# levayz/ProtoSAM

Measured on AMD Instinct MI355X. Metric: query-slices/sec (512x512) end-to-end ProtoSAM infer, higher is better.
Workload: dtype f16

## Files before the change

include/protosam_hip.h:

```cpp
#ifndef PROTOSAM_HIP_H
#define PROTOSAM_HIP_H
#include <stddef.h>
#ifdef __cplusplus
extern "C" {
#endif

int psam_gemm_f16(const void* A, const void* W, const float* bias, void* out, const float* resid, const float* gamma,
                  int M, int N, int K, int lda, int ldw, int ldo, int ldr, int resid_mod, int out_seg,
                  int out_seg_stride, int out_seg_off, int epilogue, void* stream);
int psam_gemm_f16_heads(const void* A, const void* W, const float* bias, void* out, int M, int N, int K, int lda, int ldw,
                        int hd, void* stream);
int psam_gemm_f16_ln(const void* A, const void* W, const float* bias, void* out, const float* resid, const float* gamma,
                     int M, int N, int K, int lda, int ldw, int ldo, int ldr, int resid_mod, int out_seg,
                     int out_seg_stride, int out_seg_off, int epilogue, void* out16, int ld16, float* stats,
                     const float* ln_mr, const float* ln_s, void* stream);
int psam_ln_finalize(const float* stats, int M, int D, float eps, float* mr, void* stream);


int psam_gemm_splitk_ranges(int M, int N, int K);
int psam_gemm_f16_splitk_ln(const void* A, const void* W, const float* bias, float* x, int M, int N, int K, int lda, int ldw, int ldx,
                            int ks, float* ws, const float* ln_w, const float* ln_b, float eps, void* out16, int ld16, void* stream);

int psam_gemm_set_tile(int tile);
int psam_gemm_asm_variant(int variant);
int psam_gemm_set_option(const char* name, int value);
int psam_gemm_set_workspace(void* ptr, size_t bytes);

int psam_layernorm(const float* x, const float* w, const float* b, void* y, float* y2, int M, int D, int ldx, int ldy,
                   float eps, int out_dtype, int zero_tail_rows, void* stream);

int psam_attention_f16(const void* qkv, void* out, const float* rel_h, const float* rel_w, const void* relq,
                       const void* rpack, const void* pad_row, int B, int N, int H, int hd, float scale, int mode, int gh,
                       int gw, int ws, int head_major, void* stream);
int psam_attention_set_variant(int v);
int psam_attention_fused_relpos(int B, int N, int H, int hd, int gh, int gw);

int psam_relpos(const void* qkv, const void* Rpack, float* rel_h, float* rel_w, void* relq, int B, int N, int H, int hd,
                int gw, int K, int windowed, float scale, int head_major, void* stream);

int psam_alp_bank(const float* sup, int ld, int h, int w, int C, const float* mask, const float* bmask, int MH, int MW,
                  int pool_w, int kernel_size, float thresh, float eps, float* bank, int cap, int* meta, int* slot_bg,
                  int* slot_fg, float* mres, int force_mode, void* stream);

int psam_alp_sim(const float* qry, long long q_bstride, int ld, int B, int npix, int C, const float* bank, int cap,
                 const int* meta, float eps, float sim_scale, float* part, float* pred, int which_only, void* stream);
int psam_alp_sim_pairs(const float* qry, long long q_bstride, int ld, int npix, int C, const void* tab, int n_entries,
                       int max_groups, float eps, float sim_scale, float* part, float* pred, void* stream);

int psam_patchify_bilinear(const float* img, int B, int C, int H, int W, int S, int P, int Kpad, void* out, void* stream);
int psam_bilinear_nchw(const float* in, int planes, int IH, int IW, int OH, int OW, float* out, void* stream);
int psam_resize2d(const float* in, int planes, int IH, int IW, int OH, int OW, int mode, float* out, void* stream);
int psam_bilinear_tokens(const float* in, long long in_bstride, int ld, int B, int ih, int iw, int C, int oh, int ow,
                         float* out, void* stream);
int psam_prob_argmax(const float* logits, int B, int IH, int IW, int OH, int OW, float* prob, void* pred, int* fg_sum,
                     void* stream);
int psam_broadcast_rows(const float* row, int D, float* out, int B, long long stride, long long off, void* stream);
int psam_prob2_argmax(const float* scores, int P, int IH, int IW, int OH, int OW, void* pred, float* pfg2, int* fg_sum,
                      float* prob, void* stream);
int psam_scores_prob_argmax(const float* scores, int P, int GH, int GW, int IH, int IW, int OH, int OW, float* prob, void* pred,
                            int* fg_sum, void* stream);
int psam_minmax(const float* x, int B, long long n_per_img, void* mm, void* stream);
int psam_sam_patchify(const float* img, const void* mm, int B, int S, int P, const float* mean3, const float* std3,
                      int quantise, void* out, void* u8out, void* stream);
int psam_normalize_chw(const void* x, int in_u8, int B, long long plane, const float* mean3, const float* std3,
                       float* y, void* stream);
int psam_im2col3x3(const void* in, int B, int H, int W, int C, void* out, void* stream);
int psam_cast_f16(const float* x, void* y, long long n, void* stream);
int psam_cast_f32(const void* x, float* y, long long n, void* stream);
int psam_gelu_f32(float* x, long long n, void* stream);
int psam_split_f16(const float* x, void* hi, void* lo, long long n, int write_hi, void* stream);

int psam_ccl(const void* pred, const float* pfg, int H, int W, int cap, int* labels, int* parent, int* counters,
             int* roots, int* acc_i, void* acc_u, double* acc_d, const int* fg_sum, double* tab, void* stream);
int psam_ccl_batch(const void* pred, const float* pfg, long long pfg_stride, int B, int H, int W, int cap, int* labels, int* parent,
                   int* counters, int* roots, int* acc_i, void* acc_u, double* acc_d, const int* fg_sum, double* tab, void* stream);

int psam_small_linear(const float* x, const float* x2, const float* W, const float* b, const float* resid, float* y,
                      int G, int M, int N, int K, long long xg, long long wg, long long bg, long long yg, int ldx,
                      int ldy, int act, void* stream);
int psam_small_linear_splitk(const float* x, const float* W, const float* b, const float* resid, float* y, float* parts, int M, int N,
                             int K, int ks, int ldx, int ldy, void* stream);
int psam_small_attention(const void* q, const float* k, const float* v, void* out, int B, int Tq, int Tk, int NH, int hd,
                         int ldq, int ldk, int ldv, int ldo, int q_f16, void* stream);
int psam_t2i_attention(const float* q, const void* K, const void* V, float* out, int B, int T, int Nk, int NH,
                       int kv_f32, void* stream);
int psam_t2i_attention_split(const float* q, const void* K, const void* V, float* out, int B, int T, int Nk, int NH,
                             int kv_f32, int S, float* part, void* stream);
int psam_gemm_f32(const float* a, const float* a2, int a2_mod, const float* w, const float* bias, const float* resid,
                  float* out, int M, int N, int K, int lda, int ldw, int ldo, void* stream);
int psam_gemm_f32_heads(const float* a, const float* a2, int a2_mod, const float* w, const float* bias, float* out, int M, int N, int K,
                        int lda, int ldw, int nk, int hd, void* stream);

int psam_gemm_f32x3(const float* a, const float* a2, int a2_mod, const void* wh, const void* wl, const float* bias, const float* resid,
                    float* out, int M, int N, int K, int lda, int ldw, int ldo, int nk, int hd, float acc_scale, void* stream);
int psam_ln_pe(const float* x, const float* add_vec, const float* w, const float* b, const float* pe, float* y32,
               void* y16, void* ype16, int M, int in_mod, int pe_mod, float eps, int do_ln, const int* img_of_prompt,
               void* stream);
int psam_dense_pe(const float* G, int gh, int gw, float* pe, void* stream);
int psam_prompt_tokens(const float* coords, const int* labels, const float* G, const float* type_emb,
                       const float* out_tok, int B, int Ns, float img_size, float* tokens, void* stream);
int psam_upscale_tail(const float* u1, const float* lnw, const float* lnb, const float* W2r, const float* b2,
                      const float* hyper, float* masks, int B, int g, void* stream);
int psam_mask_upsample(const float* low, int planes, int IN, int MID, int variant, float* out, void* stream);
int psam_mask_union(const float* low, int B, int C, int sel, int IN, int MID, int OUT, int variant, float thr,
                    float* pred, void* stream);
int psam_mask_union_seg(const float* low, int Pm, int C, int sel, int IN, const int* segs, int nseg, int nout, int MID, int OUT,
                        int variant, float thr, void* out, void* stream);

int psam_mask_stats(const float* low, int B, int C, int first, int nsel, int IN, int MID, int H, int W, int variant,
                    float thr, float off, int* stats, void* stream);
int psam_mask_binarize(const float* low, const int* idx, int n, int IN, int MID, int H, int W, int variant, float thr,
                       unsigned char* out, const unsigned char* label, long long* counts, void* stream);
int psam_plane_stats(const float* planes, int n, int H, int W, float thr, float off, int* stats, void* out, void* stream);

int psam_rle_workspace(int H, int W, long long* ints_per_mask);
int psam_rle_count(const unsigned char* masks, int n, int H, int W, int* cells, long long* totals, void* stream);
int psam_rle_write(const unsigned char* masks, int n, int H, int W, const int* cells, const long long* offsets, int* counts,
                   void* stream);
int psam_rle_decode(const long long* ends, const long long* offsets, int n, int H, int W, unsigned char* masks_out,
                    void* stream);

int psam_seg_counts(const void* pred, int pred_dtype, int pred_planes, long long pred_stride, const void* label,
                    int label_dtype, int label_planes, long long label_stride, int H, int W, const int* rows, int n,
                    long long* out, void* stream);

int psam_mask_downscale(const float* masks, const float* wts, int n, int g, float eps, float* out, void* stream);

int psam_neg_points(const int* labels, const float* pbg, const double* tab, int H, int W, int max_comp, int r, float thr,
                    unsigned long long* keys, void* stream);
int psam_neg_points_batch(const int* labels, const float* pbg, long long pbg_stride, const double* tabs, int cap, int P, int H,
                          int W, int max_comp, int r, float thr, unsigned long long* keys, void* stream);

int psam_volume_stats(const void* vol, int vol_dtype, long long n, float slope, float inter, double* out, void* stream);
int psam_volume_slices(const void* vol, int vol_dtype, int Z, int H, int W, float slope, float inter, float mean,
                       float inv_std, int S, int tile, int mode, float* out, void* stream);

int psam_im2col(const void* in, int B, int H, int W, int C, int kh, int kw, int stride, int dil, int pad, int ldo, void* out,
                void* stream);
int psam_im2col_stem(const float* img, int B, int H, int W, int ldo, void* out, void* stream);
int psam_maxpool3x3s2(const void* in, int B, int H, int W, int C, void* out, void* stream);

int psam_rotate_nearest(const float* src, float* dst, const float* xg, const float* yg, const float* rt6, int C, int H, int W,
                        int crop_y, int crop_x, int outH, int outW, void* stream);
int psam_resize_aa(const float* src, float* tmp, float* dst, int C, int H, int W, int OH, int OW, void* stream);

#ifdef __cplusplus
}
#endif
#endif
```

protosam_amd/_lib.py:

```python
import ctypes
import os

import torch

_HERE = os.path.dirname(os.path.abspath(__file__))
LIB_PATH = os.environ.get("PSAM_LIB_PATH") or os.path.join(_HERE, "libprotosam_hip.so")

c_void_p, c_int, c_float, c_longlong, c_size_t = ctypes.c_void_p, ctypes.c_int, ctypes.c_float, ctypes.c_longlong, ctypes.c_size_t

SIGNATURES = {
    "psam_gemm_f16": [c_void_p, c_void_p, c_void_p, c_void_p, c_void_p, c_void_p] + [c_int] * 12 + [c_void_p],
    "psam_gemm_f16_heads": [c_void_p, c_void_p, c_void_p, c_void_p] + [c_int] * 6 + [c_void_p],
    "psam_gemm_f16_ln": [c_void_p] * 6 + [c_int] * 12 + [c_void_p, c_int, c_void_p, c_void_p, c_void_p, c_void_p],
    "psam_ln_finalize": [c_void_p, c_int, c_int, c_float, c_void_p, c_void_p],
    "psam_gemm_splitk_ranges": [c_int, c_int, c_int],
    "psam_gemm_f16_splitk_ln": [c_void_p, c_void_p, c_void_p, c_void_p] + [c_int] * 7 + [c_void_p, c_void_p, c_void_p, c_float, c_void_p, c_int,
                                c_void_p],
    "psam_gemm_set_tile": [c_int],
    "psam_gemm_asm_variant": [c_int],
    "psam_gemm_set_option": [ctypes.c_char_p, c_int],
    "psam_gemm_set_workspace": [c_void_p, c_size_t],
    "psam_layernorm": [c_void_p, c_void_p, c_void_p, c_void_p, c_void_p, c_int, c_int, c_int, c_int, c_float,
                       c_int, c_int, c_void_p],
    "psam_attention_f16": [c_void_p, c_void_p, c_void_p, c_void_p, c_void_p, c_void_p, c_void_p, c_int, c_int, c_int, c_int,
                           c_float, c_int, c_int, c_int, c_int, c_int, c_void_p],
    "psam_attention_set_variant": [c_int],
    "psam_attention_fused_relpos": [c_int] * 6,
    "psam_relpos": [c_void_p, c_void_p, c_void_p, c_void_p, c_void_p] + [c_int] * 7 + [c_float, c_int, c_void_p],
    "psam_alp_bank": [c_void_p, c_int, c_int, c_int, c_int, c_void_p, c_void_p, c_int, c_int, c_int, c_int, c_float, c_float,
                      c_void_p, c_int, c_void_p, c_void_p, c_void_p, c_void_p, c_int, c_void_p],
    "psam_alp_sim": [c_void_p, c_longlong, c_int, c_int, c_int, c_int, c_void_p, c_int, c_void_p, c_float, c_float,
                     c_void_p, c_void_p, c_int, c_void_p],
    "psam_alp_sim_pairs": [c_void_p, c_longlong, c_int, c_int, c_int, c_void_p, c_int, c_int, c_float, c_float, c_void_p, c_void_p,
                           c_void_p],
    "psam_patchify_bilinear": [c_void_p, c_int, c_int, c_int, c_int, c_int, c_int, c_int, c_void_p, c_void_p],
    "psam_bilinear_nchw": [c_void_p, c_int, c_int, c_int, c_int, c_int, c_void_p, c_void_p],
    "psam_resize2d": [c_void_p, c_int, c_int, c_int, c_int, c_int, c_int, c_void_p, c_void_p],
    "psam_bilinear_tokens": [c_void_p, c_longlong, c_int, c_int, c_int, c_int, c_int, c_int, c_int, c_void_p, c_void_p],
    "psam_prob_argmax": [c_void_p, c_int, c_int, c_int, c_int, c_int, c_void_p, c_void_p, c_void_p, c_void_p],
    "psam_broadcast_rows": [c_void_p, c_int, c_void_p, c_int, c_longlong, c_longlong, c_void_p],
    "psam_prob2_argmax": [c_void_p, c_int, c_int, c_int, c_int, c_int, c_void_p, c_void_p, c_void_p, c_void_p, c_void_p],
    "psam_scores_prob_argmax": [c_void_p] + [c_int] * 7 + [c_void_p] * 4,
    "psam_minmax": [c_void_p, c_int, c_longlong, c_void_p, c_void_p],
    "psam_im2col3x3": [c_void_p, c_int, c_int, c_int, c_int, c_void_p, c_void_p],
    "psam_cast_f16": [c_void_p, c_void_p, c_longlong, c_void_p],
    "psam_cast_f32": [c_void_p, c_void_p, c_longlong, c_void_p],
    "psam_gelu_f32": [c_void_p, c_longlong, c_void_p],
    "psam_split_f16": [c_void_p, c_void_p, c_void_p, c_longlong, c_int, c_void_p],
    "psam_small_linear": [c_void_p] * 6 + [c_int] * 4 + [c_longlong] * 4 + [c_int] * 3 + [c_void_p],
    "psam_small_attention": [c_void_p] * 4 + [c_int] * 10 + [c_void_p],
    "psam_t2i_attention": [c_void_p] * 4 + [c_int] * 5 + [c_void_p],
    "psam_t2i_attention_split": [c_void_p] * 4 + [c_int] * 6 + [c_void_p] * 2,
    "psam_gemm_f32": [c_void_p, c_void_p, c_int, c_void_p, c_void_p, c_void_p, c_void_p] + [c_int] * 6 + [c_void_p],
    "psam_gemm_f32_heads": [c_void_p, c_void_p, c_int, c_void_p, c_void_p, c_void_p] + [c_int] * 7 + [c_void_p],
    "psam_gemm_f32x3": [c_void_p, c_void_p, c_int] + [c_void_p] * 5 + [c_int] * 8 + [c_float, c_void_p],
    "psam_small_linear_splitk": [c_void_p] * 6 + [c_int] * 6 + [c_void_p],
    "psam_ln_pe": [c_void_p] * 8 + [c_int, c_int, c_int, c_float, c_int, c_void_p, c_void_p],
    "psam_dense_pe": [c_void_p, c_int, c_int, c_void_p, c_void_p],
    "psam_prompt_tokens": [c_void_p] * 5 + [c_int, c_int, c_float, c_void_p, c_void_p],
    "psam_upscale_tail": [c_void_p] * 7 + [c_int, c_int, c_void_p],
    "psam_mask_upsample": [c_void_p, c_int, c_int, c_int, c_int, c_void_p, c_void_p],
    "psam_mask_union": [c_void_p, c_int, c_int, c_int, c_int, c_int, c_int, c_int, c_float, c_void_p, c_void_p],
    "psam_mask_union_seg": [c_void_p, c_int, c_int, c_int, c_int, c_void_p, c_int, c_int, c_int, c_int, c_int, c_float,
                            c_void_p, c_void_p],
    "psam_mask_stats": [c_void_p, c_int, c_int, c_int, c_int, c_int, c_int, c_int, c_int, c_int, c_float, c_float,
                        c_void_p, c_void_p],
    "psam_im2col": [c_void_p] + [c_int] * 10 + [c_void_p, c_void_p],
    "psam_im2col_stem": [c_void_p, c_int, c_int, c_int, c_int, c_void_p, c_void_p],
    "psam_maxpool3x3s2": [c_void_p, c_int, c_int, c_int, c_int, c_void_p, c_void_p],
    "psam_rotate_nearest": [c_void_p, c_void_p, c_void_p, c_void_p, c_void_p, c_int, c_int, c_int, c_int, c_int, c_int,
                            c_int, c_void_p],
    "psam_resize_aa": [c_void_p, c_void_p, c_void_p, c_int, c_int, c_int, c_int, c_int, c_void_p],
    "psam_volume_stats": [c_void_p, c_int, ctypes.c_longlong, c_float, c_float, c_void_p, c_void_p],
    "psam_volume_slices": [c_void_p, c_int, c_int, c_int, c_int, c_float, c_float, c_float, c_float, c_int, c_int, c_int,
                           c_void_p, c_void_p],
    "psam_neg_points": [c_void_p, c_void_p, c_void_p, c_int, c_int, c_int, c_int, c_float, c_void_p, c_void_p],
    "psam_neg_points_batch": [c_void_p, c_void_p, c_longlong, c_void_p] + [c_int] * 6 + [c_float, c_void_p, c_void_p],
    "psam_mask_downscale": [c_void_p, c_void_p, c_int, c_int, c_float, c_void_p, c_void_p],
    "psam_plane_stats": [c_void_p, c_int, c_int, c_int, c_float, c_float, c_void_p, c_void_p, c_void_p],
    "psam_rle_workspace": [c_int, c_int, ctypes.POINTER(c_longlong)],
    "psam_rle_count": [c_void_p, c_int, c_int, c_int, c_void_p, c_void_p, c_void_p],
    "psam_rle_write": [c_void_p, c_int, c_int, c_int, c_void_p, c_void_p, c_void_p, c_void_p],
    "psam_rle_decode": [c_void_p, c_void_p, c_int, c_int, c_int, c_void_p, c_void_p],
    "psam_seg_counts": [c_void_p, c_int, c_int, c_longlong, c_void_p, c_int, c_int, c_longlong, c_int, c_int, c_void_p, c_int,
                        c_void_p, c_void_p],
    "psam_mask_binarize": [c_void_p, c_void_p, c_int, c_int, c_int, c_int, c_int, c_int, c_float, c_void_p, c_void_p,
                           c_void_p, c_void_p],
    "psam_normalize_chw": [c_void_p, c_int, c_int, c_longlong, ctypes.POINTER(c_float), ctypes.POINTER(c_float),
                           c_void_p, c_void_p],
    "psam_ccl": [c_void_p, c_void_p, c_int, c_int, c_int] + [c_void_p] * 9 + [c_void_p],
    "psam_ccl_batch": [c_void_p, c_void_p, c_longlong, c_int, c_int, c_int, c_int] + [c_void_p] * 9 + [c_void_p],
    "psam_sam_patchify": [c_void_p, c_void_p, c_int, c_int, c_int, ctypes.POINTER(c_float), ctypes.POINTER(c_float),
                          c_int, c_void_p, c_void_p, c_void_p],
}

_lib = None


class HipExtensionMissing(RuntimeError):
    pass


def _preload_torch_hip_runtime():
    tl = os.path.join(os.path.dirname(torch.__file__), "lib", "libamdhip64.so")
    if os.path.exists(tl):
        ctypes.CDLL(tl, mode=ctypes.RTLD_GLOBAL)


def lib():
    global _lib
    if _lib is not None:
        return _lib
    if not os.path.exists(LIB_PATH):
        raise HipExtensionMissing(
            f"{LIB_PATH} not found: build it with `make -C protosam_amd/csrc` (or __graft_entry__.build()). "
            "protosam_amd has no CPU fallback.")
    _preload_torch_hip_runtime()
    L = ctypes.CDLL(LIB_PATH)
    for name, argtypes in SIGNATURES.items():
        fn = getattr(L, name)
        fn.argtypes = argtypes
        fn.restype = c_int
    _lib = L
    return L


def check(status, name):
    if status != 0:
        raise RuntimeError(f"{name} failed with status {status} (1 = bad argument, 2 = launch error)")
```

protosam_amd/csrc/gemm.hip:

```cpp
#include "common.h"
#include "gemm_asm_meta.h"
#include <stdlib.h>
#include <string.h>
#include <type_traits>
#include <map>
#include <string>
#include <vector>

enum { EPI_F16 = 0, EPI_GELU_F16 = 1, EPI_F32 = 2, EPI_RELU_F16 = 3 };

struct GemmArgs {
  const half_t* A;
  const half_t* W;
  const float* bias;
  void* out;
  const float* resid;
  const float* gamma;
  int M, N, K;
  int lda, ldw, ldo, ldr;
  int resid_mod;
  int out_seg;
  int out_seg_stride;
  int out_seg_off;
  int map_mode;
// ... 858 lines not shown
        bv[j][q] = p.bias ? *reinterpret_cast<const float4*>(p.bias + nbase + j * 32 + 8 * q + 4 * lg)
                          : make_float4(0.f, 0.f, 0.f, 0.f);
        if (LNF) sv[j][q] = *reinterpret_cast<const float4*>(p.ln_s + nbase + j * 32 + 8 * q + 4 * lg);
      }
    if (LNF) {
#pragma unroll
      for (int sidx = 0; sidx < 4; ++sidx) {
        int m = mbase + sidx * 32 + lr;
        m = m < p.M ? m : p.M - 1;
        mrv[sidx] = *reinterpret_cast<const float2*>(p.ln_mr + (size_t)m * 2);
      }
    }
    __builtin_amdgcn_sched_barrier(0);
    issue_next();
    __builtin_amdgcn_sched_barrier(0);
#pragma unroll
    for (int sidx = 0; sidx < 4; ++sidx) {
      if (LNF) {
        slab_park16h<true>(acc[sidx >> 1][sidx & 1][0], acc[sidx >> 1][sidx & 1][1], slab, bv, lane, EPI == EPI_GELU_F16, sv,
                           mrv[sidx]);
      } else {
        slab_park16h<false>(acc[sidx >> 1][sidx & 1][0], acc[sidx >> 1][sidx & 1][1], slab, bv, lane, EPI == EPI_GELU_F16, bv,
                            make_float2(0.f, 1.f));
      }
      slab_emit16h(slab, mbase + sidx * 32, nbase, lane, p);
    }
  }
}

template <int EPI, bool LNF = false, bool SPLITK = false>
__global__ __launch_bounds__(512) void gemm8kp_f16_kernel(GemmArgs p, int total) {
  extern __shared__ __attribute__((aligned(16))) half_t ring[];
  constexpr int HT = 128 * 64;
  const int ntn = p.N / 256;
  const int ntm = (p.M + 255) / 256;
  const int t = threadIdx.x, lane = t & 63;
  const int wv = __builtin_amdgcn_readfirstlane(t >> 6);
  const int wr = wv >> 2, wc = wv & 3;
  const int lr = lane & 31, lg = lane >> 5;
  half_t* slab = ring + 8 * HT + wv * 2048;
  const int nk = p.K / 64;
  const unsigned bh = 32u * (unsigned)p.ldw;
  const int arow0 = wr * 64 + lr, brow0 = wc * 32 + lr;

  const int KSP = SPLITK ? p.ksplit : 1;
  int idx = blockIdx.x, tm = 0, tn = 0;
  while (idx < total && !tile_map(idx / KSP, ntm, ntn, p.map_mode, tm, tn)) idx += gridDim.x;
  if (idx >= total) return;
  int k_lo = SPLITK ? (idx % KSP) * nk / KSP : 0, k_hi = SPLITK ? (idx % KSP + 1) * nk / KSP : nk;

  unsigned aoff[2][2], boff[2];
  auto offsets = [&](int m0, int n0) {
#pragma unroll
    for (int j = 0; j < 2; ++j) {
      const int lrow = j * 64 + (t >> 3);
      const int chunk = (t & 7) ^ ((lrow >> 1) & 7);
      const int arow = (lrow >> 6) * 128 + (lrow & 63);
      const int brow = (lrow >> 5) * 64 + (lrow & 31);
#pragma unroll
      for (int h = 0; h < 2; ++h) {
        int am = m0 + arow + h * 64;
        am = am < p.M ? am : p.M - 1;
        aoff[j][h] = (unsigned)am * (unsigned)p.lda + chunk * 8;
      }
      boff[j] = (unsigned)(n0 + brow) * (unsigned)p.ldw + chunk * 8;
    }
  };
  auto stage = [&](int which, int kt) {
    half_t* dst = ring + ((kt & 1) * 4 + which) * HT + wv * 512;
    const int h = which & 1;
#pragma unroll
    for (int j = 0; j < 2; ++j) {
      const half_t* g = which < 2 ? p.A + (aoff[j][h] + (unsigned)kt * 64u) : p.W + (boff[j] + h * bh + (unsigned)kt * 64u);
      glds16(g, dst + j * 4096);
    }
  };
  auto prologue = [&](int k0, int k1) {
    stage(0, k0); stage(2, k0); stage(3, k0); stage(1, k0);
    if (k1 - k0 > 1) stage(0, k0 + 1);
  };

  offsets(tm * 256, tn * 256);
  prologue(k_lo, k_hi);

  half8_t fa[2][2];
  half8_t fb[2][2][2];

#define RD_A(bufp, h, kh)                                                                                         \
  _Pragma("unroll") for (int i = 0; i < 2; ++i) _Pragma("unroll") for (int k2 = 0; k2 < 2; ++k2)                   \
      fa[i][k2] = *reinterpret_cast<const half8_t*>(&(bufp)[(h) * HT + lds_off64(arow0 + i * 32, ((kh) * 2 + k2) * 2 + lg)]);
#define RD_B(bufp, kh)                                                                                            \
  _Pragma("unroll") for (int b = 0; b < 2; ++b) _Pragma("unroll") for (int k2 = 0; k2 < 2; ++k2)                   \
      fb[kh][b][k2] = *reinterpret_cast<const half8_t*>(&(bufp)[(2 + b) * HT + lds_off64(brow0, ((kh) * 2 + k2) * 2 + lg)]);
#define MMA_H(a, kh)                                                                                              \
  _Pragma("unroll") for (int k2 = 0; k2 < 2; ++k2) _Pragma("unroll") for (int i = 0; i < 2; ++i)                   \
      _Pragma("unroll") for (int b = 0; b < 2; ++b)                                                               \
          acc[a][i][b] = __builtin_amdgcn_mfma_f32_32x32x16_f16(fb[kh][b][k2], fa[i][k2], acc[a][i][b], 0, 0, 0);
#define PHASE_SYNC_IN()                                   \
  __builtin_amdgcn_s_barrier();                           \
  asm volatile("s_waitcnt lgkmcnt(0)" ::: "memory");      \
  __builtin_amdgcn_sched_barrier(0);                      \
  __builtin_amdgcn_s_setprio(1);
#define PHASE_SYNC_OUT()                                  \
  __builtin_amdgcn_s_setprio(0);                          \
  __builtin_amdgcn_sched_barrier(0);                      \
  __builtin_amdgcn_s_barrier();                           \
  asm volatile("" ::: "memory");

  bool first = true;
  for (;;) {
    const int m0 = tm * 256, n0 = tn * 256;
    f32x16 acc[2][2][2];
#pragma unroll
    for (int a = 0; a < 2; ++a)
#pragma unroll
      for (int i = 0; i < 2; ++i)
#pragma unroll
        for (int b = 0; b < 2; ++b)
#pragma unroll
          for (int r = 0; r < 16; ++r) acc[a][i][b][r] = 0.f;

    if (first) { if (k_hi - k_lo > 1) wait_vmcnt<4>(); else wait_vmcnt<2>(); } else { wait_vmcnt<0>(); }
    first = false;
    __builtin_amdgcn_s_barrier();
    if (wr == 1) __builtin_amdgcn_s_barrier();
    asm volatile("" ::: "memory");

    for (int kt = k_lo; kt < k_hi; ++kt) {
      const half_t* buf = ring + (kt & 1) * 4 * HT;
      const bool more1 = kt + 1 < k_hi, more2 = kt + 2 < k_hi;
#define LOAD_PHASE(RDS, ST) RDS __builtin_amdgcn_sched_barrier(0); ST
      LOAD_PHASE(RD_B(buf, 0) __builtin_amdgcn_sched_barrier(0); RD_A(buf, 0, 0), if (more1) stage(2, kt + 1);)
      if (more1) wait_vmcnt<6>(); else wait_vmcnt<0>();
      PHASE_SYNC_IN();
      MMA_H(0, 0)
      PHASE_SYNC_OUT();
      LOAD_PHASE(RD_B(buf, 1) __builtin_amdgcn_sched_barrier(0); RD_A(buf, 0, 1), if (more1) stage(3, kt + 1);)
      if (more1) wait_vmcnt<6>(); else wait_vmcnt<0>();
      PHASE_SYNC_IN();
      MMA_H(0, 1)
      PHASE_SYNC_OUT();
      LOAD_PHASE(RD_A(buf, 1, 0), if (more1) stage(1, kt + 1);)
      if (more1) wait_vmcnt<6>(); else wait_vmcnt<0>();
      PHASE_SYNC_IN();
      MMA_H(1, 0)
      PHASE_SYNC_OUT();
      LOAD_PHASE(RD_A(buf, 1, 1), if (more2) stage(0, kt + 2);)
      if (more2) { wait_vmcnt<4>(); } else if (more1) { wait_vmcnt<2>(); } else { wait_vmcnt<0>(); }
      PHASE_SYNC_IN();
      MMA_H(1, 1)
      PHASE_SYNC_OUT();
#undef LOAD_PHASE
    }
    if (wr == 0) __builtin_amdgcn_s_barrier();

    int nidx = idx + gridDim.x, ntm_ = 0, ntn_ = 0;
    while (nidx < total && !tile_map(nidx / KSP, ntm, ntn, p.map_mode, ntm_, ntn_)) nidx += gridDim.x;
    const bool have = nidx < total;
    const int nk_lo = SPLITK && have ? (nidx % KSP) * nk / KSP : 0, nk_hi = SPLITK && have ? (nidx % KSP + 1) * nk / KSP : nk;
    auto issue_next = [&]() {
      if (have) {
        offsets(ntm_ * 256, ntn_ * 256);
        prologue(nk_lo, nk_hi);
      }
    };
    __builtin_amdgcn_sched_barrier(0);
#ifndef PSAM_EPI_EARLY_NEXT
#define PSAM_EPI_EARLY_NEXT 1
#endif
#if PSAM_EPI_EARLY_NEXT
    persist_epilogue<EPI, LNF, SPLITK>(acc, slab, m0 + wr * 128, n0 + wc * 64, lane, p, SPLITK ? idx % KSP : 0, issue_next);
#else
    issue_next();
    __builtin_amdgcn_sched_barrier(0);
    persist_epilogue<EPI, LNF, SPLITK>(acc, slab, m0 + wr * 128, n0 + wc * 64, lane, p, SPLITK ? idx % KSP : 0);
#endif
    if (!have) break;
    idx = nidx; tm = ntm_; tn = ntn_; k_lo = nk_lo; k_hi = nk_hi;
  }
#undef RD_A
#undef RD_B
#undef MMA_H
#undef PHASE_SYNC_IN
#undef PHASE_SYNC_OUT
}

template <int EPI, bool LNF = false>
static void launch8kp(const GemmArgs& p, hipStream_t s) {
  constexpr int LDS = 2 * 4 * 128 * 64 * 2 + 8 * 4096;
  static bool attr = false;
  if (!attr) {
    (void)hipFuncSetAttribute((const void*)gemm8kp_f16_kernel<EPI, LNF>, hipFuncAttributeMaxDynamicSharedMemorySize, LDS);
    attr = true;
  }
  const int ntm = (p.M + 255) / 256, ntn = p.N / 256;
  GemmArgs q = p;
  q.map_mode = pick_map_mode(ntm, ntn);
  const int total = tile_map_grid(ntm, ntn, q.map_mode);
  hipLaunchKernelGGL((gemm8kp_f16_kernel<EPI, LNF>), dim3(total < num_cus() ? total : num_cus()), dim3(512), LDS, s, q, total);
}

__global__ __launch_bounds__(256) void splitk_reduce_kernel(const float* __restrict__ ws, int ks, const float* __restrict__ bias,
                                                            const float* __restrict__ gamma, const float* resid, int ldr,
                                                            int resid_mod, float* out, int ldo, int M, int N) {
  const int n4 = N >> 2;
  const size_t i = (size_t)blockIdx.x * 256 + threadIdx.x;
  if (i >= (size_t)M * n4) return;
  const int m = (int)(i / n4), n = (int)(i - (size_t)m * n4) * 4;
  float4 v = bias ? *reinterpret_cast<const float4*>(bias + n) : make_float4(0.f, 0.f, 0.f, 0.f);
  for (int r = 0; r < ks; ++r) {
    const float4 q = *reinterpret_cast<const float4*>(ws + ((size_t)r * M + m) * N + n);
    v.x += q.x; v.y += q.y; v.z += q.z; v.w += q.w;
  }
  if (gamma) {
    const float4 g = *reinterpret_cast<const float4*>(gamma + n);
    v.x *= g.x; v.y *= g.y; v.z *= g.z; v.w *= g.w;
  }
  if (resid) {
    const size_t rrow = resid_mod ? (size_t)(m % resid_mod) : (size_t)m;
    const float4 r = *reinterpret_cast<const float4*>(resid + rrow * ldr + n);
    v.x += r.x; v.y += r.y; v.z += r.z; v.w += r.w;
  }
  *reinterpret_cast<float4*>(out + (size_t)m * ldo + n) = v;
}

struct KsWorkspace { float* ptr = nullptr; size_t bytes = 0; hipEvent_t done = nullptr; hipStream_t last = nullptr; bool used = false; };
static std::map<int, KsWorkspace> g_ks;
static KsWorkspace* ks_workspace() {
  int dev = 0;
  (void)hipGetDevice(&dev);
  auto it = g_ks.find(dev);
  return it == g_ks.end() || !it->second.ptr ? nullptr : &it->second;
}
extern "C" int psam_gemm_set_workspace(void* ptr, size_t bytes) {
  if (ptr && (reinterpret_cast<uintptr_t>(ptr) & 15)) return PSAM_ERR_ARG;
  int dev = 0;
  (void)hipGetDevice(&dev);
  KsWorkspace& w = g_ks[dev];
  w.ptr = (float*)ptr;
  w.bytes = ptr ? bytes : 0;
  w.used = false;
  return PSAM_OK;
}

static void launch8kp_splitk(const GemmArgs& p, hipStream_t s) {
  constexpr int LDS = 2 * 4 * 128 * 64 * 2 + 8 * 4096;
  static bool attr = false;
  if (!attr) {
    (void)hipFuncSetAttribute((const void*)gemm8kp_f16_kernel<EPI_F32, false, true>, hipFuncAttributeMaxDynamicSharedMemorySize, LDS);
    attr = true;
  }
  const int ntm = (p.M + 255) / 256, ntn = p.N / 256;
  GemmArgs q = p;
  q.map_mode = 1;
  KsWorkspace* w = ks_workspace();
  q.ks_ws = w->ptr;
  if (w->used && w->last != s) (void)hipStreamWaitEvent(s, w->done, 0);
  const int total = ntm * ntn * q.ksplit;
  hipLaunchKernelGGL((gemm8kp_f16_kernel<EPI_F32, false, true>), dim3(total < num_cus() ? total : num_cus()), dim3(512), LDS, s, q, total);
  const size_t n4 = (size_t)p.M * (p.N / 4);
  hipLaunchKernelGGL(splitk_reduce_kernel, dim3((unsigned)((n4 + 255) / 256)), dim3(256), 0, s, w->ptr, q.ksplit, p.bias, p.gamma,
                     p.resid, p.ldr, p.resid_mod, reinterpret_cast<float*>(p.out), p.ldo, p.M, p.N);
  if (!w->done) (void)hipEventCreateWithFlags(&w->done, hipEventDisableTiming);
  (void)hipEventRecord(w->done, s);
  w->last = s;
  w->used = true;
}


extern "C" const unsigned char psam_gemm_asm_co[];
extern "C" const unsigned char psam_gemm_asm_co_end[];
struct AsmGemmArgs {
  const void* A; const void* W; const void* bias; void* out; const void* resid; const void* gamma; const void* tab;
  int M, N, K, lda, ldw, ldo, ldr, G, flags, pad;
  void* trace;
  void* out16; float* stats; int ld16, pad2;
};
static_assert(sizeof(AsmGemmArgs) == 128, "kernarg layout of gemm_asm_gen.py");
struct AsmModule { hipModule_t mod = nullptr; int state = 0; std::map<int, std::vector<hipFunction_t>> fns; std::map<std::string, hipFunction_t> named; };
static std::map<int, AsmModule> g_asm;
static int g_asm_variant = 0;
extern "C" int psam_gemm_asm_variant(int v) {
  g_asm_variant = v;
  return PSAM_OK;
}
static AsmModule* asm_module() {
  AsmModule& m = g_asm[cur_device()];
  if (m.state == 0) {
    m.state = -1;
    const char* path = getenv("PSAM_GEMM_ASM_CO");
    hipError_t st = path ? hipModuleLoad(&m.mod, path) : hipModuleLoadData(&m.mod, psam_gemm_asm_co);
    if (st != hipSuccess) { (void)hipGetLastError(); return nullptr; }
    m.state = 1;
  }
  return m.state < 0 ? nullptr : &m;
}
static const hipFunction_t* asm_load(int family = 1) {
  AsmModule* m = asm_module();
  if (!m) return nullptr;
  const int key = family * 1000 + g_asm_variant;
  auto it = m->fns.find(key);
  if (it != m->fns.end()) return it->second.data();
  const char* names[3] = {"f16", "gelu", "f32"};
  const char* suffix[3] = {"", "_l2", "_ln"};
  const int nf = (family == 1 && g_asm_variant == 0) ? 9 : 3;
  std::vector<hipFunction_t> f(9, nullptr);
  for (int i = 0; i < nf; ++i) {
    std::string n = std::string(family == 2 ? "psam_gemm_asm2_" : "psam_gemm_asm_") + names[i % 3] + suffix[i / 3] +
                    (g_asm_variant > 0 ? "_v" + std::to_string(g_asm_variant) : std::string());
    if (hipModuleGetFunction(&f[i], m->mod, n.c_str()) != hipSuccess) {
      (void)hipGetLastError();
      if (i < 6) return nullptr;
      f[i] = nullptr;
    }
  }
  for (int i = nf; i < 6; ++i) f[i] = f[i - 3];
  return (m->fns[key] = f).data();
}
hipFunction_t psam_asm_function(const char* name) {
  AsmModule* m = asm_module();
  if (!m) return nullptr;
  auto it = m->named.find(name);
  if (it != m->named.end()) return it->second;
  hipFunction_t f = nullptr;
  if (hipModuleGetFunction(&f, m->mod, name) != hipSuccess) { (void)hipGetLastError(); f = nullptr; }
  return m->named[name] = f;
}
struct AsmTable { int grid; int* dev; };
static std::map<unsigned long long, AsmTable> g_asm_tabs;
static const AsmTable* asm_table(int ntm, int ntn, int mode, int halves = 0, int wg_per_cu = 1) {
  int dev = 0;
  (void)hipGetDevice(&dev);
  if (ntm >= 4096 || ntn >= (1 << 20)) return nullptr;
  const unsigned long long key = ((unsigned long long)eff_cus() << 52) | ((unsigned long long)ntm << 40) | ((unsigned long long)ntn << 20) | ((unsigned long long)(halves ? 1 : 0) << 19) |
                                 ((unsigned long long)(halves & 1) << 18) | ((unsigned long long)(wg_per_cu - 1) << 16) | ((unsigned long long)mode << 8) | (unsigned)dev;
  auto it = g_asm_tabs.find(key);
  if (it != g_asm_tabs.end()) return &it->second;
  const int total = tile_map_grid(ntm, ntn, mode);
  const int G = total < eff_cus() * wg_per_cu ? total : eff_cus() * wg_per_cu;
  std::vector<std::vector<int>> lists(G);
  for (int b = 0; b < G; ++b)
    for (int idx = b; idx < total; idx += G) {
      int tm = 0, tn = 0;
      if (!tile_map(idx, ntm, ntn, mode, tm, tn)) continue;
      if (!halves) { lists[b].push_back(tm | (tn << 16)); continue; }
      lists[b].push_back(tm | ((2 * tn) << 16));
      if (2 * tn + 1 < halves) lists[b].push_back(tm | ((2 * tn + 1) << 16));
    }
  size_t rows = 0;
  for (auto& l : lists) rows = l.size() > rows ? l.size() : rows;
  rows += 3;
  std::vector<int> h(rows * G, -1);
  for (int b = 0; b < G; ++b)
    for (size_t i = 0; i < lists[b].size(); ++i) h[i * G + b] = lists[b][i];
  AsmTable t;
  t.grid = G;
  t.dev = nullptr;
  if (hipMalloc((void**)&t.dev, h.size() * sizeof(int)) != hipSuccess) return nullptr;
  if (hipMemcpy(t.dev, h.data(), h.size() * sizeof(int), hipMemcpyHostToDevice) != hipSuccess) {
    (void)hipFree(t.dev);
    return nullptr;
  }
  return &(g_asm_tabs[key] = t);
}
static bool asm_eligible(const GemmArgs& p, int epilogue, int lnf) {
  if (lnf) {
    const hipFunction_t* f = asm_load(1);
    const bool cons = p.ln_mr || p.ln_s, prod = p.out16 || p.stats;
    if (!f || g_asm_variant != 0 || (cons && prod)) return false;
    if (cons && (!f[6 + epilogue] || !p.ln_mr || !p.ln_s || !p.bias || (reinterpret_cast<uintptr_t>(p.ln_mr) & 15) || (reinterpret_cast<uintptr_t>(p.ln_s) & 15))) return false;
    if (prod && (!f[8] || !p.out16 || !p.stats)) return false;
  }
  if (p.head_hd || p.out_seg || epilogue > EPI_F32) return false;
  if (p.resid_mod && (epilogue != EPI_F32 || !p.resid || p.resid_mod < 256 || (p.resid_mod & (p.resid_mod - 1)) != 0 || g_asm_variant != 0)) return false;
  if (p.N % 256 || p.K % 64 || p.K < 128 || p.M < 1) return false;
  if ((p.lda % 8) || (p.ldw % 8) || (reinterpret_cast<uintptr_t>(p.A) & 15) || (reinterpret_cast<uintptr_t>(p.W) & 15)) return false;
  const unsigned long long lim = 0xffffffffull;
  if ((unsigned long long)p.M * p.lda * 2 > lim || (unsigned long long)p.N * p.ldw * 2 > lim) return false;
  if (p.bias && (reinterpret_cast<uintptr_t>(p.bias) & 15)) return false;
  if (epilogue == EPI_F32) {
    if ((p.ldo % 4) || (reinterpret_cast<uintptr_t>(p.out) & 15) || (unsigned long long)p.M * p.ldo * 4 > lim) return false;
    if (p.resid && ((p.ldr % 4) || (reinterpret_cast<uintptr_t>(p.resid) & 15) || (unsigned long long)p.M * p.ldr * 4 > lim)) return false;
    if (p.gamma && (reinterpret_cast<uintptr_t>(p.gamma) & 15)) return false;
  } else {
    if (!p.wide16 || (unsigned long long)p.M * p.ldo * 2 > lim) return false;
  }
  return true;
}
static bool asm2_eligible(const GemmArgs& p, int epilogue, int lnf) {
  if (epilogue > EPI_F32 || (p.N % 128)) return false;
  GemmArgs q = p;
  q.N = 256;
  if (lnf || p.resid_mod || !asm_eligible(q, epilogue, 0)) return false;
  if ((unsigned long long)p.N * p.ldw * 2 > 0xffffffffull) return false;
  const int e = epilogue == EPI_F16 ? PSAM_ASM2_E_F16 : epilogue == EPI_GELU_F16 ? PSAM_ASM2_E_GELU : PSAM_ASM2_E_F32;
  return p.K / 64 >= e + 1 && p.K / 64 >= 3;
}
static int launch_asm(const GemmArgs& p, int epilogue, hipStream_t s, int family = 1) {
  const hipFunction_t* fns = asm_load(family);
  if (!fns) return PSAM_ERR_LAUNCH;
  const int ntm = (p.M + 255) / 256, ntn = family >= 2 ? p.N / 128 : p.N / 256;
  const AsmTable* t = asm_table(ntm, ntn, pick_map_mode(ntm, ntn));
  if (!t) return PSAM_ERR_LAUNCH;
  AsmGemmArgs a;
  a.A = p.A; a.W = p.W; a.bias = p.bias; a.out = p.out; a.resid = p.resid; a.gamma = p.gamma; a.tab = t->dev;
  a.M = p.M; a.N = p.N; a.K = p.K; a.lda = p.lda; a.ldw = p.ldw; a.ldo = p.ldo; a.ldr = p.resid ? p.ldr : 0; a.G = t->grid;
  a.flags = p.gamma ? 1 : 0;
  a.pad = (family == 1 && p.resid_mod > 0) ? p.resid_mod - 1 : -1;
  a.trace = nullptr;
  const bool ln_cons = family == 1 && p.ln_mr && p.ln_s, ln_prod = family == 1 && (p.out16 || p.stats);
  if (ln_cons) {
    a.resid = p.ln_mr;
    a.gamma = p.ln_s + p.N;
  }
  a.out16 = p.out16; a.stats = p.stats; a.ld16 = p.ld16; a.pad2 = 0;
  static const char* tr = getenv("PSAM_GEMM_ASM_TRACE");
  const bool trace = tr && g_asm_variant > 0;
  if (trace) { (void)hipMalloc(&a.trace, (size_t)t->grid * 32); (void)hipMemsetAsync(a.trace, 0, (size_t)t->grid * 32, s); }
  size_t sz = ln_prod ? sizeof(a) : 104;
  void* extra[] = {HIP_LAUNCH_PARAM_BUFFER_POINTER, &a, HIP_LAUNCH_PARAM_BUFFER_SIZE, &sz, HIP_LAUNCH_PARAM_END};
  const size_t out_bytes = (size_t)p.M * p.N * (epilogue == EPI_F32 ? 4 : 2);
  const int fsel = (ln_cons || ln_prod) ? 6 + epilogue : epilogue + ((family == 1 && out_bytes <= ((size_t)48 << 20)) ? 3 : 0);
  if (hipModuleLaunchKernel(fns[fsel], t->grid, 1, 1, 256, 1, 1, 0, s, nullptr, extra) != hipSuccess) {
    (void)hipGetLastError();
    return PSAM_ERR_LAUNCH;
  }
  if (trace) {
    std::vector<unsigned> h((size_t)t->grid * 8);
    (void)hipStreamSynchronize(s);
    (void)hipMemcpy(h.data(), a.trace, h.size() * 4, hipMemcpyDeviceToHost);
    (void)hipFree(a.trace);
    double loop = 0, epi = 0, kt = 0, tot = 0, rt = 0;
    unsigned tmax = 0;
    for (int b = 0; b < t->grid; ++b) rt += h[(size_t)t->grid * 4 + b * 4];
    for (int b = 0; b < t->grid; ++b) { loop += h[b * 4]; epi += h[b * 4 + 1]; kt += h[b * 4 + 2]; tot += h[b * 4 + 3]; tmax = h[b * 4 + 3] > tmax ? h[b * 4 + 3] : tmax; }
    const double tiles = kt / (p.K / 64);
    if (kt > 0) fprintf(stderr, "asm v%d %dx%dx%d epi%d: %.0f cycles per K-tile, %.0f cycles per epilogue (%.1f tiles per workgroup) kernel entry to exit: mean %.0f max %u cycles = %.1f us (shader clock %.0f MHz)\n", g_asm_variant, p.M, p.N,
                        p.K, epilogue, loop / kt, epi / tiles, tiles / t->grid, tot / t->grid, tmax, rt / t->grid * 0.01, rt > 0 ? tot / rt * 100.0 : 0.0);
  }
  return PSAM_OK;
}

static const AsmTable* asm_table_splitk(int ntm, int ntn, int ks) {
  int dev = 0;
  (void)hipGetDevice(&dev);
  if (ntm >= 4096 || ntn >= (1 << 16) || ks < 2 || ks > 8) return nullptr;
  const unsigned long long key = (1ull << 63) | ((unsigned long long)eff_cus() << 52) | ((unsigned long long)ntm << 40) | ((unsigned long long)ntn << 20) |
                                 ((unsigned long long)ks << 8) | (unsigned)dev;
  auto it = g_asm_tabs.find(key);
  if (it != g_asm_tabs.end()) return &it->second;
  const int mode = pick_map_mode(ntm, ntn);
  const int ntiles = tile_map_grid(ntm, ntn, mode);
  std::vector<int> items;
  for (int idx = 0; idx < ntiles; ++idx) {
    int tm = 0, tn = 0;
    if (!tile_map(idx, ntm, ntn, mode, tm, tn)) continue;
    for (int r = 0; r < ks; ++r) items.push_back(tm | (r << 12) | (tn << 16));
  }
  const int total = (int)items.size();
  const int G = total < eff_cus() ? total : eff_cus();
  const size_t rows = (size_t)(total + G - 1) / G + 3;
  std::vector<int> h(rows * G, -1);
  for (int i = 0; i < total; ++i) h[(size_t)(i / G) * G + (i % G)] = items[i];
  AsmTable t;
  t.grid = G;
  t.dev = nullptr;
  if (hipMalloc((void**)&t.dev, h.size() * sizeof(int)) != hipSuccess) return nullptr;
  if (hipMemcpy(t.dev, h.data(), h.size() * sizeof(int), hipMemcpyHostToDevice) != hipSuccess) {
    (void)hipFree(t.dev);
    return nullptr;
  }
  return &(g_asm_tabs[key] = t);
}

#define SKR_MAXV 8
__global__ __launch_bounds__(256) void splitk_reduce_ln_kernel(const float* __restrict__ ws, int ks, const float* __restrict__ bias,
                                                               float* __restrict__ x, int ldx, const float* __restrict__ ln_w,
                                                               const float* __restrict__ ln_b, float eps, half_t* __restrict__ out16, int ld16,
                                                               int M, int N) {
  const int row = blockIdx.x * 4 + (threadIdx.x >> 6), lane = threadIdx.x & 63;
  if (row >= M) return;
  const int nv = N >> 2;
  const size_t Mp = (size_t)((M + 255) & ~255);
  float4 v[SKR_MAXV];
  float* xr = x + (size_t)row * ldx;
#pragma unroll
  for (int k = 0; k < SKR_MAXV; ++k) {
    const int i = lane + 64 * k;
    if (i < nv) v[k] = bias ? reinterpret_cast<const float4*>(bias)[i] : make_float4(0.f, 0.f, 0.f, 0.f);
  }
  for (int r = 0; r < ks; ++r) {
    const float4* pr = reinterpret_cast<const float4*>(ws + ((size_t)r * Mp + row) * N);
#pragma unroll
    for (int k = 0; k < SKR_MAXV; ++k) {
      const int i = lane + 64 * k;
      if (i < nv) { const float4 q = pr[i]; v[k].x += q.x; v[k].y += q.y; v[k].z += q.z; v[k].w += q.w; }
    }
  }
  float s = 0.f;
#pragma unroll
  for (int k = 0; k < SKR_MAXV; ++k) {
    const int i = lane + 64 * k;
    if (i < nv) {
      const float4 q = reinterpret_cast<const float4*>(xr)[i];
      v[k].x += q.x; v[k].y += q.y; v[k].z += q.z; v[k].w += q.w;
      reinterpret_cast<float4*>(xr)[i] = v[k];
      s += (v[k].x + v[k].y) + (v[k].z + v[k].w);
    }
  }
  if (!out16) return;
  float mean = 0.f, rstd = 1.f;
  if (ln_w) {
    mean = wave_sum(s) / (float)N;
    float q = 0.f;
#pragma unroll
    for (int k = 0; k < SKR_MAXV; ++k) {
      const int i = lane + 64 * k;
      if (i < nv) {
        const float a = v[k].x - mean, c = v[k].y - mean, d = v[k].z - mean, e = v[k].w - mean;
        q += (a * a + c * c) + (d * d + e * e);
      }
    }
    rstd = 1.0f / sqrtf(wave_sum(q) / (float)N + eps);
  }
#pragma unroll
  for (int k = 0; k < SKR_MAXV; ++k) {
    const int i = lane + 64 * k;
    if (i < nv) {
      float o0 = v[k].x, o1 = v[k].y, o2 = v[k].z, o3 = v[k].w;
      if (ln_w) {
        const float4 ww = reinterpret_cast<const float4*>(ln_w)[i], bb = reinterpret_cast<const float4*>(ln_b)[i];
        o0 = (o0 - mean) * rstd * ww.x + bb.x; o1 = (o1 - mean) * rstd * ww.y + bb.y;
        o2 = (o2 - mean) * rstd * ww.z + bb.z; o3 = (o3 - mean) * rstd * ww.w + bb.w;
      }
      half4_t h = {(half_t)o0, (half_t)o1, (half_t)o2, (half_t)o3};
      *reinterpret_cast<half4_t*>(out16 + (size_t)row * ld16 + i * 4) = h;
    }
  }
}

extern "C" int psam_gemm_splitk_ranges(int M, int N, int K) {
  if (M <= 0 || N <= 0 || K <= 0 || (N % 256) || (K % 64) || N > 64 * 4 * SKR_MAXV) return 0;
  const int tiles = ((M + 255) / 256) * (N / 256), nkt = K / 64, ncu = eff_cus();
  if (tiles * 2 > ncu) return 0;
  int ks = ncu / tiles;
  if (ks > 8) ks = 8;
  while (ks >= 2 && nkt / ks < 16) --ks;
  if (ks < 2 || tiles * ks * 4 < ncu * 3) return 0;
  return psam_asm_function("psam_gemm_asm_f32_sk") ? ks : 0;
}

extern "C" int psam_gemm_f16_splitk_ln(const void* A, const void* W, const float* bias, float* x, int M, int N, int K, int lda, int ldw,
                                       int ldx, int ks, float* ws, const float* ln_w, const float* ln_b, float eps, void* out16, int ld16,
                                       void* stream) {
  if (ks < 2 || ks > 8 || ks != psam_gemm_splitk_ranges(M, N, K) || !ws || !x || (ldx % 4) || (ln_w && !ln_b) || (out16 && (ld16 % 4)))
    return PSAM_ERR_ARG;
  if ((reinterpret_cast<uintptr_t>(ws) | reinterpret_cast<uintptr_t>(x) | reinterpret_cast<uintptr_t>(bias) | reinterpret_cast<uintptr_t>(ln_w) |
       reinterpret_cast<uintptr_t>(ln_b)) & 15 || (reinterpret_cast<uintptr_t>(out16) & 7))
    return PSAM_ERR_ARG;
  GemmArgs p;
  p.A = (const half_t*)A; p.W = (const half_t*)W; p.bias = nullptr; p.out = ws; p.resid = nullptr; p.gamma = nullptr;
  p.M = M; p.N = N; p.K = K; p.lda = lda; p.ldw = ldw; p.ldo = N; p.ldr = 0;
  p.resid_mod = 0; p.out_seg = 0; p.out_seg_stride = 0; p.out_seg_off = 0; p.map_mode = 0; p.head_hd = 0;
  p.out16 = nullptr; p.ld16 = 0; p.stats = nullptr; p.ln_mr = nullptr; p.ln_s = nullptr; p.wide16 = false; p.ksplit = 1; p.ks_ws = nullptr;
  if (!asm_eligible(p, EPI_F32, 0) || (unsigned long long)ks * ((M + 255) & ~255) * N * 4 > 0xffffffffull) return PSAM_ERR_ARG;
  hipFunction_t fn = psam_asm_function("psam_gemm_asm_f32_sk");
  const AsmTable* t = asm_table_splitk((M + 255) / 256, N / 256, ks);
  if (!fn || !t) return PSAM_ERR_LAUNCH;
  AsmGemmArgs a;
  a.A = A; a.W = W; a.bias = nullptr; a.out = ws; a.resid = nullptr; a.gamma = nullptr; a.tab = t->dev;
  a.M = M; a.N = N; a.K = K; a.lda = lda; a.ldw = ldw; a.ldo = N; a.ldr = 0; a.G = t->grid; a.flags = 0; a.pad = ks;
  a.trace = nullptr; a.out16 = nullptr; a.stats = nullptr; a.ld16 = 0; a.pad2 = 0;
  size_t sz = 104;
  void* extra[] = {HIP_LAUNCH_PARAM_BUFFER_POINTER, &a, HIP_LAUNCH_PARAM_BUFFER_SIZE, &sz, HIP_LAUNCH_PARAM_END};
  hipStream_t s = (hipStream_t)stream;
  if (hipModuleLaunchKernel(fn, t->grid, 1, 1, 256, 1, 1, 0, s, nullptr, extra) != hipSuccess) {
    (void)hipGetLastError();
    return PSAM_ERR_LAUNCH;
  }
  hipLaunchKernelGGL(splitk_reduce_ln_kernel, dim3((M + 3) / 4), dim3(256), 0, s, ws, ks, bias, x, ldx, ln_w, ln_b, eps, (half_t*)out16, ld16, M, N);
  return psam_launch_status();
}

enum { OPT_ASM = 0, OPT_HALF, OPT_SPLITK, OPT_NSPLIT, OPT_DEEP, OPT_SMALL, OPT_COUNT };
static const char* const g_opt_names[OPT_COUNT] = {"asm", "half_tiles", "splitk", "nsplit", "deep", "small"};
static const char* const g_opt_env[OPT_COUNT] = {"PSAM_GEMM_ASM", "PSAM_GEMM_HALF", "PSAM_GEMM_SPLITK", "PSAM_GEMM_NSPLIT", "PSAM_GEMM_DEEP", "PSAM_GEMM_SMALL"};
static int g_opt[OPT_COUNT] = {-1, -1, -1, -1, -1, -1};
static int gemm_option(int i) {
  if (g_opt[i] < 0) { const char* e = getenv(g_opt_env[i]); g_opt[i] = e ? (atoi(e) != 0) : 1; }
  return g_opt[i];
}
extern "C" int psam_gemm_set_option(const char* name, int value) {
  if (name && strcmp(name, "max_wgs") == 0) { g_max_wgs = value > 0 ? value : 0; return PSAM_OK; }
  for (int i = 0; i < OPT_COUNT; ++i)
    if (name && strcmp(name, g_opt_names[i]) == 0) { g_opt[i] = value != 0; return PSAM_OK; }
  return PSAM_ERR_ARG;
}
static int g_tile_override = -1;
extern "C" int psam_gemm_set_tile(int t) {
  g_tile_override = t;
  return PSAM_OK;
}
static int pick_tile(int M, int N, int K, int epilogue) {
  if (g_tile_override < 0) {
    const char* e = getenv("PSAM_GEMM_TILE");
    g_tile_override = e ? atoi(e) : 0;
  }
  if (g_tile_override > 0) return g_tile_override;
  if (N % 256 == 0) {
    const long t256 = (long)((M + 255) / 256) * (N / 256);
    const long ncu = eff_cus();
    const long rounds = (t256 + ncu - 1) / ncu;
    const bool short_f32 = epilogue == EPI_F32 && K < 2048;
    const int fill = short_f32 ? 95 : (epilogue == EPI_F32 || rounds > 1) ? 80 : 50;
    if (K >= 768 && t256 * 100 >= rounds * ncu * fill) {
      return gemm_option(OPT_ASM) ? 15 : 11;
    }
  }
  if (N % 128 == 0 && K >= 768) {
    const int half_on = gemm_option(OPT_HALF);
    const long th = (long)((M + 255) / 256) * (N / 128), ncu = eff_cus();
    if (half_on && th * 20 >= ncu * 9) return 16;
  }
  return 1;
}

struct LnFold {
  void* out16 = nullptr;
  int ld16 = 0;
  float* stats = nullptr;
  const float* ln_mr = nullptr;
  const float* ln_s = nullptr;
};

static int gemm_dispatch(const void* A, const void* W, const float* bias, void* out, const float* resid,
                         const float* gamma, int M, int N, int K, int lda, int ldw, int ldo, int ldr,
                         int resid_mod, int out_seg, int out_seg_stride, int out_seg_off, int epilogue, int head_hd,
                         void* stream, const LnFold& ln = LnFold()) {
  if (M <= 0 || N <= 0 || K <= 0 || (N % BN) != 0 || (K % BK) != 0 || (lda % 8) != 0 || (ldw % 8) != 0 ||
      (ldo % 4) != 0 || (resid && (ldr % 4) != 0))
    return PSAM_ERR_ARG;
  if (epilogue < 0 || epilogue > 3) return PSAM_ERR_ARG;
  if (epilogue == EPI_RELU_F16 && resid_mod != 0) return PSAM_ERR_ARG;
  GemmArgs p;
  p.A = (const half_t*)A;
  p.W = (const half_t*)W;
  p.bias = bias;
  p.out = out;
  p.resid = resid;
  p.gamma = gamma;
  p.M = M;
  p.N = N;
  p.K = K;
  p.lda = lda;
  p.ldw = ldw;
  p.ldo = ldo;
  p.ldr = ldr;
  p.resid_mod = resid_mod;
  p.out_seg = out_seg;
  p.out_seg_stride = out_seg_stride;
  p.out_seg_off = out_seg_off;
  { static int mm = -2; if (mm == -2) { const char* e = getenv("PSAM_GEMM_MAP"); mm = e ? atoi(e) : (xcd_maps_apply() ? 0 : 1); } p.map_mode = mm; }
  p.head_hd = head_hd;
  p.out16 = (half_t*)ln.out16;
  p.ld16 = ln.ld16;
  p.stats = ln.stats;
  p.ln_mr = ln.ln_mr;
  p.ln_s = ln.ln_s;
  const bool ln_prod = ln.out16 || ln.stats, ln_cons = ln.ln_mr || ln.ln_s;
  if (ln_prod && (epilogue != EPI_F32 || (ln.out16 && ((ln.ld16 % 8) != 0 || (reinterpret_cast<uintptr_t>(ln.out16) & 15) != 0)))) return PSAM_ERR_ARG;
  if (ln_cons && (!(epilogue == EPI_F16 || epilogue == EPI_GELU_F16) || !ln.ln_mr || !ln.ln_s)) return PSAM_ERR_ARG;
  const int ntm = (M + BM - 1) / BM, ntn = N / BN;
  dim3 grid(tile_map_grid(ntm, ntn, p.map_mode)), block(256);
  hipStream_t s = (hipStream_t)stream;
  int tsel = epilogue == EPI_RELU_F16 ? 1 : pick_tile(M, N, K, epilogue);
  p.wide16 = (ldo % 8) == 0 && (reinterpret_cast<uintptr_t>(out) & 15) == 0 && (!head_hd || head_hd % 8 == 0);
  if (tsel == 16 && !asm2_eligible(p, epilogue, ln_prod || ln_cons)) tsel = (g_tile_override > 0 || ln_prod || ln_cons) ? 15 : 1;
  if (tsel == 15 && !asm_eligible(p, epilogue, ln_prod || ln_cons)) tsel = (N % 256 == 0) ? 11 : 1;
  if (tsel != 1 && tsel != 11 && tsel != 12 && tsel != 13 && tsel != 15 && tsel != 16) tsel = (N % 256 == 0) ? 11 : 1;
  if (tsel == 11 && (N % 256) != 0) tsel = 1;
  if (tsel == 11 && epilogue != EPI_F32 && !p.wide16) tsel = 1;
  if (ln_cons && !p.wide16) return PSAM_ERR_ARG;
  {
    static const bool logging = getenv("PSAM_GEMM_LOG") != nullptr;
    if (logging) {
      static std::map<std::string, int> seen;
      char key[160];
      snprintf(key, sizeof(key), "%d x %d x %d epilogue %d ln %d%d head_hd %d out_seg %d resid_mod %d -> tile %d", M, N, K, epilogue, (int)ln_prod,
               (int)ln_cons, head_hd, out_seg, resid_mod, tsel);
      if (seen[key]++ == 0) fprintf(stderr, "psam_gemm_f16: %s\n", key);
    }
  }
  if (tsel == 15) return launch_asm(p, epilogue, s);
  if (tsel == 16) return launch_asm(p, epilogue, s, 2);
  p.ksplit = 1;
  p.ks_ws = nullptr;
  {
    const int ks_on = gemm_option(OPT_SPLITK);
    const bool auto_sel = g_tile_override <= 0;
    const KsWorkspace* ksw = ks_workspace();
    hipStreamCaptureStatus cap = hipStreamCaptureStatusNone;
    if (ksw && hipStreamIsCapturing(s, &cap) != hipSuccess) { (void)hipGetLastError(); cap = hipStreamCaptureStatusNone; }
    if (ks_on && auto_sel && ksw && cap == hipStreamCaptureStatusNone && tsel == 1 && epilogue == EPI_F32 && !ln_prod && !ln_cons && !head_hd && N % 256 == 0 &&
        out_seg == 0 && (ldo % 4) == 0) {
      const int t256 = ((M + 255) / 256) * (N / 256), nkt = K / 64;
      int ks = num_cus() / t256;
      if (ks > nkt / 24) ks = nkt / 24;
      if (ks > 8) ks = 8;
      while (ks >= 2 && (size_t)ks * M * N * sizeof(float) > ksw->bytes) --ks;
      if (ks >= 2 && t256 * ks * 4 >= num_cus() * 3) {
        p.ksplit = ks;
        launch8kp_splitk(p, s);
        return psam_launch_status();
      }
    }
  }
  const bool lnf = ln_prod || ln_cons;
  if ((tsel == 13 || (tsel == 1 && g_tile_override <= 0 && gemm_option(OPT_SMALL) && (int)grid.x * 2 <= num_cus())) && !lnf && !head_hd && K >= 64 &&
      epilogue != EPI_RELU_F16 && (epilogue == EPI_F32 || (ldo % 4) == 0)) {
    switch (epilogue) {
      case EPI_F16: launch_s64<EPI_F16>(p, s); break;
      case EPI_GELU_F16: launch_s64<EPI_GELU_F16>(p, s); break;
      default: launch_s64<EPI_F32>(p, s); break;
    }
    return psam_launch_status();
  }
  if (tsel == 13) tsel = 1;
  if ((tsel == 12 || (tsel == 1 && g_tile_override <= 0 && gemm_option(OPT_DEEP) && (int)grid.x <= num_cus())) && !lnf && K >= 256 &&
      epilogue != EPI_RELU_F16) {
    switch (epilogue) {
      case EPI_F16: launch_deep<EPI_F16>(p, grid, s); break;
      case EPI_GELU_F16: launch_deep<EPI_GELU_F16>(p, grid, s); break;
      default: launch_deep<EPI_F32>(p, grid, s); break;
    }
    return psam_launch_status();
  }
  if (tsel == 12) tsel = 1;
  if (tsel == 11) {
    if (lnf) {
      if (epilogue == EPI_F16) launch8kp<EPI_F16, true>(p, s);
      else if (epilogue == EPI_GELU_F16) launch8kp<EPI_GELU_F16, true>(p, s);
      else launch8kp<EPI_F32, true>(p, s);
    } else {
      if (epilogue == EPI_F16) launch8kp<EPI_F16>(p, s);
      else if (epilogue == EPI_GELU_F16) launch8kp<EPI_GELU_F16>(p, s);
      else launch8kp<EPI_F32>(p, s);
    }
    return psam_launch_status();
  }
  if (lnf) {
    switch (epilogue) {
      case EPI_F16: hipLaunchKernelGGL((gemm_f16_kernel<EPI_F16, true>), grid, block, 0, s, p); break;
      case EPI_GELU_F16: hipLaunchKernelGGL((gemm_f16_kernel<EPI_GELU_F16, true>), grid, block, 0, s, p); break;
      default: hipLaunchKernelGGL((gemm_f16_kernel<EPI_F32, true>), grid, block, 0, s, p); break;
    }
    return psam_launch_status();
  }
  switch (epilogue) {
    case EPI_F16: hipLaunchKernelGGL(gemm_f16_kernel<EPI_F16>, grid, block, 0, s, p); break;
    case EPI_GELU_F16: hipLaunchKernelGGL(gemm_f16_kernel<EPI_GELU_F16>, grid, block, 0, s, p); break;
    case EPI_RELU_F16: hipLaunchKernelGGL(gemm_f16_kernel<EPI_RELU_F16>, grid, block, 0, s, p); break;
    default: hipLaunchKernelGGL(gemm_f16_kernel<EPI_F32>, grid, block, 0, s, p); break;
  }
  return psam_launch_status();
}

extern "C" int psam_gemm_f16(const void* A, const void* W, const float* bias, void* out, const float* resid,
                             const float* gamma, int M, int N, int K, int lda, int ldw, int ldo, int ldr,
                             int resid_mod, int out_seg, int out_seg_stride, int out_seg_off, int epilogue,
                             void* stream) {
  {
    const int ns_on = gemm_option(OPT_NSPLIT);
    const int ncu = num_cus();
    const int ntm = (M + 255) / 256;
    const bool whole16 = epilogue == EPI_GELU_F16 && pick_tile(M, N, K, epilogue) == 16 && K / 64 >= PSAM_ASM2_E_GELU + 1 &&
                         (lda % 8) == 0 && (ldw % 8) == 0 && (ldo % 8) == 0 && ((reinterpret_cast<uintptr_t>(A) | reinterpret_cast<uintptr_t>(W) |
                           reinterpret_cast<uintptr_t>(out) | reinterpret_cast<uintptr_t>(bias)) & 15) == 0;
    if (ns_on && !whole16 && g_tile_override <= 0 && (epilogue == EPI_F16 || epilogue == EPI_GELU_F16) && out_seg == 0 && N % 256 == 0 &&
        K >= 768 && ntm > 0 && ntm <= ncu) {
      const int ntn = N / 256, c1 = ncu / ntm;
      if (c1 >= 1 && c1 < ntn && ntm * c1 * 100 >= ncu * 95 && (ntn - c1) * 2 <= c1) {
        const int n1 = c1 * 256;
        const half_t* Wh = (const half_t*)W;
        int st = gemm_dispatch(A, W, bias, out, resid, gamma, M, n1, K, lda, ldw, ldo, ldr, resid_mod, 0, 0, 0, epilogue, 0, stream);
        if (st != PSAM_OK) return st;
        return gemm_dispatch(A, Wh + (size_t)n1 * ldw, bias ? bias + n1 : nullptr, (half_t*)out + n1, resid, gamma ? gamma + n1 : nullptr,
                             M, N - n1, K, lda, ldw, ldo, ldr, resid_mod, 0, 0, 0, epilogue, 0, stream);
      }
    }
  }
  return gemm_dispatch(A, W, bias, out, resid, gamma, M, N, K, lda, ldw, ldo, ldr, resid_mod, out_seg, out_seg_stride,
                       out_seg_off, epilogue, 0, stream);
}

extern "C" int psam_gemm_f16_ln(const void* A, const void* W, const float* bias, void* out, const float* resid,
                                const float* gamma, int M, int N, int K, int lda, int ldw, int ldo, int ldr, int resid_mod,
                                int out_seg, int out_seg_stride, int out_seg_off, int epilogue, void* out16, int ld16,
                                float* stats, const float* ln_mr, const float* ln_s, void* stream) {
  LnFold ln;
  ln.out16 = out16; ln.ld16 = ld16; ln.stats = stats; ln.ln_mr = ln_mr; ln.ln_s = ln_s;
  if (stats && (N % 64) != 0) return PSAM_ERR_ARG;
  return gemm_dispatch(A, W, bias, out, resid, gamma, M, N, K, lda, ldw, ldo, ldr, resid_mod, out_seg, out_seg_stride,
                       out_seg_off, epilogue, 0, stream, ln);
}

extern "C" int psam_gemm_f16_heads(const void* A, const void* W, const float* bias, void* out, int M, int N, int K, int lda,
                                   int ldw, int hd, void* stream) {
  if (hd <= 0 || (hd % 4) != 0 || (N % hd) != 0) return PSAM_ERR_ARG;
  return gemm_dispatch(A, W, bias, out, nullptr, nullptr, M, N, K, lda, ldw,  N, 0, 0, 0, 0, 0, EPI_F16,
                       hd, stream);
}
```

protosam_amd/csrc/gemm_asm_gen.py:

```python
#!/usr/bin/env python3
import sys

from asm_common import AsmWriter, kernel_begin, kernel_end, kernel_metadata, module_text, younger

import os
_pol = (os.environ.get("PSAM_GEN_GEMM_DMA", ",") + ",").split(",")
DMA_POLICY_A, DMA_POLICY_W = (" " + _pol[0] if _pol[0] else ""), (" " + _pol[1] if _pol[1] else "")
GELU_MODE = os.environ.get("PSAM_GEN_GELU", "sigpoly")

S_KARG = 0
S_WG = 2
S_A, S_W, S_BIAS, S_OUT, S_RES, S_GAM, S_TAB = 4, 6, 8, 10, 12, 14, 16
S_M, S_N, S_K, S_LDA, S_LDW, S_LDO, S_LDR, S_G, S_FLAGS = 18, 19, 20, 21, 22, 23, 24, 25, 26
S_RMASK = 27
SRD_A, SRD_B, SRD_O, SRD_R, SRD_BIAS, SRD_GAM = 28, 32, 36, 40, 44, 48
S_M0BASE = 68
S_KREM, S_DKREM, S_NK = 69, 70, 71
S_TCUR, S_TDMA, S_TNEXT, S_CUR, S_STRIDE = 72, 73, 74, 75, 76
S_WV, S_WR, S_WC = 77, 78, 79
S_FA, S_FB = 80, 81
S_LDA2, S_LDW2 = 82, 83
S_T0, S_T1, S_T2, S_T3, S_T4 = 84, 85, 86, 87, 88
S_ROW4, S_TOFF, S_N0X4, S_ROFF, S_RROW4 = 89, 90, 91, 92, 93
S_C = 52
S_ROW28, S_RROW28 = 65, 66
S_ACC_LOOP, S_ACC_EPI, S_NKT = 67, 94, 95
S_TS0, S_TS1, S_TRP = 96, 98, 100
S_SKQ, S_SKREM, S_SKR, S_SKT = 96, 97, 98, 99
NUM_SGPR = 102

V_TID = 0
V_FA = 1
V_FB = 5
V_DA = 9
V_DB = 17
V_LANE, V_LR, V_LG, V_T0, V_T1, V_T2, V_T3 = 25, 26, 27, 28, 29, 30, 31
V_SFOFF, V_MFOFF, V_RSOFF, V_RSTD = 25, 26, 27, 28
SRD_O16, SRD_ST = 96, 52
S_LD16X2, S_O16ROW4, S_STROW4, S_O16ROW28, S_STROW28, S_PARTS8, S_O16OFF, S_STOFF = 56, 57, 58, 59, 60, 61, 62, 63
S_EXROW = 100
V_O16, V_ST, V_SQ, V_SUM = 25, 254, 26, 252
SRD_MR, SRD_SF, SRD_MF = 40, 48, 96
V_SET = [32, 64, 96, 128]
V_PARK = 160
V_EADDR = 176
V_EM = [180, 212]
V_TMP = 244
V_BIAS = 96
V_OLANE, V_RLANE, V_O, V_R = 248, 249, 250, 251
V_BG0, V_GG0, V_BG1, V_GG1 = 168, 172, 244, 28

LDS_BUF = 16384
LDS_SLAB = 131072

EPI_F16, EPI_GELU_F16, EPI_F32 = 0, 1, 2


class Gen(AsmWriter):
    def __init__(self, name, epi, sched):
        AsmWriter.__init__(self, name)
        self.epi, self.sched = epi, sched
        self.lnc = bool(sched.get("ln_cons")) and epi != EPI_F32
        self.lnp = bool(sched.get("ln_prod")) and epi == EPI_F32
        self.sk = bool(sched.get("splitk")) and epi == EPI_F32 and not self.lnp
        assert not (self.sk and sched.get("trace"))

    def item_rows_cols(self, item):
        e = self.e
        e("s_and_b32 s%d, s%d, 0x%x" % (S_T0, item, 0xfff if self.sk else 0xffff))
        e("s_lshr_b32 s%d, s%d, 16" % (S_T1, item))

    def item_ktiles(self, item, dst):
        e = self.e
        e("s_bfe_u32 s%d, s%d, 0x4000c" % (S_SKR, item))
        e("s_cmp_lt_u32 s%d, s%d" % (S_SKR, S_SKREM))
        e("s_addc_u32 s%d, s%d, 0" % (dst, S_SKQ))

    def switch_tile(self):
        e = self.e
        done, out = self.u("L_sw_none"), self.u("L_sw_out")
        e("s_mov_b32 s%d, s%d" % (S_TDMA, S_TNEXT))
        e("s_cmp_eq_u32 s%d, -1" % S_TDMA)
        e("s_cbranch_scc1 %s" % done)
        self.item_rows_cols(S_TDMA)
        e("s_lshl_b32 s%d, s%d, 8" % (S_T0, S_T0))
        e("s_lshl_b32 s%d, s%d, 8" % (S_T1, S_T1))
        e("s_mul_i32 s%d, s%d, s%d" % (S_T2, S_T0, S_LDA2))
        e("s_mul_hi_u32 s%d, s%d, s%d" % (S_T3, S_T0, S_LDA2))
        e("s_add_u32 s%d, s%d, s%d" % (SRD_A, S_A, S_T2))
        e("s_addc_u32 s%d, s%d, s%d" % (SRD_A + 1, S_A + 1, S_T3))
        e("s_sub_u32 s%d, s%d, s%d" % (S_T4, S_M, S_T0))
        e("s_mul_i32 s%d, s%d, s%d" % (SRD_A + 2, S_T4, S_LDA2))
        e("s_mul_i32 s%d, s%d, s%d" % (S_T2, S_T1, S_LDW2))
        e("s_mul_hi_u32 s%d, s%d, s%d" % (S_T3, S_T1, S_LDW2))
        e("s_add_u32 s%d, s%d, s%d" % (SRD_B, S_W, S_T2))
        e("s_addc_u32 s%d, s%d, s%d" % (SRD_B + 1, S_W + 1, S_T3))
        e("s_sub_u32 s%d, s%d, s%d" % (S_T4, S_N, S_T1))
        e("s_mul_i32 s%d, s%d, s%d" % (SRD_B + 2, S_T4, S_LDW2))
        if self.sk:
            self.item_ktiles(S_TDMA, S_DKREM)
            e("s_min_u32 s%d, s%d, s%d" % (S_SKT, S_SKR, S_SKREM))
            e("s_mul_i32 s%d, s%d, s%d" % (S_T4, S_SKR, S_SKQ))
            e("s_add_u32 s%d, s%d, s%d" % (S_T4, S_T4, S_SKT))
            e("s_lshl_b32 s%d, s%d, 7" % (S_T4, S_T4))
            for srd in (SRD_A, SRD_B):
                e("s_add_u32 s%d, s%d, s%d" % (srd, srd, S_T4))
                e("s_addc_u32 s%d, s%d, 0" % (srd + 1, srd + 1))
                e("s_max_u32 s%d, s%d, s%d" % (srd + 2, srd + 2, S_T4))
                e("s_sub_u32 s%d, s%d, s%d" % (srd + 2, srd + 2, S_T4))
        else:
            e("s_mov_b32 s%d, s%d" % (S_DKREM, S_NK))
        e("s_add_u32 s%d, s%d, s%d" % (S_CUR, S_CUR, S_STRIDE))
        e("s_load_dword s%d, s[%d:%d], s%d" % (S_TNEXT, S_TAB, S_TAB + 1, S_CUR))
        e("s_branch %s" % out)
        self.lab(done)
        e("s_mov_b32 s%d, 0" % (SRD_A + 2))
        e("s_mov_b32 s%d, 0" % (SRD_B + 2))
        e("s_mov_b32 s%d, 0x7fffffff" % S_DKREM)
        self.lab(out)

    def dma_m0(self, p):
        j = p & 7
        const = (65536 if p >= 8 else 0) + (j >> 2) * 32768 + (j & 3) * 4096
        return "s_add_u32 m0, s%d, 0x%x" % (S_M0BASE, const)

    def dma_issue(self, p):
        if p < 8:
            return "buffer_load_dwordx4 v%d, s[%d:%d], 0 offen%s lds" % (V_DA + p, SRD_A, SRD_A + 3, DMA_POLICY_A)
        return "buffer_load_dwordx4 v%d, s[%d:%d], 0 offen%s lds" % (V_DB + p - 8, SRD_B, SRD_B + 3, DMA_POLICY_W)

    def dma_advance(self):
        out = []
        for srd in (SRD_A, SRD_B):
            out += ["s_add_u32 s%d, s%d, 128" % (srd, srd), "s_addc_u32 s%d, s%d, 0" % (srd + 1, srd + 1),
                    "s_max_u32 s%d, s%d, 128" % (srd + 2, srd + 2), "s_sub_u32 s%d, s%d, 128" % (srd + 2, srd + 2)]
        out.append("s_sub_u32 s%d, s%d, 1" % (S_DKREM, S_DKREM))
        return out

    def frag_read(self, st, ks, idx):
        if idx < 4:
            return "ds_read_b128 v[%d:%d], v%d offset:%d" % (V_SET[st] + 4 * idx, V_SET[st] + 4 * idx + 3, V_FA + ks, idx * 4096)
        j = idx - 4
        return "ds_read_b128 v[%d:%d], v%d offset:%d" % (V_SET[st] + 16 + 4 * j, V_SET[st] + 16 + 4 * j + 3, V_FB + ks, j * 4096)

    def mfma(self, st, rb, cb, zero):
        blk = (rb * 4 + cb) * 16
        a = "v[%d:%d]" % (V_SET[st] + 16 + 4 * cb, V_SET[st] + 16 + 4 * cb + 3)
        b = "v[%d:%d]" % (V_SET[st] + 4 * rb, V_SET[st] + 4 * rb + 3)
        cc = "0" if zero else "a[%d:%d]" % (blk, blk + 15)
        return "v_mfma_f32_32x32x16_f16 a[%d:%d], %s, %s, %s" % (blk, blk + 15, a, b, cc)

    def build_slots(self):
        sc = self.sched
        slots = [[] for _ in range(64)]
        for i in range(16):
            if not sc.get("no_reads"):
                slots[sc["rd23"][i]].append(self.frag_read(2 + i // 8, 2 + i // 8, i % 8))
        for i, r in enumerate((V_FA + 2, V_FA + 3, V_FB + 2, V_FB + 3)):
            slots[sc["tog23"] + i].append("v_xor_b32 v%d, 0x%x, v%d" % (r, LDS_BUF, r))
        if not sc.get("no_epilogue"):
            slots[sc.get("pre_slot", 17)] += ["s_cmp_eq_u32 s%d, 1" % S_KREM, "s_cbranch_scc1 L_pre_%s" % self.name, "L_pre_ret_%s:" % self.name]
        if self.lnc and not sc.get("no_epilogue"):
            slots[48] += ["s_cmp_eq_u32 s%d, 1" % S_KREM, "s_cbranch_scc1 L_pre2_%s" % self.name, "L_pre2_ret_%s:" % self.name]
        a = sc["barA"]
        if not sc.get("no_barrier"):
            slots[a] += ["s_waitcnt lgkmcnt(0)", "s_barrier"]
        slots[a] += ["s_cmp_eq_u32 s%d, 0" % S_DKREM, "s_cbranch_scc1 L_switch_%s" % self.name, "L_switch_ret_%s:" % self.name]
        for p in range(16):
            s = sc["dma"][p]
            if sc.get("no_dma"):
                continue
            slots[s - 1].append(self.dma_m0(p))
            slots[s].append(self.dma_issue(p))
        last = sc["dma"][15]
        adv = self.dma_advance()
        for i, ins in enumerate(adv):
            slots[min(63, last + 1 + i // 3)].append(ins)
        slots[min(63, last + 1)].append("s_xor_b32 s%d, s%d, 0x%x" % (S_M0BASE, S_M0BASE, LDS_BUF))
        b = sc["barB"]
        issued = sum(1 for p in range(16) if sc["dma"][p] <= b)
        if not sc.get("no_barrier"):
            slots[b] += ["s_waitcnt vmcnt(%d)" % (0 if sc.get("no_dma") else issued), "s_barrier"]
        if sc.get("prio"):
            slots[0].insert(0, "s_setprio %d" % sc["prio"])
        for i in range(16):
            s = sc["rd01"][i]
            assert s > b
            if not sc.get("no_reads"):
                slots[s].append(self.frag_read(i // 8, i // 8, i % 8))
        return slots

    def ktile(self, slots, zero_first):
        e = self.e
        for s in range(64):
            ks, rb, cb = s // 16, (s % 16) // 4, s % 4
            if s == 0:
                e("s_waitcnt lgkmcnt(8)")
            if s == 16:
                e("s_waitcnt lgkmcnt(15)")
            e(self.mfma(ks, rb, cb, zero_first and ks == 0))
            for ins in slots[s]:
                if ins.endswith(":"):
                    self.lab(ins[:-1])
                else:
                    e(ins)
            if s == 15 and zero_first:
                e("s_branch L_after_ks0_%s" % self.name)
                return

    def gelu_pair(self, x, t):
        e = self.e
        d, n, p = t, t + 2, t + 4
        mode = self.sched.get("gelu_mode", "packed")
        if mode == "none":
            return
        e("v_pk_mul_f32 v[%d:%d], v[%d:%d], v[%d:%d]" % (n, n + 1, x, x + 1, x, x + 1))
        for i in range(2):
            e("v_fma_f32 v%d, |v%d|, s%d, 1.0" % (d + i, x + i, S_C))
        e("v_pk_mul_f32 v[%d:%d], v[%d:%d], s[%d:%d] op_sel_hi:[1,0]" % (n, n + 1, n, n + 1, S_C + 4, S_C + 5))
        for i in range(2):
            e(("v_mov_b32 v%d, v%d" if mode == "notrans" else "v_rcp_f32 v%d, v%d") % (d + i, d + i))
        for i in range(2):
            e(("v_mov_b32 v%d, v%d" if mode == "notrans" else "v_exp_f32 v%d, v%d") % (n + i, n + i))
        e("v_pk_fma_f32 v[%d:%d], v[%d:%d], s[%d:%d], v[%d:%d] op_sel_hi:[1,0,1]" % (p, p + 1, d, d + 1, S_C + 2, S_C + 3, V_TMP + 8, V_TMP + 9))
        for k in range(3):
            e("v_pk_fma_f32 v[%d:%d], v[%d:%d], v[%d:%d], s[%d:%d] op_sel_hi:[1,1,0]" % (p, p + 1, p, p + 1, d, d + 1, S_C + 6 + 2 * k, S_C + 7 + 2 * k))
        e("v_pk_mul_f32 v[%d:%d], v[%d:%d], v[%d:%d] neg_lo:[0,1] neg_hi:[0,1]" % (p, p + 1, d, d + 1, p, p + 1))
        e("v_pk_fma_f32 v[%d:%d], v[%d:%d], v[%d:%d], 1.0 op_sel_hi:[1,1,0]" % (p, p + 1, p, p + 1, n, n + 1))
        for i in range(2):
            e("v_bfi_b32 v%d, s%d, v%d, v%d" % (p + i, S_C + 12, p + i, x + i))
        e("v_pk_mul_f32 v[%d:%d], v[%d:%d], 0.5 op_sel_hi:[1,0]" % (x, x + 1, x, x + 1))
        e("v_pk_fma_f32 v[%d:%d], v[%d:%d], v[%d:%d], v[%d:%d]" % (x, x + 1, x, x + 1, p, p + 1, x, x + 1))

    def gelu_quad(self, xa, ta, xb, tb):
        e = self.e
        mode = self.sched.get("gelu_mode", GELU_MODE)
        if mode != "sigpoly":
            self.gelu_pair(xa, ta)
            self.gelu_pair(xb, tb)
            return
        P = ((xa, ta, ta + 2), (xb, tb, tb + 2))
        for (x, u, q) in P:
            e("v_pk_mul_f32 v[%d:%d], v[%d:%d], v[%d:%d]" % (u, u + 1, x, x + 1, x, x + 1))
        for (x, u, q) in P:
            e("v_pk_fma_f32 v[%d:%d], v[%d:%d], s[%d:%d], v[%d:%d] op_sel_hi:[1,0,1]" % (q, q + 1, u, u + 1, S_C, S_C + 1, V_TMP + 8, V_TMP + 9))
        for k in range(3):
            for (x, u, q) in P:
                e("v_pk_fma_f32 v[%d:%d], v[%d:%d], v[%d:%d], s[%d:%d] op_sel_hi:[1,1,0]" % (q, q + 1, q, q + 1, u, u + 1, S_C + 2 + 2 * k, S_C + 3 + 2 * k))
        for (x, u, q) in P:
            e("v_pk_mul_f32 v[%d:%d], v[%d:%d], v[%d:%d]" % (q, q + 1, x, x + 1, q, q + 1))
        for i in range(2):
            for (x, u, q) in P:
                e("v_exp_f32 v%d, v%d" % (q + i, q + i))
        for (x, u, q) in P:
            e("v_pk_add_f32 v[%d:%d], v[%d:%d], 1.0 op_sel_hi:[1,0]" % (q, q + 1, q, q + 1))
        for i in range(2):
            for (x, u, q) in P:
                e("v_rcp_f32 v%d, v%d" % (q + i, q + i))
        for (x, u, q) in P:
            e("v_pk_mul_f32 v[%d:%d], v[%d:%d], v[%d:%d]" % (x, x + 1, x, x + 1, q, q + 1))

    def tile_offsets(self, esize):
        e = self.e
        self.item_rows_cols(S_TCUR)
        e("s_lshl_b32 s%d, s%d, 8" % (S_T0, S_T0))
        e("s_lshl_b32 s%d, s%d, 8" % (S_T1, S_T1))
        e("s_mul_i32 s%d, s%d, s%d" % (S_TOFF, S_T0, S_LDO))
        e("s_add_u32 s%d, s%d, s%d" % (S_TOFF, S_TOFF, S_T1))
        e("s_lshl_b32 s%d, s%d, %d" % (S_TOFF, S_TOFF, 1 if esize == 2 else 2))
        if self.sk:
            e("s_bfe_u32 s%d, s%d, 0x4000c" % (S_SKR, S_TCUR))
            e("s_add_u32 s%d, s%d, 255" % (S_SKT, S_M))
            e("s_andn2_b32 s%d, s%d, 255" % (S_SKT, S_SKT))
            e("s_mul_i32 s%d, s%d, s%d" % (S_SKT, S_SKT, S_LDO))
            e("s_lshl_b32 s%d, s%d, 2" % (S_SKT, S_SKT))
            e("s_mul_i32 s%d, s%d, s%d" % (S_SKT, S_SKT, S_SKR))
            e("s_add_u32 s%d, s%d, s%d" % (S_TOFF, S_TOFF, S_SKT))
        e("s_lshl_b32 s%d, s%d, 2" % (S_N0X4, S_T1))

    F16_BIAS, F16_EM = 180, (96, 128)
    F32_RING, F32_EM = (180, 212, 96), 128

    def resid_loads(self, slab, vm, dest=None):
        e = self.e
        rb, h = slab >> 1, slab & 1
        kind, base = dest if dest else ("v", self.F32_RING[slab % 3])
        for it in range(8):
            e("buffer_load_dwordx4 %s[%d:%d], v%d, s[%d:%d], 0 offen offset:%d%s" % (kind, base + 4 * it, base + 4 * it + 3, V_R, SRD_R, SRD_R + 3, h * 256,
                                                                                   self.sched.get("resid_policy", "")))
            vm.append(("res", slab))
            if it < 7:
                e("v_add_u32 v%d, s%d, v%d" % (V_R, S_RROW4, V_R))
        if h == 0:
            e("v_subrev_u32 v%d, s%d, v%d" % (V_R, S_RROW28, V_R))
        else:
            e("v_add_u32 v%d, s%d, v%d" % (V_R, S_RROW4, V_R))

    def pre_epilogue(self):
        e = self.e
        vm = []
        self.item_rows_cols(S_TCUR)
        e("s_lshl_b32 s%d, s%d, 8" % (S_T0, S_T0))
        e("s_lshl_b32 s%d, s%d, 8" % (S_T1, S_T1))
        e("s_lshl_b32 s%d, s%d, 2" % (S_N0X4, S_T1))
        if self.epi == EPI_F32:
            if self.sched.get("trace"):
                e("s_mul_i32 s%d, s%d, s%d" % (S_ROFF, S_T0, S_LDR))
            else:
                e("s_and_b32 s%d, s%d, s%d" % (S_T2, S_T0, S_RMASK))
                e("s_mul_i32 s%d, s%d, s%d" % (S_ROFF, S_T2, S_LDR))
            e("s_add_u32 s%d, s%d, s%d" % (S_ROFF, S_ROFF, S_T1))
            e("s_lshl_b32 s%d, s%d, 2" % (S_ROFF, S_ROFF))
            e("v_add_u32 v%d, s%d, v%d" % (V_R, S_ROFF, V_RLANE))
            for h in range(2):
                bb, gg = (V_BG0, V_GG0) if h == 0 else (V_BG1, V_GG1)
                e("buffer_load_dwordx4 v[%d:%d], v%d, s[%d:%d], s%d offen offset:%d" % (bb, bb + 3, V_TMP + 11, SRD_BIAS, SRD_BIAS + 3, S_N0X4, h * 256))
                e("buffer_load_dwordx4 v[%d:%d], v%d, s[%d:%d], s%d offen offset:%d" % (gg, gg + 3, V_TMP + 11, SRD_GAM, SRD_GAM + 3, S_N0X4, h * 256))
                vm += [("bg", 0), ("bg", 0)]
            self.resid_loads(0, vm)
            self.resid_loads(1, vm)
        else:
            for cb in range(4):
                for q in range(4):
                    r = self.F16_BIAS + (cb * 4 + q) * 4
                    e("buffer_load_dwordx4 v[%d:%d], v%d, s[%d:%d], s%d offen offset:%d" % (r, r + 3, V_TMP + 11, SRD_BIAS, SRD_BIAS + 3, S_N0X4, (cb * 32 + 8 * q) * 4))
                    vm.append(("bias", 0))
        return vm

    def pre2_epilogue(self):
        e = self.e
        vm = []
        e("s_and_b32 s%d, s%d, 0xffff" % (S_T0, S_TCUR))
        e("s_lshr_b32 s%d, s%d, 16" % (S_T1, S_TCUR))
        e("s_lshl_b32 s%d, s%d, 12" % (S_T2, S_T1))
        e("s_lshl_b32 s%d, s%d, 12" % (S_T3, S_T0))
        e("s_lshl_b32 s%d, s%d, 11" % (S_T4, S_T0))
        for cb in range(4):
            e("buffer_load_dwordx4 v[%d:%d], v%d, s[%d:%d], s%d offen offset:%d" % (96 + 4 * cb, 99 + 4 * cb, V_SFOFF, SRD_SF, SRD_SF + 3, S_T2, cb * 512))
            vm.append(("sf", 0))
        for rb in range(4):
            e("buffer_load_dwordx4 v[%d:%d], v%d, s[%d:%d], s%d offen offset:%d" % (112 + 4 * rb, 115 + 4 * rb, V_MFOFF, SRD_MF, SRD_MF + 3, S_T3, rb * 512))
            vm.append(("mf", 0))
        for rb in range(4):
            e("buffer_load_dword v%d, v%d, s[%d:%d], s%d offen offset:%d" % (V_RSTD + rb, V_RSOFF, SRD_MR, SRD_MR + 3, S_T4, rb * 256))
            vm.append(("rs", 0))
        return vm

    def younger(self, vm, tag):
        return younger(vm, tag)

    def epilogue_f16(self, gelu, vm):
        e = self.e
        self.c("---- epilogue: bias (+ GELU) -> fp16, through the wave's slab so that 16 lanes store one 256-byte row piece")
        e("s_nop 7")
        self.tile_offsets(2)
        e("v_add_u32 v%d, s%d, v%d" % (V_O, S_TOFF, V_OLANE))
        e("s_waitcnt vmcnt(%d)" % self.younger(vm, ("bias", 0)))
        if self.lnc:
            self.c("folded LayerNorm: acc -= mean_row * s_col, one rank-1 MFMA per block (fp16 hi / lo operands: fp32-accurate)")
            e("s_waitcnt vmcnt(%d)" % self.younger(vm, ("rs", 0)))
            for rb in range(4):
                for cb in range(4):
                    blk = (rb * 4 + cb) * 16
                    e("v_mfma_f32_32x32x16_f16 a[%d:%d], v[%d:%d], v[%d:%d], a[%d:%d]" % (blk, blk + 15, 96 + 4 * cb, 99 + 4 * cb, 112 + 4 * rb, 115 + 4 * rb, blk, blk + 15))
            e("s_nop 7")
            e("s_nop 7")
            e("s_nop 3")
        for rb in range(4):
            em = self.F16_EM[rb & 1]
            for cb in range(4):
                for q in range(4):
                    blk = (rb * 4 + cb) * 16 + 4 * q
                    t = V_TMP
                    for i in range(4):
                        e("v_accvgpr_read_b32 v%d, a%d" % (t + i, blk + i))
                    b = self.F16_BIAS + (cb * 4 + q) * 4
                    if self.lnc:
                        rp, hs = V_RSTD + (rb & ~1), rb & 1
                        for hh in range(2):
                            e("v_pk_fma_f32 v[%d:%d], v[%d:%d], v[%d:%d], v[%d:%d] op_sel:[0,%d,0] op_sel_hi:[1,%d,1]" % (
                                t + 2 * hh, t + 2 * hh + 1, t + 2 * hh, t + 2 * hh + 1, rp, rp + 1, b + 2 * hh, b + 2 * hh + 1, hs, hs))
                    else:
                        e("v_pk_add_f32 v[%d:%d], v[%d:%d], v[%d:%d]" % (t, t + 1, t, t + 1, b, b + 1))
                        e("v_pk_add_f32 v[%d:%d], v[%d:%d], v[%d:%d]" % (t + 2, t + 3, t + 2, t + 3, b + 2, b + 3))
                    if gelu:
                        self.gelu_quad(t, self.F16_EM[(rb + 1) & 1], t + 2, self.F16_EM[(rb + 1) & 1] + 8)
                    e("v_cvt_pk_f16_f32 v%d, v%d, v%d" % (t, t, t + 1))
                    e("v_cvt_pk_f16_f32 v%d, v%d, v%d" % (t + 1, t + 2, t + 3))
                    e("ds_write_b64 v%d, v[%d:%d]" % (V_PARK + cb * 4 + q, t, t + 1))
            for it in range(8):
                e("ds_read_b128 v[%d:%d], v%d offset:%d" % (em + 4 * it, em + 4 * it + 3, V_EADDR + (it & 3), (it >> 2) * 4096))
            for it in range(8):
                e("s_waitcnt lgkmcnt(%d)" % (7 - it))
                e("buffer_store_dwordx4 v[%d:%d], v%d, s[%d:%d], 0 offen%s" % (em + 4 * it, em + 4 * it + 3, V_O, SRD_O, SRD_O + 3, self.sched.get("store_policy", "")))
                e("v_add_u32 v%d, s%d, v%d" % (V_O, S_ROW4, V_O))

    def epilogue_f32(self, vm):
        e = self.e
        deep = self.sched.get("deep_ring", False)
        self.c("---- epilogue: out = resid + gamma * (acc + bias) in fp32; eight 32x64 slabs through the wave's 8 KiB; the residual")
        self.c("     slabs come through a ring of three (two requested in the last K-tile, one more ahead of every slab processed).")
        e("s_nop 7")
        self.tile_offsets(4)
        e("v_add_u32 v%d, s%d, v%d" % (V_O, S_TOFF, V_OLANE))
        if self.lnp:
            self.lnp_setup()
        self.resid_loads(2, vm)
        nog = self.u("L_gamma")
        e("s_bitcmp1_b32 s%d, 0" % S_FLAGS)
        e("s_cbranch_scc1 %s" % nog)
        e("s_waitcnt vmcnt(%d)" % self.younger(vm, ("bg", 0)))
        for gg in (V_GG0, V_GG1):
            for i in range(4):
                e("v_mov_b32 v%d, 1.0" % (gg + i))
        self.lab(nog)
        em = self.F32_EM
        R0, R1, R2 = self.F32_RING
        if deep:
            where = {0: ("v", R0), 1: ("v", R1), 2: ("v", R2), 3: ("a", 0), 4: ("v", R0), 5: ("a", 32), 6: ("v", R1), 7: ("a", 64)}
            after_park = {0: 3, 1: 5, 2: 7}
            after_slab = {0: 4, 1: 6}
        else:
            where = dict((j, ("v", self.F32_RING[j % 3])) for j in range(8))
            after_park = {}
            after_slab = dict((j, j + 3) for j in range(5))
        for slab in range(8):
            rb, h = slab >> 1, slab & 1
            for cbl in range(2):
                for q in range(4):
                    blk = (rb * 4 + 2 * h + cbl) * 16 + 4 * q
                    e("ds_write_b128 v%d, a[%d:%d]" % (V_PARK + cbl * 4 + q, blk, blk + 3))
            for it in range(8):
                e("ds_read_b128 v[%d:%d], v%d offset:%d" % (em + 4 * it, em + 4 * it + 3, V_EADDR + (it & 3), (it >> 2) * 4096))
            if slab in after_park:
                e("s_waitcnt lgkmcnt(7)")
                self.resid_loads(after_park[slab], vm, where[after_park[slab]])
            kind, rbase = where[slab]
            bb, gg = (V_BG0, V_GG0) if h == 0 else (V_BG1, V_GG1)
            e("s_waitcnt vmcnt(%d)" % self.younger(vm, ("res", slab)))
            for it in range(8):
                if kind == "a":
                    for i in range(4):
                        e("v_accvgpr_read_b32 v%d, a%d" % (R2 + 4 * it + i, rbase + 4 * it + i))
                e("s_waitcnt lgkmcnt(%d)" % (7 - it))
                r = em + 4 * it
                rr = (R2 if kind == "a" else rbase) + 4 * it
                for half in range(2):
                    e("v_pk_add_f32 v[%d:%d], v[%d:%d], v[%d:%d]" % (r + 2 * half, r + 2 * half + 1, r + 2 * half, r + 2 * half + 1, bb + 2 * half, bb + 2 * half + 1))
                for half in range(2):
                    e("v_pk_fma_f32 v[%d:%d], v[%d:%d], v[%d:%d], v[%d:%d]" % (r + 2 * half, r + 2 * half + 1, r + 2 * half, r + 2 * half + 1, gg + 2 * half, gg + 1 + 2 * half,
                                                                      rr + 2 * half, rr + 2 * half + 1))
                e("buffer_store_dwordx4 v[%d:%d], v%d, s[%d:%d], 0 offen offset:%d%s" % (r, r + 3, V_O, SRD_O, SRD_O + 3, h * 256, self.sched.get("store_policy", "")))
                vm.append(("st", slab))
                if self.lnp:
                    self.ln_producer_row(r, h, vm, slab)
                if it < 7:
                    e("v_add_u32 v%d, s%d, v%d" % (V_O, S_ROW4, V_O))
                    if self.lnp:
                        e("v_add_u32 v%d, s%d, v%d" % (V_O16, S_O16ROW4, V_O16))
                        e("v_add_u32 v%d, s%d, v%d" % (V_ST, S_STROW4, V_ST))
            if h == 0:
                e("v_subrev_u32 v%d, s%d, v%d" % (V_O, S_ROW28, V_O))
            else:
                e("v_add_u32 v%d, s%d, v%d" % (V_O, S_ROW4, V_O))
            if self.lnp:
                for vv, r28, r4 in ((V_O16, S_O16ROW28, S_O16ROW4), (V_ST, S_STROW28, S_STROW4)):
                    e(("v_subrev_u32 v%d, s%d, v%d" if h == 0 else "v_add_u32 v%d, s%d, v%d") % (vv, r28 if h == 0 else r4, vv))
            if slab in after_slab:
                self.resid_loads(after_slab[slab], vm, where[after_slab[slab]])

    def lnp_setup(self):
        e = self.e
        e("s_lshl_b32 s%d, s%d, 7" % (S_T2, S_WR))
        e("s_add_u32 s%d, s%d, s%d" % (S_T2, S_T2, S_T0))
        e("s_lshl_b32 s%d, s%d, 7" % (S_T3, S_WC))
        e("s_add_u32 s%d, s%d, s%d" % (S_T3, S_T3, S_T1))
        e("s_mul_i32 s%d, s%d, s%d" % (S_O16OFF, S_T2, S_LD16X2))
        e("s_lshl_b32 s%d, s%d, 1" % (S_T4, S_T3))
        e("s_add_u32 s%d, s%d, s%d" % (S_O16OFF, S_O16OFF, S_T4))
        e("s_mul_i32 s%d, s%d, s%d" % (S_STOFF, S_T2, S_PARTS8))
        e("s_lshr_b32 s%d, s%d, 6" % (S_T4, S_T3))
        e("s_lshl_b32 s%d, s%d, 3" % (S_T4, S_T4))
        e("s_add_u32 s%d, s%d, s%d" % (S_STOFF, S_STOFF, S_T4))
        e("v_bfe_u32 v%d, v0, 4, 2" % V_SQ)
        e("v_mul_lo_u32 v%d, v%d, s%d" % (V_ST, V_SQ, S_PARTS8))
        e("v_add_u32 v%d, s%d, v%d" % (V_ST, S_STOFF, V_ST))
        e("v_mul_lo_u32 v%d, v%d, s%d" % (V_O16, V_SQ, S_LD16X2))
        e("v_and_b32 v%d, 15, v0" % V_SQ)
        e("v_lshl_add_u32 v%d, v%d, 3, v%d" % (V_O16, V_SQ, V_O16))
        e("v_add_u32 v%d, s%d, v%d" % (V_O16, S_O16OFF, V_O16))

    def ln_producer_row(self, r, h, vm, slab):
        e = self.e
        abl = self.sched.get("lnp_ablate", "")
        if "valu" in abl:
            e("v_cvt_pk_f16_f32 v%d, v%d, v%d" % (V_SQ, r, r + 1))
            e("v_cvt_pk_f16_f32 v%d, v%d, v%d" % (V_SQ + 1, r + 2, r + 3))
        if "valu" not in abl:
            self.ln_producer_valu(r)
        if "st16" not in abl:
            e("buffer_store_dwordx2 v[%d:%d], v%d, s[%d:%d], 0 offen offset:%d%s" % (V_SQ, V_SQ + 1, V_O16, SRD_O16, SRD_O16 + 3, h * 128, self.sched.get("store16_policy", "")))
            vm.append(("st", slab))
        if "stst" not in abl:
            e("s_mov_b64 exec, s[%d:%d]" % (S_EXROW, S_EXROW + 1))
            e("buffer_store_dwordx2 v[%d:%d], v%d, s[%d:%d], 0 offen offset:%d" % (V_SUM, V_SUM + 1, V_ST, SRD_ST, SRD_ST + 3, h * 8))
            vm.append(("st", slab))
            e("s_mov_b64 exec, -1")

    def ln_producer_valu(self, r):
        e = self.e
        e("v_pk_add_f32 v[%d:%d], v[%d:%d], v[%d:%d]" % (V_SUM, V_SUM + 1, r, r + 1, r + 2, r + 3))
        e("v_pk_mul_f32 v[%d:%d], v[%d:%d], v[%d:%d]" % (V_SQ, V_SQ + 1, r, r + 1, r, r + 1))
        e("v_pk_fma_f32 v[%d:%d], v[%d:%d], v[%d:%d], v[%d:%d]" % (V_SQ, V_SQ + 1, r + 2, r + 3, r + 2, r + 3, V_SQ, V_SQ + 1))
        e("v_add_f32 v%d, v%d, v%d" % (V_SUM, V_SUM, V_SUM + 1))
        e("v_add_f32 v%d, v%d, v%d" % (V_SUM + 1, V_SQ, V_SQ + 1))
        dpp = ("quad_perm:[1,0,3,2]", "quad_perm:[2,3,0,1]", "row_half_mirror", "row_mirror")
        fill = ["v_cvt_pk_f16_f32 v%d, v%d, v%d" % (V_SQ, r, r + 1), "v_cvt_pk_f16_f32 v%d, v%d, v%d" % (V_SQ + 1, r + 2, r + 3), "s_nop 0", "s_nop 0"]
        e("s_nop 0")
        for st in range(4):
            e("v_add_f32_dpp v%d, v%d, v%d %s row_mask:0xf bank_mask:0xf" % (V_SUM, V_SUM, V_SUM, dpp[st]))
            e("v_add_f32_dpp v%d, v%d, v%d %s row_mask:0xf bank_mask:0xf" % (V_SUM + 1, V_SUM + 1, V_SUM + 1, dpp[st]))
            e(fill[st])

    def kernel(self):
        e, n = self.e, self.name
        esize = 4 if self.epi == EPI_F32 else 2
        self.L += kernel_begin(n)
        e("s_load_dwordx16 s[4:19], s[0:1], 0x0")
        e("s_load_dwordx8 s[20:27], s[0:1], 0x40")
        if self.sched.get("trace"):
            e("s_load_dwordx2 s[%d:%d], s[0:1], 0x60" % (S_TRP, S_TRP + 1))
            e("s_memtime s[%d:%d]" % (S_TS0, S_TS0 + 1))
            e("s_waitcnt lgkmcnt(0)")
            e("s_mov_b32 s3, s%d" % S_TS0)
            e("s_memrealtime s[%d:%d]" % (S_TS0, S_TS0 + 1))
            e("s_waitcnt lgkmcnt(0)")
            e("s_mov_b32 s27, s%d" % S_TS0)
            for r in (S_ACC_LOOP, S_ACC_EPI, S_NKT):
                e("s_mov_b32 s%d, 0" % r)
        e("v_and_b32 v%d, 63, v0" % V_LANE)
        e("v_lshrrev_b32 v%d, 6, v0" % V_T0)
        e("s_nop 1")
        e("v_readfirstlane_b32 s%d, v%d" % (S_WV, V_T0))
        e("v_and_b32 v%d, 31, v%d" % (V_LR, V_LANE))
        e("v_lshrrev_b32 v%d, 5, v%d" % (V_LG, V_LANE))
        e("s_waitcnt lgkmcnt(0)")
        e("s_lshr_b32 s%d, s%d, 1" % (S_WR, S_WV))
        e("s_and_b32 s%d, s%d, 1" % (S_WC, S_WV))
        e("s_lshl_b32 s%d, s%d, 15" % (S_FA, S_WR))
        e("s_lshl_b32 s%d, s%d, 15" % (S_FB, S_WC))
        e("s_add_u32 s%d, s%d, 0x10000" % (S_FB, S_FB))
        e("s_lshl_b32 s%d, s%d, 1" % (S_LDA2, S_LDA))
        e("s_lshl_b32 s%d, s%d, 1" % (S_LDW2, S_LDW))
        e("s_lshr_b32 s%d, s%d, 6" % (S_NK, S_K))
        if self.sk:
            lp, dn = self.u("L_skdiv"), self.u("L_skdiv_done")
            e("s_mov_b32 s%d, 0" % S_SKQ)
            e("s_mov_b32 s%d, s%d" % (S_SKREM, S_NK))
            self.lab(lp)
            e("s_cmp_lt_u32 s%d, s%d" % (S_SKREM, S_RMASK))
            e("s_cbranch_scc1 %s" % dn)
            e("s_sub_u32 s%d, s%d, s%d" % (S_SKREM, S_SKREM, S_RMASK))
            e("s_add_u32 s%d, s%d, 1" % (S_SKQ, S_SKQ))
            e("s_branch %s" % lp)
            self.lab(dn)
        e("s_lshl_b32 s%d, s%d, 10" % (S_M0BASE, S_WV))
        e("s_lshl_b32 s%d, s%d, 2" % (S_CUR, S_WG))
        e("s_lshl_b32 s%d, s%d, 2" % (S_STRIDE, S_G))
        e("s_load_dword s%d, s[%d:%d], s%d" % (S_TNEXT, S_TAB, S_TAB + 1, S_CUR))
        for srd in (SRD_A, SRD_B, SRD_O, SRD_R, SRD_BIAS, SRD_GAM):
            e("s_mov_b32 s%d, 0x00020000" % (srd + 3))
        e("s_mov_b32 s%d, s%d" % (SRD_O, S_OUT)); e("s_mov_b32 s%d, s%d" % (SRD_O + 1, S_OUT + 1))
        e("s_mul_i32 s%d, s%d, s%d" % (SRD_O + 2, S_M, S_LDO)); e("s_lshl_b32 s%d, s%d, %d" % (SRD_O + 2, SRD_O + 2, 1 if esize == 2 else 2))
        if self.sk:
            e("s_add_u32 s%d, s%d, 255" % (S_T0, S_M))
            e("s_andn2_b32 s%d, s%d, 255" % (S_T0, S_T0))
            e("s_mul_i32 s%d, s%d, s%d" % (SRD_O + 2, S_T0, S_LDO))
            e("s_lshl_b32 s%d, s%d, 2" % (SRD_O + 2, SRD_O + 2))
            e("s_mul_i32 s%d, s%d, s%d" % (SRD_O + 2, SRD_O + 2, S_RMASK))
        e("s_mov_b32 s%d, s%d" % (SRD_R, S_RES)); e("s_mov_b32 s%d, s%d" % (SRD_R + 1, S_RES + 1))
        if self.sched.get("trace") or self.epi != EPI_F32 or self.sk:
            e("s_mul_i32 s%d, s%d, s%d" % (SRD_R + 2, S_M, S_LDR)); e("s_lshl_b32 s%d, s%d, 2" % (SRD_R + 2, SRD_R + 2))
        else:
            e("s_add_u32 s%d, s%d, 1" % (S_T0, S_RMASK))
            e("s_cmp_eq_u32 s%d, -1" % S_RMASK)
            e("s_cselect_b32 s%d, s%d, s%d" % (S_T0, S_M, S_T0))
            e("s_mul_i32 s%d, s%d, s%d" % (SRD_R + 2, S_T0, S_LDR)); e("s_lshl_b32 s%d, s%d, 2" % (SRD_R + 2, SRD_R + 2))
        e("s_mov_b32 s%d, s%d" % (SRD_BIAS, S_BIAS)); e("s_mov_b32 s%d, s%d" % (SRD_BIAS + 1, S_BIAS + 1))
        e("s_lshl_b32 s%d, s%d, 2" % (SRD_BIAS + 2, S_N))
        e("s_mov_b32 s%d, s%d" % (SRD_GAM, S_GAM)); e("s_mov_b32 s%d, s%d" % (SRD_GAM + 1, S_GAM + 1))
        e("s_lshl_b32 s%d, s%d, 2" % (SRD_GAM + 2, S_N))
        for ptr, srd in ((S_BIAS, SRD_BIAS), (S_RES, SRD_R), (S_GAM, SRD_GAM)):
            e("s_or_b32 s%d, s%d, s%d" % (S_T0, ptr, ptr + 1))
            e("s_cmp_eq_u32 s%d, 0" % S_T0)
            e("s_cselect_b32 s%d, 0, s%d" % (srd + 2, srd + 2))
        e("v_lshrrev_b32 v%d, 1, v%d" % (V_T0, V_LR))
        e("v_and_b32 v%d, 7, v%d" % (V_T0, V_T0))
        e("v_lshlrev_b32 v%d, 7, v%d" % (V_T1, V_LR))
        for ks in range(4):
            e("v_or_b32 v%d, %d, v%d" % (V_T2, 2 * ks, V_LG))
            e("v_xor_b32 v%d, v%d, v%d" % (V_T2, V_T2, V_T0))
            e("v_lshl_add_u32 v%d, v%d, 4, v%d" % (V_T2, V_T2, V_T1))
            e("v_add_u32 v%d, s%d, v%d" % (V_FA + ks, S_FA, V_T2))
            e("v_add_u32 v%d, s%d, v%d" % (V_FB + ks, S_FB, V_T2))
        e("v_lshrrev_b32 v%d, 3, v%d" % (V_T0, V_LANE))
        e("s_lshl_b32 s%d, s%d, 3" % (S_T0, S_WV))
        e("v_add_u32 v%d, s%d, v%d" % (V_T0, S_T0, V_T0))
        e("v_lshrrev_b32 v%d, 1, v%d" % (V_T1, V_T0))
        e("v_and_b32 v%d, 7, v%d" % (V_T1, V_T1))
        e("v_and_b32 v%d, 7, v%d" % (V_T2, V_LANE))
        e("v_xor_b32 v%d, v%d, v%d" % (V_T1, V_T1, V_T2))
        e("v_lshlrev_b32 v%d, 4, v%d" % (V_T1, V_T1))
        for j in range(8):
            e("v_add_u32 v%d, %d, v%d" % (V_T2, j * 32, V_T0))
            e("v_mul_lo_u32 v%d, v%d, s%d" % (V_T3, V_T2, S_LDA2))
            e("v_add_u32 v%d, v%d, v%d" % (V_DA + j, V_T3, V_T1))
            e("v_mul_lo_u32 v%d, v%d, s%d" % (V_T3, V_T2, S_LDW2))
            e("v_add_u32 v%d, v%d, v%d" % (V_DB + j, V_T3, V_T1))
        e("s_lshl_b32 s%d, s%d, 13" % (S_T0, S_WV))
        e("s_add_u32 s%d, s%d, 0x%x" % (S_T0, S_T0, LDS_SLAB))
        e("v_and_b32 v%d, 15, v%d" % (V_T0, V_LR))
        e("v_lshlrev_b32 v%d, 8, v%d" % (V_T1, V_LR))
        e("v_add_u32 v%d, s%d, v%d" % (V_T1, S_T0, V_T1))
        if self.epi == EPI_F32:
            e("v_xor_b32 v%d, v%d, v%d" % (V_T0, V_T0, V_LG))
            for cq in range(8):
                e("v_xor_b32 v%d, %d, v%d" % (V_T2, (cq >> 2) * 8 + 2 * (cq & 3), V_T0))
                e("v_lshl_add_u32 v%d, v%d, 4, v%d" % (V_PARK + cq, V_T2, V_T1))
        else:
            e("v_lshl_add_u32 v%d, v%d, 3, v%d" % (V_T1, V_LG, V_T1))
            for cq in range(16):
                e("v_xor_b32 v%d, %d, v%d" % (V_T2, cq, V_T0))
                e("v_lshl_add_u32 v%d, v%d, 4, v%d" % (V_PARK + cq, V_T2, V_T1))
        e("v_lshrrev_b32 v%d, 4, v%d" % (V_T0, V_LANE))
        e("v_and_b32 v%d, 15, v%d" % (V_T1, V_LANE))
        for i in range(4):
            e("v_add_u32 v%d, %d, v%d" % (V_T2, 4 * i, V_T0))
            e("v_xor_b32 v%d, v%d, v%d" % (V_T3, V_T2, V_T1))
            e("v_and_b32 v%d, 15, v%d" % (V_T3, V_T3))
            e("v_lshlrev_b32 v%d, 4, v%d" % (V_T3, V_T3))
            e("v_lshl_add_u32 v%d, v%d, 8, v%d" % (V_T3, V_T2, V_T3))
            e("v_add_u32 v%d, s%d, v%d" % (V_EADDR + i, S_T0, V_T3))
        e("s_lshl_b32 s%d, s%d, 7" % (S_T1, S_WR))
        e("v_add_u32 v%d, s%d, v%d" % (V_T2, S_T1, V_T0))
        e("s_lshl_b32 s%d, s%d, 7" % (S_T2, S_WC))
        cols = 8 if esize == 2 else 4
        e("v_mul_lo_u32 v%d, v%d, s%d" % (V_T3, V_T2, S_LDO))
        e("v_mad_u32_u24 v%d, v%d, %d, v%d" % (V_T3, V_T1, cols, V_T3))
        e("v_add_u32 v%d, s%d, v%d" % (V_T3, S_T2, V_T3))
        e("v_lshlrev_b32 v%d, %d, v%d" % (V_OLANE, 1 if esize == 2 else 2, V_T3))
        e("s_lshl_b32 s%d, s%d, %d" % (S_ROW4, S_LDO, 3 if esize == 2 else 4))
        e("s_mul_i32 s%d, s%d, 7" % (S_ROW28, S_ROW4))
        if self.epi == EPI_F32:
            e("v_mul_lo_u32 v%d, v%d, s%d" % (V_T3, V_T2, S_LDR))
            e("v_mad_u32_u24 v%d, v%d, 4, v%d" % (V_T3, V_T1, V_T3))
            e("v_add_u32 v%d, s%d, v%d" % (V_T3, S_T2, V_T3))
            e("v_lshlrev_b32 v%d, 2, v%d" % (V_RLANE, V_T3))
            e("s_lshl_b32 s%d, s%d, 4" % (S_RROW4, S_LDR))
            e("s_mul_i32 s%d, s%d, 7" % (S_RROW28, S_RROW4))
            e("v_lshlrev_b32 v%d, 2, v%d" % (V_T3, V_T1))
            e("v_add_u32 v%d, s%d, v%d" % (V_T3, S_T2, V_T3))
            e("v_lshlrev_b32 v%d, 2, v%d" % (V_TMP + 11, V_T3))
        else:
            e("v_lshlrev_b32 v%d, 2, v%d" % (V_T3, V_LG))
            e("v_add_u32 v%d, s%d, v%d" % (V_T3, S_T2, V_T3))
            e("v_lshlrev_b32 v%d, 2, v%d" % (V_TMP + 11, V_T3))
        if self.epi == EPI_GELU_F16 and self.sched.get("gelu_mode", GELU_MODE) == "sigpoly":
            consts = [0xb658b1ce, 0xb658b1ce, 0x39bce2fa, 0x39bce2fa, 0xbdd78116, 0xbdd78116, 0xc01354b6, 0xc01354b6]
            for i, cst in enumerate(consts):
                e("s_mov_b32 s%d, 0x%08x" % (S_C + i, cst))
            e("v_mov_b32 v%d, 0x38b90ca2" % (V_TMP + 8))
            e("v_mov_b32 v%d, 0x38b90ca2" % (V_TMP + 9))
        elif self.epi == EPI_GELU_F16:
            consts = [0x3e6d3388, 0x3e6d3388, 0x3f87dc22, 0x3f87dc22, 0xbf38aa3b, 0xbf38aa3b, 0x3fb5f0e3, 0x3fb5f0e3,
                      0xbe91a98e, 0xbe91a98e, 0x3e827906, 0x3e827906, 0x7fffffff]
            for i, cst in enumerate(consts):
                e("s_mov_b32 s%d, 0x%08x" % (S_C + i, cst))
            e("v_mov_b32 v%d, 0xbfba00e3" % (V_TMP + 8))
            e("v_mov_b32 v%d, 0xbfba00e3" % (V_TMP + 9))
        if self.lnp:
            e("s_load_dwordx4 s[%d:%d], s[0:1], 0x68" % (SRD_O16, SRD_O16 + 3))
            e("s_load_dword s%d, s[0:1], 0x78" % S_LD16X2)
            e("s_waitcnt lgkmcnt(0)")
            e("s_mov_b32 s%d, s%d" % (SRD_ST, SRD_O16 + 2)); e("s_mov_b32 s%d, s%d" % (SRD_ST + 1, SRD_O16 + 3))
            e("s_lshl_b32 s%d, s%d, 1" % (S_LD16X2, S_LD16X2))
            e("s_mul_i32 s%d, s%d, s%d" % (SRD_O16 + 2, S_M, S_LD16X2)); e("s_mov_b32 s%d, 0x00020000" % (SRD_O16 + 3))
            e("s_lshr_b32 s%d, s%d, 6" % (S_PARTS8, S_N)); e("s_lshl_b32 s%d, s%d, 3" % (S_PARTS8, S_PARTS8))
            e("s_mul_i32 s%d, s%d, s%d" % (SRD_ST + 2, S_M, S_PARTS8)); e("s_mov_b32 s%d, 0x00020000" % (SRD_ST + 3))
            e("s_lshl_b32 s%d, s%d, 2" % (S_O16ROW4, S_LD16X2)); e("s_mul_i32 s%d, s%d, 7" % (S_O16ROW28, S_O16ROW4))
            e("s_lshl_b32 s%d, s%d, 2" % (S_STROW4, S_PARTS8)); e("s_mul_i32 s%d, s%d, 7" % (S_STROW28, S_STROW4))
            e("s_mov_b32 s%d, 0x00010001" % S_EXROW); e("s_mov_b32 s%d, 0x00010001" % (S_EXROW + 1))
        if self.lnc:
            e("s_mov_b32 s%d, s%d" % (SRD_MR, S_RES)); e("s_mov_b32 s%d, s%d" % (SRD_MR + 1, S_RES + 1))
            e("s_lshl_b32 s%d, s%d, 3" % (SRD_MR + 2, S_M)); e("s_mov_b32 s%d, 0x00020000" % (SRD_MR + 3))
            e("s_add_u32 s%d, s%d, s%d" % (SRD_MF, S_RES, SRD_MR + 2)); e("s_addc_u32 s%d, s%d, 0" % (SRD_MF + 1, S_RES + 1))
            e("s_lshl_b32 s%d, s%d, 4" % (SRD_MF + 2, S_M)); e("s_mov_b32 s%d, 0x00020000" % (SRD_MF + 3))
            e("s_mov_b32 s%d, s%d" % (SRD_SF, S_GAM)); e("s_mov_b32 s%d, s%d" % (SRD_SF + 1, S_GAM + 1))
            e("s_lshl_b32 s%d, s%d, 4" % (SRD_SF + 2, S_N)); e("s_mov_b32 s%d, 0x00020000" % (SRD_SF + 3))
            e("v_lshlrev_b32 v%d, 4, v%d" % (V_T0, V_LR))
            e("s_lshl_b32 s%d, s%d, 11" % (S_T0, S_WC))
            e("s_lshl_b32 s%d, s%d, 11" % (S_T1, S_WR))
            e("v_add_u32 v%d, s%d, v%d" % (V_T1, S_T0, V_T0))
            e("v_add_u32 v%d, s%d, v%d" % (V_T2, S_T1, V_T0))
            e("v_mov_b32 v%d, 0x40000000" % V_T3)
            e("v_cmp_eq_u32 vcc, 1, v%d" % V_LG)
            e("v_cndmask_b32 v%d, v%d, v%d, vcc" % (V_T1, V_T1, V_T3))
            e("v_cndmask_b32 v%d, v%d, v%d, vcc" % (V_T2, V_T2, V_T3))
            e("v_lshlrev_b32 v%d, 3, v%d" % (V_T0, V_LR))
            e("s_lshl_b32 s%d, s%d, 10" % (S_T1, S_WR))
            e("s_add_u32 s%d, s%d, 4" % (S_T1, S_T1))
            e("v_add_u32 v%d, s%d, v%d" % (V_RSOFF, S_T1, V_T0))
            e("v_mov_b32 v%d, v%d" % (V_SFOFF, V_T1))
            e("v_mov_b32 v%d, v%d" % (V_MFOFF, V_T2))
        e("s_waitcnt lgkmcnt(0)")
        e("s_cmp_eq_u32 s%d, -1" % S_TNEXT)
        e("s_cbranch_scc1 L_exit_%s" % n)
        if self.sched.get("stagger"):
            groups, units = self.sched["stagger"]
            lp, done = self.u("L_stag"), self.u("L_stag_done")
            if self.sched.get("stagger_by") == "xcd":
                assert groups == 2
                e("s_bfe_u32 s%d, s%d, 0x10002" % (S_T0, S_WG))
            else:
                e("s_lshr_b32 s%d, s%d, 3" % (S_T0, S_WG))
                e("s_and_b32 s%d, s%d, %d" % (S_T0, S_T0, groups - 1))
            e("s_mul_i32 s%d, s%d, %d" % (S_T0, S_T0, units))
            self.lab(lp)
            e("s_cmp_eq_u32 s%d, 0" % S_T0)
            e("s_cbranch_scc1 %s" % done)
            e("s_sleep 127")
            e("s_sub_u32 s%d, s%d, 1" % (S_T0, S_T0))
            e("s_branch %s" % lp)
            self.lab(done)
        self.switch_tile()
        for kt in range(2):
            for p in range(16):
                e(self.dma_m0(p))
                e("s_nop 0")
                e(self.dma_issue(p))
            for ins in self.dma_advance():
                e(ins)
            e("s_xor_b32 s%d, s%d, 0x%x" % (S_M0BASE, S_M0BASE, LDS_BUF))
        e("s_mov_b32 s%d, s%d" % (S_TCUR, S_TDMA))
        if self.sk:
            self.item_ktiles(S_TCUR, S_KREM)
        else:
            e("s_mov_b32 s%d, s%d" % (S_KREM, S_NK))
        e("s_waitcnt vmcnt(16)")
        e("s_barrier")
        for i in range(16):
            e(self.frag_read(i // 8, i // 8, i % 8))
        for r in (V_FA, V_FA + 1, V_FB, V_FB + 1):
            e("v_xor_b32 v%d, 0x%x, v%d" % (r, LDS_BUF, r))
        slots = self.build_slots()
        self.lab("L_tile_begin_%s" % n)
        if self.sched.get("trace"):
            e("s_memtime s[%d:%d]" % (S_TS0, S_TS0 + 1))
        self.ktile(slots, True)
        self.L.append(".p2align 4")
        self.lab("L_loop_%s" % n)
        e("s_waitcnt lgkmcnt(8)")
        for s in range(16):
            e(self.mfma(0, s // 4, s % 4, False))
            for ins in slots[s]:
                e(ins)
        self.lab("L_after_ks0_%s" % n)
        for s in range(16, 64):
            ks, rb, cb = s // 16, (s % 16) // 4, s % 4
            if s == 16:
                e("s_waitcnt lgkmcnt(15)")
            e(self.mfma(ks, rb, cb, False))
            for ins in slots[s]:
                if ins.endswith(":"):
                    self.lab(ins[:-1])
                else:
                    e(ins)
        for r in (V_FA, V_FA + 1, V_FB, V_FB + 1):
            e("v_xor_b32 v%d, 0x%x, v%d" % (r, LDS_BUF, r))
        e("s_sub_u32 s%d, s%d, 1" % (S_KREM, S_KREM))
        e("s_cmp_eq_u32 s%d, 0" % S_KREM)
        e("s_cbranch_scc0 L_loop_%s" % n)
        if self.sched.get("trace"):
            e("s_memtime s[%d:%d]" % (S_TS1, S_TS1 + 1))
            e("s_waitcnt lgkmcnt(0)")
            e("s_sub_u32 s%d, s%d, s%d" % (S_T0, S_TS1, S_TS0))
            e("s_add_u32 s%d, s%d, s%d" % (S_ACC_LOOP, S_ACC_LOOP, S_T0))
            e("s_add_u32 s%d, s%d, s%d" % (S_NKT, S_NKT, S_NK))
        n_dma_after = 0 if self.sched.get("no_dma") else sum(1 for p in range(16) if self.sched["dma"][p] > self.sched.get("pre_slot", 17))
        if self.sched.get("no_epilogue"):
            pass
        else:
            pre_lines = self.L
            self.L = []
            vm = self.pre_epilogue()
            self.pre_code = self.L
            self.L = pre_lines
            n_late = 0 if self.sched.get("no_dma") else sum(1 for p in range(16) if self.sched["dma"][p] > 48)
            vm += [("dma", 0)] * (n_dma_after - n_late)
            if self.lnc:
                pre_lines = self.L
                self.L = []
                vm += self.pre2_epilogue()
                self.pre2_code = self.L
                self.L = pre_lines
            vm += [("dma", 0)] * n_late
            if self.epi == EPI_F32:
                self.epilogue_f32(vm)
            else:
                self.epilogue_f16(self.epi == EPI_GELU_F16, vm)
        if self.sched.get("trace"):
            e("s_memtime s[%d:%d]" % (S_TS0, S_TS0 + 1))
            e("s_waitcnt lgkmcnt(0)")
            e("s_sub_u32 s%d, s%d, s%d" % (S_T0, S_TS0, S_TS1))
            e("s_add_u32 s%d, s%d, s%d" % (S_ACC_EPI, S_ACC_EPI, S_T0))
        e("s_mov_b32 s%d, s%d" % (S_TCUR, S_TDMA))
        if self.sk:
            self.item_ktiles(S_TCUR, S_KREM)
        else:
            e("s_mov_b32 s%d, s%d" % (S_KREM, S_NK))
        e("s_cmp_eq_u32 s%d, -1" % S_TCUR)
        e("s_cbranch_scc0 L_tile_begin_%s" % n)
        self.lab("L_exit_%s" % n)
        e("s_waitcnt vmcnt(0) lgkmcnt(0)")
        if self.sched.get("trace"):
            done = self.u("L_trace_done")
            e("s_cmp_eq_u32 s%d, 0" % S_WV)
            e("s_cbranch_scc0 %s" % done)
            e("s_lshl_b32 s%d, s%d, 4" % (S_T0, S_WG))
            e("v_mov_b32 v%d, s%d" % (V_T0, S_T0))
            e("v_mov_b32 v%d, s%d" % (V_EM[0], S_ACC_LOOP))
            e("v_mov_b32 v%d, s%d" % (V_EM[0] + 1, S_ACC_EPI))
            e("v_mov_b32 v%d, s%d" % (V_EM[0] + 2, S_NKT))
            e("s_memtime s[%d:%d]" % (S_TS0, S_TS0 + 1))
            e("s_waitcnt lgkmcnt(0)")
            e("s_sub_u32 s3, s%d, s3" % S_TS0)
            e("v_mov_b32 v%d, s3" % (V_EM[0] + 3))
            e("global_store_dwordx4 v%d, v[%d:%d], s[%d:%d]" % (V_T0, V_EM[0], V_EM[0] + 3, S_TRP, S_TRP + 1))
            e("s_memrealtime s[%d:%d]" % (S_TS0, S_TS0 + 1))
            e("s_waitcnt lgkmcnt(0)")
            e("s_sub_u32 s27, s%d, s27" % S_TS0)
            e("s_lshl_b32 s%d, s%d, 4" % (S_T0, S_G))
            e("v_add_u32 v%d, s%d, v%d" % (V_T0, S_T0, V_T0))
            e("v_mov_b32 v%d, s27" % V_EM[0])
            e("global_store_dwordx4 v%d, v[%d:%d], s[%d:%d]" % (V_T0, V_EM[0], V_EM[0] + 3, S_TRP, S_TRP + 1))
            e("s_waitcnt vmcnt(0)")
            self.lab(done)
        e("s_endpgm")
        self.lab("L_switch_%s" % n)
        self.switch_tile()
        e("s_branch L_switch_ret_%s" % n)
        if not self.sched.get("no_epilogue"):
            self.lab("L_pre_%s" % n)
            self.L += self.pre_code
            e("s_branch L_pre_ret_%s" % n)
            if self.lnc:
                self.lab("L_pre2_%s" % n)
                self.L += self.pre2_code
                e("s_branch L_pre2_ret_%s" % n)
        self.L += kernel_end(n, 163840, 128 if self.lnp else 104, NUM_SGPR)

    def metadata(self):
        args = ["ptr"] * 7 + ["i32"] * 10 + ["ptr"] + (["ptr"] * 2 + ["i32"] * 2 if self.lnp else [])
        return kernel_metadata(self.name, args, 163840, NUM_SGPR)


def default_sched():
    return {
        "rd23": list(range(16)),
        "tog23": 16,
        "barA": 19,
        "dma": [21 + (5 * p) // 2 for p in range(16)],
        "barB": 46,
        "rd01": [47 + i for i in range(16)],
        "resid_policy": " nt",
        "store_policy": " nt",
    }


def experiment_scheds():
    out = []
    b = default_sched()
    out.append(dict(b, trace=True))
    out.append(dict(b, trace=True, no_epilogue=True))
    out.append(dict(b, trace=True, no_epilogue=True, no_dma=True))
    out.append(dict(b, trace=True, no_epilogue=True, no_dma=True, no_reads=True))
    out.append(dict(b, trace=True, no_epilogue=True, no_dma=True, no_reads=True, no_barrier=True))
    out.append(dict(b, trace=True, no_epilogue=True, no_reads=True))
    out.append(dict(b, trace=True, dma=[21 + p for p in range(16)], barB=46))
    out.append(dict(b, trace=True, dma=[21 + 2 * p for p in range(16)], barB=46))
    out.append(dict(b, trace=True, rd23=[i // 2 for i in range(16)], barA=17, dma=[19 + (3 * p) // 2 for p in range(16)]))
    out.append(dict(b, trace=True, prio=1))
    out.append(dict(b, trace=True))
    out.append(dict(b, trace=True, gelu_mode="notrans"))
    out.append(dict(b, trace=True, gelu_mode="none"))
    out.append(dict(b, trace=True, dma=[21 + (5 * p) // 2 for p in range(16)]))
    out.append(dict(b, trace=True, dma=[21 + (11 * p) // 4 for p in range(16)]))
    out.append(dict(b, trace=True, resid_policy=""))
    out.append(dict(b, trace=True, store_policy=""))
    out.append(dict(b, trace=True, store_policy=" sc0 sc1"))
    out.append(dict(b, trace=True, store_policy=" sc0 sc1 nt", resid_policy=" sc0 sc1 nt"))
    out.append(dict(b, resid_policy=""))
    out.append(dict(b, store_policy=""))
    out.append(dict(b, trace=True, store_policy=""))
    out.append(dict(b, store_policy=" sc1"))
    out.append(dict(b, store_policy=" sc0 sc1"))
    out.append(dict(b, trace=True, deep_ring=True))
    out.append(dict(b, stagger=(2, 2)))
    out.append(dict(b, stagger=(4, 1)))
    out.append(dict(b, stagger=(2, 1)))
    out.append(dict(b, stagger=(4, 2)))
    out.append(dict(b, stagger=(8, 1)))
    out.append(dict(b, trace=True, pre_slot=47))
    out.append(dict(b, pre_slot=47))
    out.append(dict(b, resid_policy=" sc1"))
    out.append(dict(b, resid_policy=" sc0 sc1"))
    out.append(dict(b, resid_policy=" sc1 nt"))
    out.append(dict(b, gelu_mode="none"))
    out.append(dict(b, gelu_mode="notrans"))
    for u in (2, 3, 4, 5, 6):
        out.append(dict(b, stagger=(2, u), stagger_by="xcd"))
    return out


def variants():
    base = default_sched()
    out = [("psam_gemm_asm_f16", EPI_F16, base), ("psam_gemm_asm_gelu", EPI_GELU_F16, base), ("psam_gemm_asm_f32", EPI_F32, base)]
    keep = dict(base, resid_policy="", store_policy="")
    out += [("psam_gemm_asm_f16_l2", EPI_F16, keep), ("psam_gemm_asm_gelu_l2", EPI_GELU_F16, keep), ("psam_gemm_asm_f32_l2", EPI_F32, keep)]
    out += [("psam_gemm_asm_f32_sk", EPI_F32, dict(keep, splitk=True))]
    ln = dict(base, ln_cons=True, ln_prod=True, store16_policy=" nt")
    out += [("psam_gemm_asm_f16_ln", EPI_F16, ln), ("psam_gemm_asm_gelu_ln", EPI_GELU_F16, ln), ("psam_gemm_asm_f32_ln", EPI_F32, ln)]
    if "--experiments" in sys.argv:
        for i, sc in enumerate(experiment_scheds()):
            for nm, epi in (("f16", EPI_F16), ("gelu", EPI_GELU_F16), ("f32", EPI_F32)):
                out.append(("psam_gemm_asm_%s_v%d" % (nm, i + 1), epi, sc))
    return out


def main():
    import gemm_asm2_gen
    l2, meta2, es = gemm_asm2_gen.build_all()
    if "--meta" in sys.argv:
        out = ["// generated by gemm_asm_gen.py --meta: a half-tile's epilogue is spread over E K-tile iterations of the next one"]
        for nm in ("f16", "gelu", "f32"):
            out.append("#define PSAM_ASM2_E_%s %d" % (nm.upper(), es["psam_gemm_asm2_" + nm]))
        sys.stdout.write("\n".join(out) + "\n")
        return
    ks = variants()
    lines = []
    meta = []
    for name, epi, sc in ks:
        g = Gen(name, epi, sc)
        g.kernel()
        lines += g.L
        meta.append(g.metadata())
    lines += l2
    meta += meta2
    import gattn_asm_gen
    l3, meta3 = gattn_asm_gen.build_all()
    lines += l3
    meta += meta3
    import wattn_asm_gen
    l4, meta4 = wattn_asm_gen.build_all()
    lines += l4
    meta += meta4
    sys.stdout.write(module_text(lines, meta))


if __name__ == "__main__":
    main()
```

protosam_amd/ops.py:

```python
import torch

from . import _lib

EPI_F16, EPI_GELU_F16, EPI_F32, EPI_RELU_F16 = 0, 1, 2, 3


_raw_stream = getattr(torch._C, "_cuda_getCurrentRawStream", None)
_raw_device = getattr(torch._C, "_cuda_getDevice", None)


def _stream():
    if _raw_stream is not None and _raw_device is not None:
        return _raw_stream(_raw_device())
    return torch.cuda.current_stream().cuda_stream


class KernelTimer:

    def __init__(self):
        self.records = []
        self.tags = {}

    def start(self):
        e = torch.cuda.Event(enable_timing=True)
        e.record()
        return e

    def stop(self, e0, work, tag=None):
        e1 = torch.cuda.Event(enable_timing=True)
        e1.record()
        self.records.append((e0, e1, work))
        if tag is not None:
            self.tags[len(self.records) - 1] = tag

    def by_tag(self):
        out = {}
        for i, tag in self.tags.items():
            a, b, w = self.records[i]
            n, t, f = out.get(tag, (0, 0.0, 0.0))
            out[tag] = (n + 1, t + a.elapsed_time(b) * 1e-3, f + float(w[0] if isinstance(w, tuple) else w))
        return out

    def summary(self):
        t = sum(a.elapsed_time(b) for a, b, _ in self.records) * 1e-3
        return len(self.records), t, float(sum((w[0] if isinstance(w, tuple) else w) for _, _, w in self.records))

    def summary2(self):
        return float(sum(w[1] for _, _, w in self.records if isinstance(w, tuple)))


GEMM_TIMER = None
TIMERS = {}


def _tstart(name):
    t = TIMERS.get(name)
    return None if t is None else (t, t.start())


def _tstop(h, work):
    if h is not None:
        h[0].stop(h[1], work)

import os as _os
QKV_HEAD_MAJOR = _os.environ.get("PSAM_QKV_HEAD_MAJOR", "0") != "0"
FUSE_WINDOW_RELPOS = _os.environ.get("PSAM_FUSE_WINDOW_RELPOS", "1") != "0"
FUSE_GLOBAL_RELPOS = _os.environ.get("PSAM_FUSE_GLOBAL_RELPOS", "1") != "0"


def _ptr(t):
    return 0 if t is None else t.data_ptr()


def _req(t, dtype, name):
    if t is None:
        return
    if not t.is_cuda:
        raise RuntimeError(f"{name}: expected a device tensor (protosam_amd has no CPU path)")
    if t.dtype != dtype:
        raise TypeError(f"{name}: expected {dtype}, got {t.dtype}")
    if t.stride(-1) != 1:
        raise ValueError(f"{name}: innermost dimension must be contiguous")


def _req_aligned(t, nbytes, name):
    if t is not None and t.data_ptr() % nbytes:
        raise ValueError(f"{name}: data pointer must be {nbytes}-byte aligned (got a view at offset {t.data_ptr() % nbytes})")


def gemm(a, w, bias=None, out=None, epilogue=EPI_F16, resid=None, gamma=None, resid_mod=0, out_seg=0,
         out_seg_stride=0, out_seg_off=0, M=None, out16=None, stats=None, ln_mr=None, ln_s=None):
    _req(a, torch.float16, "a"); _req(w, torch.float16, "w")
    _req(bias, torch.float32, "bias"); _req(gamma, torch.float32, "gamma")
    _req(resid, torch.float16 if epilogue == EPI_RELU_F16 else torch.float32, "resid")
    a2 = a.reshape(-1, a.shape[-1]) if a.dim() != 2 else a
    if M is None:
        M = a2.shape[0]
    K = a2.shape[1]
    N = w.shape[0]
    assert w.shape[1] == K, (w.shape, K)
    odt = torch.float32 if epilogue == EPI_F32 else torch.float16
    if out is None:
        out = torch.empty((M, N), dtype=odt, device=a.device)
    _req(out, odt, "out")
    out2 = out.reshape(-1, out.shape[-1]) if out.dim() != 2 else out
    ldr = 0
    if resid is not None:
        r2 = resid.reshape(-1, resid.shape[-1]) if resid.dim() != 2 else resid
        ldr = r2.stride(0)
    fold = out16 is not None or stats is not None or ln_mr is not None
    if fold:
        _req(out16, torch.float16, "out16"); _req(stats, torch.float32, "stats")
        _req(ln_mr, torch.float32, "ln_mr"); _req(ln_s, torch.float32, "ln_s")
        if ln_mr is not None:
            assert ln_s is not None and ln_mr.numel() >= 6 * M and ln_s.numel() >= 5 * N, (ln_mr.numel(), 6 * M, ln_s.numel(), 5 * N)
        if stats is not None:
            assert stats.numel() >= M * (N // 64) * 2 and N % 64 == 0
        if out16 is not None:
            assert out16.shape[-1] >= N and out16.numel() >= M * N
    if epilogue == EPI_F32 and a.device.index not in _GEMM_WS:
        _ensure_gemm_workspace(a.device)
    t0 = GEMM_TIMER.start() if GEMM_TIMER is not None else None
    if fold:
        st = _lib.lib().psam_gemm_f16_ln(_ptr(a2), _ptr(w), _ptr(bias), _ptr(out2), _ptr(resid), _ptr(gamma), M, N, K,
                                        a2.stride(0), w.stride(0), out2.stride(0), ldr, resid_mod, out_seg,
                                        out_seg_stride, out_seg_off, epilogue, _ptr(out16),
                                        0 if out16 is None else out16.stride(-2), _ptr(stats), _ptr(ln_mr), _ptr(ln_s),
                                        _stream())
    else:
        st = _lib.lib().psam_gemm_f16(_ptr(a2), _ptr(w), _ptr(bias), _ptr(out2), _ptr(resid), _ptr(gamma), M, N, K,
                                     a2.stride(0), w.stride(0), out2.stride(0), ldr, resid_mod, out_seg,
                                     out_seg_stride, out_seg_off, epilogue, _stream())
    if t0 is not None:
        GEMM_TIMER.stop(t0, 2.0 * M * N * K, tag=(M, N, K, epilogue, 1 if fold else 0))
    _lib.check(st, "psam_gemm_f16_ln" if fold else "psam_gemm_f16")
    return out


_SPLITK = {}


def gemm_splitk_ranges(M, N, K):
    if _os.environ.get("PSAM_GEMM_SPLITK_ASM", "1") == "0":
        return 0
    key = (M, N, K, torch.cuda.current_device(), DISPATCH_EPOCH)
    if key not in _SPLITK:
        _SPLITK[key] = int(_lib.lib().psam_gemm_splitk_ranges(M, N, K))
    return _SPLITK[key]


def splitk_rows(M):
    return (M + 255) // 256 * 256


def gemm_splitk_ln(a, w, bias, x, ks, ws, ln_w=None, ln_b=None, eps=1e-6, out16=None):
    _req(a, torch.float16, "a"); _req(w, torch.float16, "w"); _req(bias, torch.float32, "bias"); _req(x, torch.float32, "x")
    _req(ws, torch.float32, "ws"); _req(ln_w, torch.float32, "ln_w"); _req(ln_b, torch.float32, "ln_b"); _req(out16, torch.float16, "out16")
    M, K = a.shape
    N = w.shape[0]
    assert x.shape == (M, N) and w.shape[1] == K and ws.is_contiguous() and ws.numel() >= ks * splitk_rows(M) * N
    assert out16 is None or (out16.shape[0] >= M and out16.shape[-1] >= N)
    t0 = GEMM_TIMER.start() if GEMM_TIMER is not None else None
    st = _lib.lib().psam_gemm_f16_splitk_ln(_ptr(a), _ptr(w), _ptr(bias), _ptr(x), M, N, K, a.stride(0), w.stride(0), x.stride(0), ks,
                                           _ptr(ws), _ptr(ln_w), _ptr(ln_b), float(eps), _ptr(out16),
                                           0 if out16 is None else out16.stride(-2), _stream())
    if t0 is not None:
        GEMM_TIMER.stop(t0, 2.0 * M * N * K, tag=(M, N, K, EPI_F32, 0))
    _lib.check(st, "psam_gemm_f16_splitk_ln")
    return x


_CU_COUNT = {}


def fold_pays(M, D, device, min_fill=0.8):
    idx = device.index if device.index is not None else torch.cuda.current_device()
    if idx not in _CU_COUNT:
        _CU_COUNT[idx] = torch.cuda.get_device_properties(idx).multi_processor_count
    return ((M + 255) // 256) * (D // 256) >= min_fill * _CU_COUNT[idx]


def ln_mr_buffer(M, device):
    return torch.empty(6 * M, dtype=torch.float32, device=device)


def ln_finalize(stats, M, D, eps, mr=None):
    _req(stats, torch.float32, "stats")
    if mr is None:
        mr = ln_mr_buffer(M, stats.device)
    _req(mr, torch.float32, "mr")
    assert mr.numel() >= 6 * M and mr.is_contiguous()
    st = _lib.lib().psam_ln_finalize(_ptr(stats), M, D, float(eps), _ptr(mr), _stream())
    _lib.check(st, "psam_ln_finalize")
    return mr


def fold_layernorm(weight, bias, ln_weight, ln_bias):
    W = weight.detach().float()
    Wp = (W * ln_weight.detach().float()[None, :]).half().contiguous()
    s = Wp.float().sum(1).contiguous()
    b = bias.detach().float() if bias is not None else torch.zeros(W.shape[0], dtype=torch.float32, device=W.device)
    hi = s.half()
    frag = torch.zeros((s.numel(), 8), dtype=torch.float16, device=s.device)
    frag[:, 0], frag[:, 1], frag[:, 2] = hi, (s - hi.float()).half(), hi
    s_ext = torch.cat([s, frag.reshape(-1).view(torch.float32)]).contiguous()
    return Wp, s_ext, (b + W @ ln_bias.detach().float()).contiguous()


def gemm_heads(a, w, bias, hd, out=None, M=None):
    _req(a, torch.float16, "a"); _req(w, torch.float16, "w"); _req(bias, torch.float32, "bias")
    a2 = a.reshape(-1, a.shape[-1]) if a.dim() != 2 else a
    if M is None:
        M = a2.shape[0]
    K, N = a2.shape[1], w.shape[0]
    assert w.shape[1] == K and N % hd == 0
    if out is None:
        out = torch.empty((N // hd, M, hd), dtype=torch.float16, device=a.device)
    _req(out, torch.float16, "out")
    assert out.is_contiguous() and out.numel() == M * N
    t0 = GEMM_TIMER.start() if GEMM_TIMER is not None else None
    st = _lib.lib().psam_gemm_f16_heads(_ptr(a2), _ptr(w), _ptr(bias), _ptr(out), M, N, K, a2.stride(0), w.stride(0), hd,
                                       _stream())
    if t0 is not None:
        GEMM_TIMER.stop(t0, 2.0 * M * N * K)
    _lib.check(st, "psam_gemm_f16_heads")
    return out


_GEMM_WS = {}
GEMM_WORKSPACE_MB = int(_os.environ.get("PSAM_GEMM_WORKSPACE_MB", "64"))


def _ensure_gemm_workspace(device):
    idx = device.index if device.index is not None else torch.cuda.current_device()
    if idx not in _GEMM_WS:
        n = GEMM_WORKSPACE_MB << 20
        with torch.cuda.device(idx):
            buf = torch.empty(max(n, 16), dtype=torch.uint8, device=torch.device("cuda", idx))
            _lib.check(_lib.lib().psam_gemm_set_workspace(buf.data_ptr() if n else 0, n), "psam_gemm_set_workspace")
        _GEMM_WS[idx] = buf
        _GEMM_WS[None] = buf


DISPATCH_EPOCH = 0


def _bump_dispatch():
    global DISPATCH_EPOCH
    DISPATCH_EPOCH += 1


def dispatch_key():
    return (DISPATCH_EPOCH, QKV_HEAD_MAJOR, FUSE_WINDOW_RELPOS, FUSE_GLOBAL_RELPOS)


def gemm_set_tile(tile):
    _bump_dispatch()
    _lib.check(_lib.lib().psam_gemm_set_tile(int(tile)), "psam_gemm_set_tile")


def gemm_set_option(name, value):
    _bump_dispatch()
    _lib.check(_lib.lib().psam_gemm_set_option(name.encode(), int(value)), "psam_gemm_set_option")


def gemm_asm_variant(v):
    _bump_dispatch()
    _lib.check(_lib.lib().psam_gemm_asm_variant(int(v)), "psam_gemm_asm_variant")


def im2col(x, B, H, W, C, kh, kw, stride, dil, pad, ldo=None, out=None):
    _req(x, torch.float16, "x")
    assert x.is_contiguous()
    Ho = (H + 2 * pad - dil * (kh - 1) - 1) // stride + 1 if stride > 0 else 0
    Wo = (W + 2 * pad - dil * (kw - 1) - 1) // stride + 1 if stride > 0 else 0
    if ldo is None:
        ldo = kh * kw * C
    if out is None:
        if min(B, H, W, C, kh, kw, stride, dil) <= 0 or pad < 0 or Ho <= 0 or Wo <= 0:
            raise ValueError(f"im2col: no output for B={B} {H}x{W}x{C}, kernel {kh}x{kw} stride {stride} dil {dil} pad {pad}")
        out = torch.empty((B * Ho * Wo, ldo), dtype=torch.float16, device=x.device)
    st = _lib.lib().psam_im2col(_ptr(x), B, H, W, C, kh, kw, stride, dil, pad, ldo, _ptr(out), _stream())
    _lib.check(st, "psam_im2col")
    return out, Ho, Wo


def im2col_stem(img, ldo=192, out=None):
    _req(img, torch.float32, "img")
    assert img.is_contiguous() and img.shape[1] == 3
    B, _, H, W = img.shape
    Ho, Wo = (H - 1) // 2 + 1, (W - 1) // 2 + 1
    if out is None:
        out = torch.empty((B * Ho * Wo, ldo), dtype=torch.float16, device=img.device)
    st = _lib.lib().psam_im2col_stem(_ptr(img), B, H, W, ldo, _ptr(out), _stream())
    _lib.check(st, "psam_im2col_stem")
    return out, Ho, Wo


def maxpool3x3s2(x, B, H, W, C, out=None):
    _req(x, torch.float16, "x")
    assert x.is_contiguous()
    Ho, Wo = (H - 1) // 2 + 1, (W - 1) // 2 + 1
    if out is None:
        if min(B, H, W, C) <= 0:
            raise ValueError(f"maxpool3x3s2: no output for B={B} {H}x{W}x{C}")
        out = torch.empty((B * Ho * Wo, C), dtype=torch.float16, device=x.device)
    st = _lib.lib().psam_maxpool3x3s2(_ptr(x), B, H, W, C, _ptr(out), _stream())
    _lib.check(st, "psam_maxpool3x3s2")
    return out, Ho, Wo


def rotate_nearest(img, xg, yg, rt, crop_y, crop_x, out_h, out_w, out=None):
    _req(img, torch.float32, "img"); _req(xg, torch.float32, "xg"); _req(yg, torch.float32, "yg")
    assert img.is_contiguous() and rt.dtype == torch.float32 and rt.device.type == "cpu" and rt.is_contiguous()
    B, C, H, W = img.shape
    if out is None:
        out = torch.empty((B, C, out_h, out_w), dtype=torch.float32, device=img.device)
    _req(out, torch.float32, "out")
    assert out.is_contiguous() and out.numel() >= B * C * max(out_h, 0) * max(out_w, 0)
    st = _lib.lib().psam_rotate_nearest(_ptr(img), _ptr(out), _ptr(xg), _ptr(yg), rt.data_ptr(), B * C, H, W, crop_y, crop_x,
                                        out_h, out_w, _stream())
    _lib.check(st, "psam_rotate_nearest")
    return out


def resize_aa(img, oh, ow, out=None):
    _req(img, torch.float32, "img")
    assert img.is_contiguous()
    B, C, H, W = img.shape
    tmp = torch.empty((B * C, H, max(ow, 0)), dtype=torch.float32, device=img.device)
    if out is None:
        out = torch.empty((B, C, oh, ow), dtype=torch.float32, device=img.device)
    _req(out, torch.float32, "out")
    assert out.is_contiguous() and out.numel() >= B * C * max(oh, 0) * max(ow, 0)
    st = _lib.lib().psam_resize_aa(_ptr(img), _ptr(tmp), _ptr(out), B * C, H, W, oh, ow, _stream())
    _lib.check(st, "psam_resize_aa")
    return out


def layernorm(x, weight, bias, eps, out=None, out_dtype=torch.float16, out2=None, zero_tail_rows=0, M=None):
    _req(x, torch.float32, "x"); _req(weight, torch.float32, "weight"); _req(bias, torch.float32, "bias")
    x2 = x.reshape(-1, x.shape[-1]) if x.dim() != 2 else x
    if M is None:
        M = x2.shape[0]
    D = x2.shape[1]
    if out is None:
        out = torch.empty((M + zero_tail_rows, D), dtype=out_dtype, device=x.device)
    o2 = out.reshape(-1, out.shape[-1]) if out.dim() != 2 else out
    h = _tstart("layernorm")
    st = _lib.lib().psam_layernorm(_ptr(x2), _ptr(weight), _ptr(bias), _ptr(o2), _ptr(out2), M, D, x2.stride(0),
                                  o2.stride(0), float(eps), 0 if out.dtype == torch.float16 else 1,
                                  zero_tail_rows, _stream())
    _tstop(h, M * D * (4 + out.element_size()) + 8 * D)
    _lib.check(st, "psam_layernorm")
    return out


def attention(qkv, B, N, H, hd, scale, out=None, mode=0, rel_h=None, rel_w=None, relq=None, pad_row=None, gh=0, gw=0,
              ws=0, head_major=False, rpack=None):
    _req(qkv, torch.float16, "qkv"); _req(rel_h, torch.float32, "rel_h"); _req(rel_w, torch.float32, "rel_w")
    _req(pad_row, torch.float16, "pad_row"); _req(relq, torch.float16, "relq"); _req(rpack, torch.float16, "rpack")
    assert qkv.is_contiguous()
    if out is None:
        out = torch.empty((B, N, H * hd), dtype=torch.float16, device=qkv.device)
    h = _tstart("attention_window" if mode == 2 else "attention_global")
    st = _lib.lib().psam_attention_f16(_ptr(qkv), _ptr(out), _ptr(rel_h), _ptr(rel_w), _ptr(relq), _ptr(rpack), _ptr(pad_row), B, N,
                                      H, hd, float(scale), mode, gh, gw, ws, 1 if head_major else 0, _stream())
    nk = ws * ws if mode == 2 else N
    _tstop(h, (B * N * 4 * H * hd * 2 + (2 * B * H * N * 64 * 4 if (mode == 1 and rel_h is not None) else 0),
               4.0 * B * H * N * nk * hd))
    _lib.check(st, "psam_attention_f16")
    return out


_FUSED_RELPOS = {}


def attention_fused_relpos(B, N, H, hd, gh, gw):
    if not FUSE_GLOBAL_RELPOS or QKV_HEAD_MAJOR:
        return False
    key = (B, N, H, hd, gh, gw, DISPATCH_EPOCH)
    if key not in _FUSED_RELPOS:
        _FUSED_RELPOS[key] = bool(_lib.lib().psam_attention_fused_relpos(B, N, H, hd, gh, gw))
    return _FUSED_RELPOS[key]


def attention_set_variant(v):
    _bump_dispatch()
    _lib.check(_lib.lib().psam_attention_set_variant(int(v)), "psam_attention_set_variant")


def pack_rel_tables(rel_pos_h, rel_pos_w, windowed, hd):
    RP = 32 if windowed else 128
    HDP = (hd + 31) // 32 * 32
    out = torch.zeros((2, 2, RP, HDP), dtype=torch.float16, device=rel_pos_h.device)
    for t, R in enumerate((rel_pos_h, rel_pos_w)):
        R = R.detach().float()
        assert R.shape[0] <= RP and R.shape[1] == hd
        hi = R.half()
        lo = (R - hi.float()).half()
        out[t, 0, :R.shape[0], :hd] = hi
        out[t, 1, :R.shape[0], :hd] = lo
    if not windowed:
        return out.contiguous()
    return torch.cat([out.reshape(-1), _window_onehot_table().to(out.device), out.new_zeros(128)]).contiguous()


_ONEHOT = None


def _window_onehot_table(ws=14):
    global _ONEHOT
    if _ONEHOT is None:
        T = torch.arange(13).view(13, 1, 1)
        lane = torch.arange(64).view(1, 64, 1)
        e = torch.arange(8).view(1, 1, 8)
        li, g = lane & 15, lane >> 4
        key = (T >> 1) * 32 + (li >> 2) * 8 + (T & 1) * 4 + (li & 3)
        slot = g * 8 + e
        hot = ((slot == key // ws) | (slot == ws + key % ws)) & (key < ws * ws)
        _ONEHOT = hot.to(torch.float16).reshape(-1)
    return _ONEHOT


def relpos(qkv, rpack, B, N, H, hd, gw, K, windowed, scale, rel_h=None, rel_w=None, relq=None, head_major=False):
    _req(qkv, torch.float16, "qkv"); _req(rpack, torch.float16, "rpack")
    assert rpack.is_contiguous()
    if windowed:
        if relq is None:
            relq = torch.zeros((B, H, N, 2, 32), dtype=torch.float16, device=qkv.device)
    else:
        if rel_h is None:
            rel_h = torch.empty((B, H, N, 64), dtype=torch.float32, device=qkv.device)
        if rel_w is None:
            rel_w = torch.empty((B, H, N, 64), dtype=torch.float32, device=qkv.device)
    st = _lib.lib().psam_relpos(_ptr(qkv), _ptr(rpack), _ptr(rel_h), _ptr(rel_w), _ptr(relq), B, N, H, hd, gw, K,
                               1 if windowed else 0, float(scale), 1 if head_major else 0, _stream())
    _lib.check(st, "psam_relpos")
    return relq if windowed else (rel_h, rel_w)


META_NBG, META_NFG, META_FGMODE, META_NCELL_FG = 0, 1, 2, 3


class AlpBank:

    def __init__(self, ncell, C, device):
        self.cap = ncell + 1
        self.C = C
        self.bank = torch.zeros((2 * self.cap, C), dtype=torch.float32, device=device)
        self.meta = torch.zeros(8, dtype=torch.int32, device=device)
        self.slot_bg = torch.empty(ncell, dtype=torch.int32, device=device)
        self.slot_fg = torch.empty(ncell, dtype=torch.int32, device=device)
        self.mres = None


def alp_bank(sup, ld, h, w, C, mask, pool_w, kernel_size, thresh=0.95, eps=1e-4, bank=None, force_mode=-1, bmask=None):
    _req(sup, torch.float32, "sup"); _req(mask, torch.float32, "mask")
    assert mask.dim() == 2 and mask.is_contiguous()
    ncell = (h // pool_w) * (w // pool_w)
    if bank is None:
        bank = AlpBank(ncell, C, sup.device)
    if bank.mres is None or bank.mres.numel() != 2 * h * w:
        bank.mres = torch.empty(2 * h * w, dtype=torch.float32, device=sup.device)
    if bmask is not None:
        _req(bmask, torch.float32, "bmask")
        assert bmask.shape == mask.shape and bmask.is_contiguous()
    st = _lib.lib().psam_alp_bank(_ptr(sup), ld, h, w, C, _ptr(mask), _ptr(bmask), mask.shape[0], mask.shape[1], pool_w,
                                 kernel_size,
                                 float(thresh), float(eps), _ptr(bank.bank), bank.cap, _ptr(bank.meta),
                                 _ptr(bank.slot_bg), _ptr(bank.slot_fg), _ptr(bank.mres), force_mode, _stream())
    _lib.check(st, "psam_alp_bank")
    return bank


def alp_sim(qry, q_bstride, ld, B, npix, C, bank, pred=None, part=None, eps=1e-4, sim_scale=20.0, which_only=-1):
    _req(qry, torch.float32, "qry")
    npt = (bank.cap + 63) // 64
    npix_pad = (npix + 63) // 64 * 64
    if part is None:
        part = torch.empty(2 * B * npt * npix_pad * 3, dtype=torch.float32, device=qry.device)
    if pred is None:
        pred = torch.empty((B, 2, npix), dtype=torch.float32, device=qry.device)
    h = _tstart("alp_sim")
    st = _lib.lib().psam_alp_sim(_ptr(qry), q_bstride, ld, B, npix, C, _ptr(bank.bank), bank.cap, _ptr(bank.meta),
                                float(eps), float(sim_scale), _ptr(part), _ptr(pred), which_only, _stream())
    _tstop(h, (B * npix * C * 4 + 2 * bank.cap * C * 4 + B * 2 * npix * 4, 2.0 * B * npix * C * 2 * bank.cap))
    _lib.check(st, "psam_alp_sim")
    return pred


def plan_alp_pairs(class_runs, B):
    entries = []
    for c, runs in enumerate(class_runs):
        if sum(n for _, _, n in runs) != B or any(n < 0 for _, _, n in runs):
            raise ValueError(f"class {c}: the run counts {[n for _, _, n in runs]} do not sum to the {B} query slices")
        b0 = 0
        for bg, fgs, n in runs:
            if not fgs:
                raise ValueError(f"class {c}: a run without a foreground bank")
            for b in range(b0, b0 + n):
                plane = (c * B + b) * 2
                entries.append((bg, b, 0, plane))
                entries.extend((f, b, 1, plane + 1) for f in fgs)
            b0 += n
    return entries, 2 * B * len(class_runs)


def alp_sim_pairs(qry, q_bstride, ld, B, npix, C, banks, entries, n_planes, pred=None, part=None, eps=1e-4, sim_scale=20.0):
    _req(qry, torch.float32, "qry")
    if not entries:
        raise ValueError("alp_sim_pairs: no entries")
    count = {}
    last = None
    for i, (k, b, which, plane) in enumerate(entries):
        if not (0 <= k < len(banks) and 0 <= b < B and which in (0, 1) and 0 <= plane < n_planes):
            raise ValueError(f"alp_sim_pairs: entry {i} {(k, b, which, plane)} is out of range")
        if plane != last and plane in count:
            raise ValueError(f"alp_sim_pairs: the entries of plane {plane} are not adjacent")
        count[plane] = count.get(plane, 0) + 1
        last = plane
    for bk in banks:
        if bk.C != C or bk.bank.device != qry.device:
            raise ValueError("alp_sim_pairs: every bank must have the query's channel count and device")
    rows, ngmax, direct = [], 1, True
    for k, b, which, plane in entries:
        bk = banks[k]
        ng = (bk.cap + 95) // 96
        ngmax = max(ngmax, ng)
        d = count[plane] == 1 and ng == 1
        direct = direct and d
        rows.append([bk.bank.data_ptr(), bk.meta.data_ptr(), bk.cap | (b << 32), (which | (2 if d else 0)) | (plane << 32)])
    npix_pad = (npix + 63) // 64 * 64
    if part is None and not direct:
        part = torch.empty(len(entries) * ngmax * npix_pad * 3, dtype=torch.float32, device=qry.device)
    assert part is None or part.numel() >= len(entries) * ngmax * npix_pad * 3
    if pred is None:
        pred = torch.empty((n_planes, npix), dtype=torch.float32, device=qry.device)
    _req(pred, torch.float32, "pred")
    assert pred.is_contiguous() and pred.numel() >= n_planes * npix
    tab = torch.tensor(rows, dtype=torch.int64).pin_memory().to(qry.device, non_blocking=True)
    h = _tstart("alp_sim")
    st = _lib.lib().psam_alp_sim_pairs(_ptr(qry), q_bstride, ld, npix, C, _ptr(tab), len(entries), ngmax, float(eps), float(sim_scale),
                                       _ptr(part), _ptr(pred), _stream())
    _tstop(h, (B * npix * C * 4 + sum(2 * bk.cap * C * 4 for bk in banks) + n_planes * npix * 4,
               sum(2.0 * npix * C * banks[k].cap for k, _, _, _ in entries)))
    _lib.check(st, "psam_alp_sim_pairs")
    return pred


def patchify_bilinear(img, S, P, Kpad, out=None):
    _req(img, torch.float32, "img")
    assert img.is_contiguous() and img.dim() == 4
    B, C, H, W = img.shape
    if out is None:
        out = torch.empty((B * (S // P) ** 2, Kpad), dtype=torch.float16, device=img.device)
    st = _lib.lib().psam_patchify_bilinear(_ptr(img), B, C, H, W, S, P, Kpad, _ptr(out), _stream())
    _lib.check(st, "psam_patchify_bilinear")
    return out


# ... 752 lines not shown
```

Before: 160.4.

## Add 16x16x32 MFMA variant of asm GEMM with auto-selection for large outputs

Generates a new family of hand-scheduled assembly GEMM kernels that use v_mfma_f32_16x16x32_f16 instead of the 32x32 MFMA, with their own LDS fragment reads, K-loop slot schedule, epilogues, and folded-LayerNorm path. The dispatcher picks this family (tile 17) by default when K is large, the tile count fills the CUs and the output exceeds 48 MB, and otherwise falls back to the existing asm path. The aim is higher MFMA throughput or better issue scheduling on big GEMMs. The cost is a large amount of new hand-scheduled code, along with the risk of register-layout or epilogue errors. It also adds a last-tile query for introspection.

```diff
diff --git a/include/protosam_hip.h b/include/protosam_hip.h
--- a/include/protosam_hip.h
+++ b/include/protosam_hip.h
@@ -22,6 +22,7 @@
                             int ks, float* ws, const float* ln_w, const float* ln_b, float eps, void* out16, int ld16, void* stream);
 
 int psam_gemm_set_tile(int tile);
+int psam_gemm_last_tile(int* tile);
 int psam_gemm_asm_variant(int variant);
 int psam_gemm_set_option(const char* name, int value);
 int psam_gemm_set_workspace(void* ptr, size_t bytes);
diff --git a/protosam_amd/_lib.py b/protosam_amd/_lib.py
--- a/protosam_amd/_lib.py
+++ b/protosam_amd/_lib.py
@@ -17,6 +17,7 @@
     "psam_gemm_f16_splitk_ln": [c_void_p, c_void_p, c_void_p, c_void_p] + [c_int] * 7 + [c_void_p, c_void_p, c_void_p, c_float, c_void_p, c_int,
                                 c_void_p],
     "psam_gemm_set_tile": [c_int],
+    "psam_gemm_last_tile": [ctypes.POINTER(c_int)],
     "psam_gemm_asm_variant": [c_int],
     "psam_gemm_set_option": [ctypes.c_char_p, c_int],
     "psam_gemm_set_workspace": [c_void_p, c_size_t],
diff --git a/protosam_amd/csrc/gemm.hip b/protosam_amd/csrc/gemm.hip
--- a/protosam_amd/csrc/gemm.hip
+++ b/protosam_amd/csrc/gemm.hip
@@ -1184,8 +1184,10 @@
   auto it = m->fns.find(key);
   if (it != m->fns.end()) return it->second.data();
   const char* names[3] = {"f16", "gelu", "f32"};
-  const char* suffix[3] = {"", "_l2", "_ln"};
-  const int nf = (family == 1 && g_asm_variant == 0) ? 9 : 3;
+  const char* suffix1[3] = {"", "_l2", "_ln"};
+  const char* suffix3[3] = {"_m16", "_m16", "_ln_m16"};
+  const char* const* suffix = family == 3 ? suffix3 : suffix1;
+  const int nf = (family != 2 && g_asm_variant == 0) ? 9 : 3;
   std::vector<hipFunction_t> f(9, nullptr);
   for (int i = 0; i < nf; ++i) {
     std::string n = std::string(family == 2 ? "psam_gemm_asm2_" : "psam_gemm_asm_") + names[i % 3] + suffix[i / 3] +
@@ -1245,9 +1247,10 @@
   }
   return &(g_asm_tabs[key] = t);
 }
-static bool asm_eligible(const GemmArgs& p, int epilogue, int lnf) {
+static bool asm_eligible(const GemmArgs& p, int epilogue, int lnf, int family = 1) {
+  if (family == 3 && !asm_load(3)) return false;
   if (lnf) {
-    const hipFunction_t* f = asm_load(1);
+    const hipFunction_t* f = asm_load(family);
     const bool cons = p.ln_mr || p.ln_s, prod = p.out16 || p.stats;
     if (!f || g_asm_variant != 0 || (cons && prod)) return false;
     if (cons && (!f[6 + epilogue] || !p.ln_mr || !p.ln_s || !p.bias || (reinterpret_cast<uintptr_t>(p.ln_mr) & 15) || (reinterpret_cast<uintptr_t>(p.ln_s) & 15))) return false;
@@ -1281,16 +1284,16 @@
 static int launch_asm(const GemmArgs& p, int epilogue, hipStream_t s, int family = 1) {
   const hipFunction_t* fns = asm_load(family);
   if (!fns) return PSAM_ERR_LAUNCH;
-  const int ntm = (p.M + 255) / 256, ntn = family >= 2 ? p.N / 128 : p.N / 256;
+  const int ntm = (p.M + 255) / 256, ntn = family == 2 ? p.N / 128 : p.N / 256;
   const AsmTable* t = asm_table(ntm, ntn, pick_map_mode(ntm, ntn));
   if (!t) return PSAM_ERR_LAUNCH;
   AsmGemmArgs a;
   a.A = p.A; a.W = p.W; a.bias = p.bias; a.out = p.out; a.resid = p.resid; a.gamma = p.gamma; a.tab = t->dev;
   a.M = p.M; a.N = p.N; a.K = p.K; a.lda = p.lda; a.ldw = p.ldw; a.ldo = p.ldo; a.ldr = p.resid ? p.ldr : 0; a.G = t->grid;
   a.flags = p.gamma ? 1 : 0;
-  a.pad = (family == 1 && p.resid_mod > 0) ? p.resid_mod - 1 : -1;
+  a.pad = (family != 2 && p.resid_mod > 0) ? p.resid_mod - 1 : -1;
   a.trace = nullptr;
-  const bool ln_cons = family == 1 && p.ln_mr && p.ln_s, ln_prod = family == 1 && (p.out16 || p.stats);
+  const bool ln_cons = family != 2 && p.ln_mr && p.ln_s, ln_prod = family != 2 && (p.out16 || p.stats);
   if (ln_cons) {
     a.resid = p.ln_mr;
     a.gamma = p.ln_s + p.N;
@@ -1317,7 +1320,7 @@
     for (int b = 0; b < t->grid; ++b) rt += h[(size_t)t->grid * 4 + b * 4];
     for (int b = 0; b < t->grid; ++b) { loop += h[b * 4]; epi += h[b * 4 + 1]; kt += h[b * 4 + 2]; tot += h[b * 4 + 3]; tmax = h[b * 4 + 3] > tmax ? h[b * 4 + 3] : tmax; }
     const double tiles = kt / (p.K / 64);
-    if (kt > 0) fprintf(stderr, "asm v%d %dx%dx%d epi%d: %.0f cycles per K-tile, %.0f cycles per epilogue (%.1f tiles per workgroup) kernel entry to exit: mean %.0f max %u cycles = %.1f us (shader clock %.0f MHz)\n", g_asm_variant, p.M, p.N,
+    if (kt > 0) fprintf(stderr, "asm%s v%d %dx%dx%d epi%d: %.0f cycles per K-tile, %.0f cycles per epilogue (%.1f tiles per workgroup) kernel entry to exit: mean %.0f max %u cycles = %.1f us (shader clock %.0f MHz)\n", family == 3 ? " m16" : "", g_asm_variant, p.M, p.N,
                         p.K, epilogue, loop / kt, epi / tiles, tiles / t->grid, tot / t->grid, tmax, rt / t->grid * 0.01, rt > 0 ? tot / rt * 100.0 : 0.0);
   }
   return PSAM_OK;
@@ -1464,24 +1467,36 @@
   return psam_launch_status();
 }
 
-enum { OPT_ASM = 0, OPT_HALF, OPT_SPLITK, OPT_NSPLIT, OPT_DEEP, OPT_SMALL, OPT_COUNT };
-static const char* const g_opt_names[OPT_COUNT] = {"asm", "half_tiles", "splitk", "nsplit", "deep", "small"};
-static const char* const g_opt_env[OPT_COUNT] = {"PSAM_GEMM_ASM", "PSAM_GEMM_HALF", "PSAM_GEMM_SPLITK", "PSAM_GEMM_NSPLIT", "PSAM_GEMM_DEEP", "PSAM_GEMM_SMALL"};
-static int g_opt[OPT_COUNT] = {-1, -1, -1, -1, -1, -1};
+enum { OPT_ASM = 0, OPT_HALF, OPT_SPLITK, OPT_NSPLIT, OPT_DEEP, OPT_SMALL, OPT_MFMA16, OPT_COUNT };
+static const char* const g_opt_names[OPT_COUNT] = {"asm", "half_tiles", "splitk", "nsplit", "deep", "small", "mfma16"};
+static const char* const g_opt_env[OPT_COUNT] = {"PSAM_GEMM_ASM", "PSAM_GEMM_HALF", "PSAM_GEMM_SPLITK", "PSAM_GEMM_NSPLIT", "PSAM_GEMM_DEEP", "PSAM_GEMM_SMALL",
+                                                 "PSAM_GEMM_MFMA16"};
+static int g_opt[OPT_COUNT] = {-1, -1, -1, -1, -1, -1, -1};
 static int gemm_option(int i) {
-  if (g_opt[i] < 0) { const char* e = getenv(g_opt_env[i]); g_opt[i] = e ? (atoi(e) != 0) : 1; }
+  if (g_opt[i] < 0) { const char* e = getenv(g_opt_env[i]); g_opt[i] = (e && atoi(e) >= 0) ? (atoi(e) != 0) : (i == OPT_MFMA16 ? 2 : 1); }
   return g_opt[i];
 }
 extern "C" int psam_gemm_set_option(const char* name, int value) {
   if (name && strcmp(name, "max_wgs") == 0) { g_max_wgs = value > 0 ? value : 0; return PSAM_OK; }
   for (int i = 0; i < OPT_COUNT; ++i)
-    if (name && strcmp(name, g_opt_names[i]) == 0) { g_opt[i] = value != 0; return PSAM_OK; }
+    if (name && strcmp(name, g_opt_names[i]) == 0) { g_opt[i] = (i == OPT_MFMA16 && value < 0) ? 2 : value != 0; return PSAM_OK; }
   return PSAM_ERR_ARG;
+}
+static int g_last_tile = 0;
+extern "C" int psam_gemm_last_tile(int* tile) {
+  if (!tile) return PSAM_ERR_ARG;
+  *tile = g_last_tile;
+  return PSAM_OK;
 }
 static int g_tile_override = -1;
 extern "C" int psam_gemm_set_tile(int t) {
   g_tile_override = t;
   return PSAM_OK;
+}
+static bool mfma16_auto(int M, int N, int K, int epilogue) {
+  const long t256 = (long)((M + 255) / 256) * (N / 256), ncu = eff_cus();
+  const size_t out_bytes = (size_t)M * N * (epilogue == EPI_F32 ? 4 : 2);
+  return K >= 768 && t256 * 10 >= ncu * 19 && out_bytes > ((size_t)48 << 20);
 }
 static int pick_tile(int M, int N, int K, int epilogue) {
   if (g_tile_override < 0) {
@@ -1496,7 +1511,9 @@
     const bool short_f32 = epilogue == EPI_F32 && K < 2048;
     const int fill = short_f32 ? 95 : (epilogue == EPI_F32 || rounds > 1) ? 80 : 50;
     if (K >= 768 && t256 * 100 >= rounds * ncu * fill) {
-      return gemm_option(OPT_ASM) ? 15 : 11;
+      if (!gemm_option(OPT_ASM)) return 11;
+      const int m16 = gemm_option(OPT_MFMA16);
+      return (m16 == 1 || (m16 == 2 && mfma16_auto(M, N, K, epilogue))) ? 17 : 15;
     }
   }
   if (N % 128 == 0 && K >= 768) {
@@ -1559,7 +1576,8 @@
   p.wide16 = (ldo % 8) == 0 && (reinterpret_cast<uintptr_t>(out) & 15) == 0 && (!head_hd || head_hd % 8 == 0);
   if (tsel == 16 && !asm2_eligible(p, epilogue, ln_prod || ln_cons)) tsel = (g_tile_override > 0 || ln_prod || ln_cons) ? 15 : 1;
   if (tsel == 15 && !asm_eligible(p, epilogue, ln_prod || ln_cons)) tsel = (N % 256 == 0) ? 11 : 1;
-  if (tsel != 1 && tsel != 11 && tsel != 12 && tsel != 13 && tsel != 15 && tsel != 16) tsel = (N % 256 == 0) ? 11 : 1;
+  if (tsel == 17 && !asm_eligible(p, epilogue, ln_prod || ln_cons, 3)) tsel = (N % 256 == 0) ? 11 : 1;
+  if (tsel != 1 && tsel != 11 && tsel != 12 && tsel != 13 && tsel != 15 && tsel != 16 && tsel != 17) tsel = (N % 256 == 0) ? 11 : 1;
   if (tsel == 11 && (N % 256) != 0) tsel = 1;
   if (tsel == 11 && epilogue != EPI_F32 && !p.wide16) tsel = 1;
   if (ln_cons && !p.wide16) return PSAM_ERR_ARG;
@@ -1573,8 +1591,10 @@
       if (seen[key]++ == 0) fprintf(stderr, "psam_gemm_f16: %s\n", key);
     }
   }
+  g_last_tile = tsel;
   if (tsel == 15) return launch_asm(p, epilogue, s);
   if (tsel == 16) return launch_asm(p, epilogue, s, 2);
+  if (tsel == 17) return launch_asm(p, epilogue, s, 3);
   p.ksplit = 1;
   p.ks_ws = nullptr;
   {
diff --git a/protosam_amd/csrc/gemm_asm_gen.py b/protosam_amd/csrc/gemm_asm_gen.py
--- a/protosam_amd/csrc/gemm_asm_gen.py
+++ b/protosam_amd/csrc/gemm_asm_gen.py
@@ -64,6 +64,8 @@
         self.lnp = bool(sched.get("ln_prod")) and epi == EPI_F32
         self.sk = bool(sched.get("splitk")) and epi == EPI_F32 and not self.lnp
         assert not (self.sk and sched.get("trace"))
+        self.m16 = sched.get("mfma", "32x32x16") == "16x16x32"
+        assert not (self.m16 and (self.sk or sched.get("deep_ring") or sched.get("stagger")))
 
     def item_rows_cols(self, item):
         e = self.e
@@ -143,6 +145,74 @@
         j = idx - 4
         return "ds_read_b128 v[%d:%d], v%d offset:%d" % (V_SET[st] + 16 + 4 * j, V_SET[st] + 16 + 4 * j + 3, V_FB + ks, j * 4096)
 
+    RD16_ORDER = tuple(range(8, 16)) + tuple(range(8))
+    M16_FA, M16_FB = (1, 2), (3, 8)
+
+    def frag_read16(self, ks, idx):
+        base = V_SET[2 * ks]
+        if idx < 8:
+            return "ds_read_b128 v[%d:%d], v%d offset:%d" % (base + 4 * idx, base + 4 * idx + 3, self.M16_FA[ks], idx * 2048)
+        j = idx - 8
+        return "ds_read_b128 v[%d:%d], v%d offset:%d" % (base + 32 + 4 * j, base + 32 + 4 * j + 3, self.M16_FB[ks], j * 2048)
+
+    def mfma16(self, ks, rb, cb, zero):
+        blk, base = (rb * 8 + cb) * 4, V_SET[2 * ks]
+        a = "v[%d:%d]" % (base + 32 + 4 * cb, base + 32 + 4 * cb + 3)
+        b = "v[%d:%d]" % (base + 4 * rb, base + 4 * rb + 3)
+        cc = "0" if zero else "a[%d:%d]" % (blk, blk + 3)
+        return "v_mfma_f32_16x16x32_f16 a[%d:%d], %s, %s, %s" % (blk, blk + 3, a, b, cc)
+
+    def build_slots16(self, zero_copy=False):
+        sc = self.sched
+        z = "_z" if zero_copy else ""
+        slots = [[] for _ in range(128)]
+        def put(s, ins):
+            assert not slots[s], (s, ins, slots[s])
+            slots[s].append(ins)
+        for i, idx in enumerate(self.RD16_ORDER):
+            if not sc.get("no_reads"):
+                put(sc["rd1"][i], self.frag_read16(1, idx))
+        for i, r in enumerate((self.M16_FA[1], self.M16_FB[1])):
+            put(sc["tog1"][i], "v_xor_b32 v%d, 0x%x, v%d" % (r, LDS_BUF, r))
+        if not sc.get("no_epilogue") and not zero_copy:
+            put(sc["pre_slot"], "s_cmp_eq_u32 s%d, 1" % S_KREM)
+            slots[sc["pre_slot"] + 1] += ["s_cbranch_scc1 L_pre_%s" % self.name, "L_pre_ret_%s:" % self.name]
+        a = sc["barA"]
+        if not sc.get("no_barrier"):
+            slots[a] += ["s_waitcnt lgkmcnt(0)", "s_barrier"]
+        put(a + 1, "s_cmp_eq_u32 s%d, 0" % S_DKREM)
+        slots[a + 2] += ["s_cbranch_scc1 L_switch%s_%s" % (z, self.name), "L_switch_ret%s_%s:" % (z, self.name)]
+        for p in range(16):
+            s = sc["dma"][p]
+            assert p == 0 or s - sc["dma"][p - 1] >= 3
+            if sc.get("no_dma"):
+                continue
+            put(s - 1, self.dma_m0(p))
+            put(s, self.dma_issue(p))
+        b = sc["barB"]
+        issued = sum(1 for p in range(16) if sc["dma"][p] <= b)
+        if not sc.get("no_barrier"):
+            assert not slots[b]
+            slots[b] += ["s_waitcnt vmcnt(%d)" % (0 if sc.get("no_dma") else issued), "s_barrier"]
+        for i, idx in enumerate(self.RD16_ORDER):
+            assert sc["rd0"][i] > b
+            if not sc.get("no_reads"):
+                put(sc["rd0"][i], self.frag_read16(0, idx))
+        for i, ins in enumerate(self.dma_advance()):
+            assert sc["adv"] + i > sc["dma"][15]
+            put(sc["adv"] + i, ins)
+        return slots
+
+    def lgkm_waits16(self):
+        sc = self.sched
+        out = {}
+        for rb in range(8):
+            s = 8 * rb
+            if s > sc["barA"]:
+                break
+            out[s] = min(15, (7 - rb) + sum(1 for x in sc["rd1"] if x < s))
+        return out
+
     def mfma(self, st, rb, cb, zero):
         blk = (rb * 4 + cb) * 16
         a = "v[%d:%d]" % (V_SET[st] + 16 + 4 * cb, V_SET[st] + 16 + 4 * cb + 3)
@@ -319,6 +389,11 @@
                 vm += [("bg", 0), ("bg", 0)]
             self.resid_loads(0, vm)
             self.resid_loads(1, vm)
+        elif self.m16:
+            for cb in range(8):
+                r = self.F16_BIAS + cb * 4
+                e("buffer_load_dwordx4 v[%d:%d], v%d, s[%d:%d], s%d offen offset:%d" % (r, r + 3, V_TMP + 11, SRD_BIAS, SRD_BIAS + 3, S_N0X4, cb * 64))
+                vm.append(("bias", 0))
         else:
             for cb in range(4):
                 for q in range(4):
@@ -335,6 +410,17 @@
         e("s_lshl_b32 s%d, s%d, 12" % (S_T2, S_T1))
         e("s_lshl_b32 s%d, s%d, 12" % (S_T3, S_T0))
         e("s_lshl_b32 s%d, s%d, 11" % (S_T4, S_T0))
+        if self.m16:
+            for cb in range(8):
+                e("buffer_load_dwordx2 v[%d:%d], v%d, s[%d:%d], s%d offen offset:%d" % (self.M16_SF + 2 * cb, self.M16_SF + 2 * cb + 1, V_SFOFF, SRD_SF, SRD_SF + 3, S_T2, cb * 256))
+                vm.append(("sf", 0))
+            for rb in range(8):
+                e("buffer_load_dwordx2 v[%d:%d], v%d, s[%d:%d], s%d offen offset:%d" % (self.M16_MF + 2 * rb, self.M16_MF + 2 * rb + 1, V_MFOFF, SRD_MF, SRD_MF + 3, S_T3, rb * 256))
+                vm.append(("mf", 0))
+            for rb in range(8):
+                e("buffer_load_dword v%d, v%d, s[%d:%d], s%d offen offset:%d" % (self.M16_RSTD[rb >> 1] + (rb & 1), V_RSOFF, SRD_MR, SRD_MR + 3, S_T4, rb * 128))
+                vm.append(("rs", 0))
+            return vm
         for cb in range(4):
             e("buffer_load_dwordx4 v[%d:%d], v%d, s[%d:%d], s%d offen offset:%d" % (96 + 4 * cb, 99 + 4 * cb, V_SFOFF, SRD_SF, SRD_SF + 3, S_T2, cb * 512))
             vm.append(("sf", 0))
@@ -346,10 +432,64 @@
             vm.append(("rs", 0))
         return vm
 
+    M16_SF, M16_MF = 212, 228
+    M16_RSTD = (28, 30, 4, 6)
+
     def younger(self, vm, tag):
         return younger(vm, tag)
 
+    def epilogue_f16_m16(self, gelu, vm):
+        e = self.e
+        self.c("---- epilogue (16x16x32 accumulators): bias (+ GELU) -> fp16, through the wave's slab so that 16 lanes store one 256-byte row piece")
+        e("s_nop 7")
+        e("s_nop 7")
+        self.tile_offsets(2)
+        e("v_add_u32 v%d, s%d, v%d" % (V_O, S_TOFF, V_OLANE))
+        e("s_waitcnt vmcnt(%d)" % self.younger(vm, ("bias", 0)))
+        if self.lnc:
+            self.c("folded LayerNorm: acc -= mean_row * s_col, one rank-1 MFMA per 16x16 block (fp16 hi / lo operands: fp32-accurate)")
+            e("s_waitcnt vmcnt(%d)" % self.younger(vm, ("rs", 0)))
+            for rb in range(8):
+                for cb in range(8):
+                    blk = (rb * 8 + cb) * 4
+                    e("v_mfma_f32_16x16x16_f16 a[%d:%d], v[%d:%d], v[%d:%d], a[%d:%d]" % (blk, blk + 3, self.M16_SF + 2 * cb, self.M16_SF + 2 * cb + 1,
+                                                                                      self.M16_MF + 2 * rb, self.M16_MF + 2 * rb + 1, blk, blk + 3))
+            e("s_nop 7")
+            e("s_nop 7")
+            e("s_nop 3")
+        for rb32 in range(4):
+            em = self.F16_EM[rb32 & 1]
+            for sub in range(2):
+                rb = 2 * rb32 + sub
+                for cb in range(8):
+                    blk = (rb * 8 + cb) * 4
+                    t = V_TMP
+                    for i in range(4):
+                        e("v_accvgpr_read_b32 v%d, a%d" % (t + i, blk + i))
+                    b = self.F16_BIAS + cb * 4
+                    if self.lnc:
+                        rp, hs = self.M16_RSTD[rb >> 1], rb & 1
+                        for hh in range(2):
+                            e("v_pk_fma_f32 v[%d:%d], v[%d:%d], v[%d:%d], v[%d:%d] op_sel:[0,%d,0] op_sel_hi:[1,%d,1]" % (
+                                t + 2 * hh, t + 2 * hh + 1, t + 2 * hh, t + 2 * hh + 1, rp, rp + 1, b + 2 * hh, b + 2 * hh + 1, hs, hs))
+                    else:
+                        e("v_pk_add_f32 v[%d:%d], v[%d:%d], v[%d:%d]" % (t, t + 1, t, t + 1, b, b + 1))
+                        e("v_pk_add_f32 v[%d:%d], v[%d:%d], v[%d:%d]" % (t + 2, t + 3, t + 2, t + 3, b + 2, b + 3))
+                    if gelu:
+                        self.gelu_quad(t, self.F16_EM[(rb32 + 1) & 1], t + 2, self.F16_EM[(rb32 + 1) & 1] + 8)
+                    e("v_cvt_pk_f16_f32 v%d, v%d, v%d" % (t, t, t + 1))
+                    e("v_cvt_pk_f16_f32 v%d, v%d, v%d" % (t + 1, t + 2, t + 3))
+                    e("ds_write_b64 v%d, v[%d:%d] offset:%d" % (V_PARK + cb, t, t + 1, sub * 4096))
+            for it in range(8):
+                e("ds_read_b128 v[%d:%d], v%d offset:%d" % (em + 4 * it, em + 4 * it + 3, V_EADDR + (it & 3), (it >> 2) * 4096))
+            for it in range(8):
+                e("s_waitcnt lgkmcnt(%d)" % (7 - it))
+                e("buffer_store_dwordx4 v[%d:%d], v%d, s[%d:%d], 0 offen%s" % (em + 4 * it, em + 4 * it + 3, V_O, SRD_O, SRD_O + 3, self.sched.get("store_policy", "")))
+                e("v_add_u32 v%d, s%d, v%d" % (V_O, S_ROW4, V_O))
+
     def epilogue_f16(self, gelu, vm):
+        if self.m16:
+            return self.epilogue_f16_m16(gelu, vm)
         e = self.e
         self.c("---- epilogue: bias (+ GELU) -> fp16, through the wave's slab so that 16 lanes store one 256-byte row piece")
         e("s_nop 7")
@@ -401,6 +541,8 @@
         self.c("---- epilogue: out = resid + gamma * (acc + bias) in fp32; eight 32x64 slabs through the wave's 8 KiB; the residual")
         self.c("     slabs come through a ring of three (two requested in the last K-tile, one more ahead of every slab processed).")
         e("s_nop 7")
+        if self.m16:
+            e("s_nop 7")
         self.tile_offsets(4)
         e("v_add_u32 v%d, s%d, v%d" % (V_O, S_TOFF, V_OLANE))
         if self.lnp:
@@ -426,7 +568,12 @@
             after_slab = dict((j, j + 3) for j in range(5))
         for slab in range(8):
             rb, h = slab >> 1, slab & 1
-            for cbl in range(2):
+            if self.m16:
+                for sub in range(2):
+                    for cbl in range(4):
+                        blk = ((2 * rb + sub) * 8 + 4 * h + cbl) * 4
+                        e("ds_write_b128 v%d, a[%d:%d] offset:%d" % (V_PARK + cbl, blk, blk + 3, sub * 4096))
+            for cbl in range(0 if self.m16 else 2):
                 for q in range(4):
                     blk = (rb * 4 + 2 * h + cbl) * 16 + 4 * q
                     e("ds_write_b128 v%d, a[%d:%d]" % (V_PARK + cbl * 4 + q, blk, blk + 3))
@@ -542,8 +689,8 @@
         e("v_lshrrev_b32 v%d, 6, v0" % V_T0)
         e("s_nop 1")
         e("v_readfirstlane_b32 s%d, v%d" % (S_WV, V_T0))
-        e("v_and_b32 v%d, 31, v%d" % (V_LR, V_LANE))
-        e("v_lshrrev_b32 v%d, 5, v%d" % (V_LG, V_LANE))
+        e("v_and_b32 v%d, %d, v%d" % (V_LR, 15 if self.m16 else 31, V_LANE))
+        e("v_lshrrev_b32 v%d, %d, v%d" % (V_LG, 4 if self.m16 else 5, V_LANE))
         e("s_waitcnt lgkmcnt(0)")
         e("s_lshr_b32 s%d, s%d, 1" % (S_WR, S_WV))
         e("s_and_b32 s%d, s%d, 1" % (S_WC, S_WV))
@@ -597,12 +744,12 @@
         e("v_lshrrev_b32 v%d, 1, v%d" % (V_T0, V_LR))
         e("v_and_b32 v%d, 7, v%d" % (V_T0, V_T0))
         e("v_lshlrev_b32 v%d, 7, v%d" % (V_T1, V_LR))
-        for ks in range(4):
-            e("v_or_b32 v%d, %d, v%d" % (V_T2, 2 * ks, V_LG))
+        for ks in range(2 if self.m16 else 4):
+            e("v_or_b32 v%d, %d, v%d" % (V_T2, (4 if self.m16 else 2) * ks, V_LG))
             e("v_xor_b32 v%d, v%d, v%d" % (V_T2, V_T2, V_T0))
             e("v_lshl_add_u32 v%d, v%d, 4, v%d" % (V_T2, V_T2, V_T1))
-            e("v_add_u32 v%d, s%d, v%d" % (V_FA + ks, S_FA, V_T2))
-            e("v_add_u32 v%d, s%d, v%d" % (V_FB + ks, S_FB, V_T2))
+            e("v_add_u32 v%d, s%d, v%d" % (self.M16_FA[ks] if self.m16 else V_FA + ks, S_FA, V_T2))
+            e("v_add_u32 v%d, s%d, v%d" % (self.M16_FB[ks] if self.m16 else V_FB + ks, S_FB, V_T2))
         e("v_lshrrev_b32 v%d, 3, v%d" % (V_T0, V_LANE))
         e("s_lshl_b32 s%d, s%d, 3" % (S_T0, S_WV))
         e("v_add_u32 v%d, s%d, v%d" % (V_T0, S_T0, V_T0))
@@ -622,7 +769,20 @@
         e("v_and_b32 v%d, 15, v%d" % (V_T0, V_LR))
         e("v_lshlrev_b32 v%d, 8, v%d" % (V_T1, V_LR))
         e("v_add_u32 v%d, s%d, v%d" % (V_T1, S_T0, V_T1))
-        if self.epi == EPI_F32:
+        if self.m16 and self.epi == EPI_F32:
+            e("v_xor_b32 v%d, v%d, v%d" % (V_T0, V_T0, V_LG))
+            for cbl in range(4):
+                e("v_xor_b32 v%d, %d, v%d" % (V_T2, 4 * cbl, V_T0))
+                e("v_lshl_add_u32 v%d, v%d, 4, v%d" % (V_PARK + cbl, V_T2, V_T1))
+        elif self.m16:
+            e("v_lshrrev_b32 v%d, 1, v%d" % (V_T2, V_LG))
+            e("v_xor_b32 v%d, v%d, v%d" % (V_T0, V_T0, V_T2))
+            e("v_and_b32 v%d, 1, v%d" % (V_T2, V_LG))
+            e("v_lshl_add_u32 v%d, v%d, 3, v%d" % (V_T1, V_T2, V_T1))
+            for cb in range(8):
+                e("v_xor_b32 v%d, %d, v%d" % (V_T2, 2 * cb, V_T0))
+                e("v_lshl_add_u32 v%d, v%d, 4, v%d" % (V_PARK + cb, V_T2, V_T1))
+        elif self.epi == EPI_F32:
             e("v_xor_b32 v%d, v%d, v%d" % (V_T0, V_T0, V_LG))
             for cq in range(8):
                 e("v_xor_b32 v%d, %d, v%d" % (V_T2, (cq >> 2) * 8 + 2 * (cq & 3), V_T0))
@@ -703,7 +863,7 @@
             e("v_add_u32 v%d, s%d, v%d" % (V_T1, S_T0, V_T0))
             e("v_add_u32 v%d, s%d, v%d" % (V_T2, S_T1, V_T0))
             e("v_mov_b32 v%d, 0x40000000" % V_T3)
-            e("v_cmp_eq_u32 vcc, 1, v%d" % V_LG)
+            e(("v_cmp_ne_u32 vcc, 0, v%d" if self.m16 else "v_cmp_eq_u32 vcc, 1, v%d") % V_LG)
             e("v_cndmask_b32 v%d, v%d, v%d, vcc" % (V_T1, V_T1, V_T3))
             e("v_cndmask_b32 v%d, v%d, v%d, vcc" % (V_T2, V_T2, V_T3))
             e("v_lshlrev_b32 v%d, 3, v%d" % (V_T0, V_LR))
@@ -748,6 +908,48 @@
             e("s_mov_b32 s%d, s%d" % (S_KREM, S_NK))
         e("s_waitcnt vmcnt(16)")
         e("s_barrier")
+        if self.m16:
+            self.kloop16()
+        else:
+            self.kloop32()
+        self.after_kloop()
+
+    def kloop16(self):
+        e, n = self.e, self.name
+        for idx in self.RD16_ORDER:
+            e(self.frag_read16(0, idx))
+        for r in (self.M16_FA[0], self.M16_FB[0]):
+            e("v_xor_b32 v%d, 0x%x, v%d" % (r, LDS_BUF, r))
+        slots, zslots, waits = self.build_slots16(), self.build_slots16(True), self.lgkm_waits16()
+        def run(sl, lo, hi, zero):
+            for s in range(lo, hi):
+                if s in waits:
+                    e("s_waitcnt lgkmcnt(%d)" % waits[s])
+                e(self.mfma16(s // 64, (s % 64) // 8, s % 8, zero))
+                for ins in sl[s]:
+                    if ins.endswith(":"):
+                        self.lab(ins[:-1])
+                    else:
+                        e(ins)
+        self.lab("L_tile_begin_%s" % n)
+        if self.sched.get("trace"):
+            e("s_memtime s[%d:%d]" % (S_TS0, S_TS0 + 1))
+        run(zslots, 0, 64, True)
+        e("s_branch L_after_ks0_%s" % n)
+        self.L.append(".p2align 4")
+        self.lab("L_loop_%s" % n)
+        run(slots, 0, 64, False)
+        self.lab("L_after_ks0_%s" % n)
+        run(slots, 64, 128, False)
+        e("s_xor_b32 s%d, s%d, 0x%x" % (S_M0BASE, S_M0BASE, LDS_BUF))
+        for r in (self.M16_FA[0], self.M16_FB[0]):
+            e("v_xor_b32 v%d, 0x%x, v%d" % (r, LDS_BUF, r))
+        e("s_sub_u32 s%d, s%d, 1" % (S_KREM, S_KREM))
+        e("s_cmp_eq_u32 s%d, 0" % S_KREM)
+        e("s_cbranch_scc0 L_loop_%s" % n)
+
+    def kloop32(self):
+        e, n = self.e, self.name
         for i in range(16):
             e(self.frag_read(i // 8, i // 8, i % 8))
         for r in (V_FA, V_FA + 1, V_FB, V_FB + 1):
@@ -780,6 +982,10 @@
         e("s_sub_u32 s%d, s%d, 1" % (S_KREM, S_KREM))
         e("s_cmp_eq_u32 s%d, 0" % S_KREM)
         e("s_cbranch_scc0 L_loop_%s" % n)
+
+    def after_kloop(self):
+        e, n = self.e, self.name
+        esize = 4 if self.epi == EPI_F32 else 2
         if self.sched.get("trace"):
             e("s_memtime s[%d:%d]" % (S_TS1, S_TS1 + 1))
             e("s_waitcnt lgkmcnt(0)")
@@ -787,6 +993,7 @@
             e("s_add_u32 s%d, s%d, s%d" % (S_ACC_LOOP, S_ACC_LOOP, S_T0))
             e("s_add_u32 s%d, s%d, s%d" % (S_NKT, S_NKT, S_NK))
         n_dma_after = 0 if self.sched.get("no_dma") else sum(1 for p in range(16) if self.sched["dma"][p] > self.sched.get("pre_slot", 17))
+        assert not self.m16 or n_dma_after in (0, 16)
         if self.sched.get("no_epilogue"):
             pass
         else:
@@ -795,7 +1002,7 @@
             vm = self.pre_epilogue()
             self.pre_code = self.L
             self.L = pre_lines
-            n_late = 0 if self.sched.get("no_dma") else sum(1 for p in range(16) if self.sched["dma"][p] > 48)
+            n_late = n_dma_after if self.m16 else 0 if self.sched.get("no_dma") else sum(1 for p in range(16) if self.sched["dma"][p] > 48)
             vm += [("dma", 0)] * (n_dma_after - n_late)
             if self.lnc:
                 pre_lines = self.L
@@ -849,11 +1056,17 @@
         self.lab("L_switch_%s" % n)
         self.switch_tile()
         e("s_branch L_switch_ret_%s" % n)
+        if self.m16:
+            self.lab("L_switch_z_%s" % n)
+            self.switch_tile()
+            e("s_branch L_switch_ret_z_%s" % n)
         if not self.sched.get("no_epilogue"):
             self.lab("L_pre_%s" % n)
             self.L += self.pre_code
+            if self.lnc and self.m16:
+                self.L += self.pre2_code
             e("s_branch L_pre_ret_%s" % n)
-            if self.lnc:
+            if self.lnc and not self.m16:
                 self.lab("L_pre2_%s" % n)
                 self.L += self.pre2_code
                 e("s_branch L_pre2_ret_%s" % n)
@@ -875,6 +1088,16 @@
         "resid_policy": " nt",
         "store_policy": " nt",
     }
+
+
+def m16_sched(base=None):
+    dma = [41 + 5 * p for p in range(16)]
+    busy = set(dma) | set(d - 1 for d in dma)
+    free = [s for s in range(93, 128) if s not in busy]
+    return dict(base or default_sched(), mfma="16x16x32",
+                rd1=[1 + 2 * i for i in range(16)],
+                tog1=(32, 35), pre_slot=33, barA=36, dma=dma, barB=92,
+                rd0=free[:16], adv=free[16])
 
 
 def experiment_scheds():
@@ -930,7 +1153,11 @@
     out += [("psam_gemm_asm_f32_sk", EPI_F32, dict(keep, splitk=True))]
     ln = dict(base, ln_cons=True, ln_prod=True, store16_policy=" nt")
     out += [("psam_gemm_asm_f16_ln", EPI_F16, ln), ("psam_gemm_asm_gelu_ln", EPI_GELU_F16, ln), ("psam_gemm_asm_f32_ln", EPI_F32, ln)]
+    out += [("psam_gemm_asm_f16_m16", EPI_F16, m16_sched(base)), ("psam_gemm_asm_gelu_m16", EPI_GELU_F16, m16_sched(base)), ("psam_gemm_asm_f32_m16", EPI_F32, m16_sched(base))]
+    out += [("psam_gemm_asm_f16_ln_m16", EPI_F16, m16_sched(ln)), ("psam_gemm_asm_gelu_ln_m16", EPI_GELU_F16, m16_sched(ln)), ("psam_gemm_asm_f32_ln_m16", EPI_F32, m16_sched(ln))]
     if "--experiments" in sys.argv:
+        for nm, epi in (("f16", EPI_F16), ("gelu", EPI_GELU_F16), ("f32", EPI_F32)):
+            out.append(("psam_gemm_asm_%s_m16_v1" % nm, epi, m16_sched(dict(base, trace=True))))
         for i, sc in enumerate(experiment_scheds()):
             for nm, epi in (("f16", EPI_F16), ("gelu", EPI_GELU_F16), ("f32", EPI_F32)):
                 out.append(("psam_gemm_asm_%s_v%d" % (nm, i + 1), epi, sc))
diff --git a/protosam_amd/ops.py b/protosam_amd/ops.py
--- a/protosam_amd/ops.py
+++ b/protosam_amd/ops.py
@@ -257,6 +257,13 @@
 def gemm_set_tile(tile):
     _bump_dispatch()
     _lib.check(_lib.lib().psam_gemm_set_tile(int(tile)), "psam_gemm_set_tile")
+
+
+def gemm_last_tile():
+    import ctypes
+    t = ctypes.c_int(0)
+    _lib.check(_lib.lib().psam_gemm_last_tile(ctypes.byref(t)), "psam_gemm_last_tile")
+    return t.value
 
 
 def gemm_set_option(name, value):
```

New measurement: 168.2, median of 6. 4.9% higher.
